# pqh22/ProxyTransformation

Hardware: AMD Instinct MI355X
Metric: scenes/sec (100k pts, 256 clusters, 64 proxies) (higher is better)
Workload: dtype f32; 1 GPU; cfg2: N=100000 pts, gs=8->M'=256 kept clusters, L=64 text + V=196 image proxies, d=256, eval forward; scenes_per_gpu=4, img_feat_dtype=bf16, input_sets_rotated=3, streams=1, lanes=1 (one forward at a time), setup_forwards=32

## Files before the change

proxytransformation_amd/csrc/api.hip:

```cpp
#include <atomic>
#include <chrono>
#include <cmath>
#include <cstdlib>
#include <cstring>
#include <mutex>
#include <utility>
#include <vector>

#include "common.h"

namespace ptx {

static thread_local char g_err[512] = "";

void set_error(const char *fmt, ...)
{
    va_list ap;
    va_start(ap, fmt);
    vsnprintf(g_err, sizeof(g_err), fmt, ap);
    va_end(ap);
}

static const char *const kKernelNames[] = {
    "k_minmax", "k_cluster", "k_select", "k_tags",
    "k_slot_net<pointnet>", "k_img_mean", "k_gemm_nt[qkv0]",
    "k_gemm_nt[we]", "img_pass2", "img_pass3", "k_gemm_nt[o]", "k_gemm_nt[c_proj]",
    "k_ln_rows[norm_img]", "k_gemm_nt[qkv+proxy_proj]", "k_gemm_nt[pp_img]", "k_attn32[proxy_as_query]",
    "k_attn32[proxy_as_key]", "k_gemm_nt[proj]", "k_gemm_nt[fc1]", "k_gemm_nt[fc2]",
    "k_heads", "k_affine<compact>", "k_proxy_attn[fused]", "k_mlp[fc1+gelu+fc2]",
    "k_gate[fork]", "k_signal[join]", "k_gate[join]", "k_gate[tags]", "k_signal[tags]"};
enum Kid : int {
    KID_MINMAX = 0, KID_CLUSTER, KID_SELECT, KID_TAGS, KID_POINTNET,
    KID_IMG_MEAN, KID_IMG_QKV0, KID_IMG_WE, KID_IMG_SCORES, KID_IMG_GATHER, KID_IMG_O, KID_IMG_C,
    KID_IMG_LN, KID_BLK_QKV, KID_BLK_PP, KID_BLK_ATTN_A, KID_BLK_ATTN_B, KID_BLK_PROJ, KID_BLK_FC1,
    KID_BLK_FC2, KID_BLK_HEADS, KID_AFFINE, KID_BLK_ATTN_F, KID_BLK_MLP,
    KID_GATE_FORK, KID_SIGNAL_JOIN, KID_GATE_JOIN, KID_GATE_TAGS, KID_SIGNAL_TAGS, KID_COUNT};
static_assert(sizeof(kKernelNames) / sizeof(kKernelNames[0]) == KID_COUNT, "kernel name table");

struct TimingRec { int kid; hipEvent_t a, b; };
struct TimingState {
    std::mutex mu;
    uint64_t mask = 0;
    int every = 1;
    unsigned seen[64] = {};
    std::vector<TimingRec> pool;
    size_t used = 0;
};
static TimingState g_timing;

static thread_local hipEvent_t g_ext_a = nullptr, g_ext_b = nullptr;
bool timing_ext_take(hipEvent_t *a, hipEvent_t *b)
{
    if (g_ext_a == nullptr) return false;
    *a = g_ext_a; *b = g_ext_b;
    g_ext_a = g_ext_b = nullptr;
    return true;
}

struct Timed {
    hipEvent_t stop = nullptr; hipStream_t st;
    Timed(int kid, hipStream_t s, bool ext = false) : st(s) {
        if (!((g_timing.mask >> kid) & 1u)) return;
        hipStreamCaptureStatus cap = hipStreamCaptureStatusNone;
        if (hipStreamIsCapturing(s, &cap) != hipSuccess || cap != hipStreamCaptureStatusNone) return;
        std::lock_guard<std::mutex> lk(g_timing.mu);
        if (g_timing.seen[kid]++ % (unsigned)g_timing.every != 0) return;
        if (g_timing.used == g_timing.pool.size()) {
            hipEvent_t a, b;
            if (hipEventCreate(&a) != hipSuccess || hipEventCreate(&b) != hipSuccess) return;
            g_timing.pool.push_back(TimingRec{kid, a, b});
        }
        TimingRec &pr = g_timing.pool[g_timing.used++];
        pr.kid = kid;
        if (ext) { g_ext_a = pr.a; g_ext_b = pr.b; return; }
        (void)hipEventRecord(pr.a, st);
        stop = pr.b;
    }
    ~Timed() {
        if (stop) (void)hipEventRecord(stop, st);
        if (g_ext_a != nullptr) {
            (void)hipEventRecord(g_ext_a, st); (void)hipEventRecord(g_ext_b, st);
            g_ext_a = g_ext_b = nullptr;
        }
    }
};
#define PTX_TIMED(kid, st, call) do { ::ptx::Timed t_(kid, st); PTX_TRY(call); } while (0)
#define PTX_TIMED_EXT(kid, st, call) do { ::ptx::Timed t_(kid, st, true); PTX_TRY(call); } while (0)

static inline float attn_scale(int hd) { return (float)(1.0 / std::sqrt((double)hd)); }

int validate_shape(const PtxShape &s)
{
    const long M = (long)s.grid_size * s.grid_size * s.grid_size;
    PTX_REQUIRE(s.B >= 1 && s.N >= 1, "shape: B=%d N=%d", s.B, s.N);
    PTX_REQUIRE(s.grid_size >= 1 && M <= (1 << 20), "shape: grid_size=%d", s.grid_size);
    PTX_REQUIRE(s.K >= 1 && s.K <= 63, "shape: num_sub K=%d must be in [1,63]", s.K);
    PTX_REQUIRE(s.Mk >= 1 && s.Mk <= s.Mt && s.Mt <= M, "shape: need 1 <= Mk=%d <= Mt=%d <= M=%ld", s.Mk, s.Mt, M);
    PTX_REQUIRE(s.C == 256 || s.C == 512, "shape: embed_dim=%d; supported: 256 (the reference, PRE:302) and 512", s.C);
    PTX_REQUIRE((s.heads == 4 || s.heads == 8 || s.heads == 16) && (s.C / s.heads == 32 || s.C / s.heads == 64),
                "shape: num_heads=%d with embed_dim=%d; the image-pool and attention kernels are built for 4, 8 or 16 heads of "
                "head_dim 32 or 64", s.heads, s.C);
    PTX_REQUIRE(s.Mt <= 4096, "shape: Mt=%d clusters after the empty-drop; the farthest point sampling holds at most 4096", s.Mt);
    PTX_REQUIRE(s.hidden >= 4 && s.hidden % 4 == 0, "shape: hidden=%d", s.hidden);
    PTX_REQUIRE(s.in_dim >= 64 && s.in_dim % 64 == 0 && s.in_dim <= 2048,
                "shape: in_dim=%d must be a multiple of 64, at most 2048", s.in_dim);
    PTX_REQUIRE(s.L >= 1 && s.V >= 1, "shape: L=%d V=%d", s.L, s.V);
    PTX_REQUIRE(s.img_dtype >= 0 && s.img_dtype <= 2, "shape: img_dtype=%d (0 fp32, 1 bf16, 2 fp16)", s.img_dtype);
    if (s.img_dtype == 0) PTX_REQUIRE(s.hw >= 4 && s.hw <= 256, "shape: H*W=%d (fp32 image features: 4..256 pixels)", s.hw);
    else PTX_REQUIRE(s.hw >= 8 && s.hw <= 256, "shape: H*W=%d (16-bit image features: 8..256 pixels)", s.hw);
    PTX_REQUIRE((long)s.Mk * s.K < (1l << 31) - 1, "shape: Mk*K overflows the ownership tag");
    return PTX_OK;
}

PrepLayout prep_layout(const PtxShape &s)
{
    PrepLayout P{};
    size_t o = 0;
    auto take = [&](size_t n) { size_t r = o; o += align_up(n, 64); return r; };
    P.hd = s.C / s.heads;
    P.KT1 = s.in_dim + s.hw + 1;
    P.KT2p = (int)align_up((size_t)s.in_dim + s.hw + 1, 4);
    P.off_ab = take(2 * kSlotHidden); P.enc_ab = take(2 * (size_t)s.C);
    P.ttn_ab = take(6); P.itn_ab = take(18);
    P.posb_t = take((size_t)s.Mk * s.C); P.posb_i = take((size_t)s.Mk * s.C);
    P.w3 = take((size_t)3 * s.C * s.in_dim); P.b3 = take((size_t)3 * s.C);
    P.t1 = take((size_t)s.heads * P.KT1 * P.hd);
    P.t2 = take((size_t)s.heads * P.hd * P.KT2p);
    P.ppg_w = take((size_t)s.C * s.C); P.ppg_c = take(s.C);
    for (int i = 0; i < 2; ++i) {
        P.fc1g_w[i] = take((size_t)s.hidden * s.C); P.fc1g_c[i] = take(s.hidden);
        const size_t planes = mlp_fused_supported(s.C, s.hidden, 1, 0) ? (size_t)s.hidden * s.C * 3 / 2 : 0;
        P.mlp_w1p[i] = take(planes); P.mlp_w2p[i] = take(planes);
    }
    for (int i = 0; i < 2; ++i) P.qkvb[i] = take((size_t)s.Mk * 3 * s.C);
    P.total = o;
    return P;
}

struct LayoutForce { int v[4]; };
static LayoutForce layout_force()
{
    LayoutForce f{{-1, -1, -1, -1}};
    if (const char *e = getenv("PTX_LAYOUT"))
        for (int i = 0; i < 4 && e[i] != '\0'; ++i) f.v[i] = e[i] == '0' ? 0 : (e[i] == '1' ? 1 : -1);
    return f;
}
struct LayoutChoice { double est_cluster, est_image; bool cluster_on_caller, img_late, early; LayoutForce lf; };
static LayoutChoice choose_layout(const PtxShape &S)
{
    static const LayoutForce lf = layout_force();
    LayoutChoice c{};
    c.lf = lf;
    const int B = S.B, Kd = S.Mt - S.Mk;
    const double img_mb = (double)B * S.V * S.in_dim * S.hw * (S.img_dtype == 0 ? 4.0 : 2.0) * 1e-6;
    c.est_cluster = 80.0 + 0.42 * Kd;
    c.est_image = 40.0 + (S.img_dtype == 0 ? 0.98 : 0.78) * img_mb;
    c.cluster_on_caller = lf.v[0] >= 0 ? lf.v[0] != 0 : c.est_cluster > c.est_image + 60.0;
    c.img_late = c.cluster_on_caller && (lf.v[2] >= 0 ? lf.v[2] != 0 : c.est_image + 60.0 < 0.8 * c.est_cluster);
    const double est_all = 1.8 * 12.0 * (double)B * S.Mt * S.C * S.C / 70e6;
    c.early = c.cluster_on_caller && (lf.v[1] >= 0 ? lf.v[1] != 0 : (Kd >= 128 && (long)B * S.Mk >= 1024 && est_all < 3.0 * 0.42 * Kd));
    return c;
}

WsLayout ws_layout(const PtxShape &s)
{
    WsLayout L{};
    const PrepLayout P = prep_layout(s);
    size_t o = 0;
    auto take = [&](size_t bytes) { size_t r = o; o += align_up(bytes, 256); return r; };
    const size_t B = s.B, N = s.N, K = s.K, C = s.C;
    const size_t M = (size_t)s.grid_size * s.grid_size * s.grid_size;
    const size_t Mk = s.Mk, Mt = s.Mt, Kd = s.Mt - s.Mk;
    const size_t nimg = B * s.V, Lp = s.L > s.V ? s.L : s.V, R = B * Mk;
    L.zero_begin = o;
    L.mm_enc = take(B * 6 * 4);
    L.scene_acc = take(B * 2 * 4);
    L.tag = take(B * N * 4);
    L.fa_ticket = take(2 * B * s.heads * 4);
    L.mlp_ticket = take(mlp_ticket_bytes((int)R));
    L.mm_ticket = take(4);
    L.zero_bytes = o - L.zero_begin;
    L.minmax = take(B * 6 * 4);
    L.centers0 = take(B * M * 3 * 4); L.cluster1 = take(B * M * K * 3 * 4);
    L.offsets = take(B * M * 3 * 4);  L.centers = take(B * M * 3 * 4);
    L.idx2 = take(B * M * K * 4);     L.cluster2 = take(B * M * K * 3 * 4);
    L.pad_count = take(B * M * 4);
    L.order = take(B * Mt * 4); L.picks = take(B * (Kd ? Kd : 1) * 4); L.keep = take(B * Mk * 4); L.ksrc = take(B * Mk * 4);
    L.kcenter = take(B * Mk * 3 * 4); L.kcluster = take(B * Mk * K * 3 * 4); L.kidx = take(B * Mk * K * 4);
    L.drop_idx = take(B * (Kd ? Kd : 1) * K * 4);
    L.tile_counts = take(B * (size_t)cdiv(s.N, kTilePts) * 4);
    L.point_proxy = take(R * C * 4);
    for (int i = 0; i < 2; ++i) L.x_in[i] = take(R * C * 4);
    bool may_early = false;
    for (int dt = 0; dt < 3; ++dt) { PtxShape t = s; t.img_dtype = dt; may_early = may_early || choose_layout(t).early; }
    const size_t em = may_early ? 1 : 0;
    L.pp_all = take(em * B * Mt * C * 4); L.order_e = take(em * B * Mt * 4);
    for (int i = 0; i < 2; ++i) { L.xln_all[i] = take(em * B * Mt * C * 4); L.g_all[i] = take(em * B * Mt * 3 * C * 4); }
    L.fm = take(nimg * s.in_dim * 4); L.qkv0 = take(nimg * 3 * C * 4);
    L.we = take(nimg * s.heads * (size_t)P.KT1 * 4);
    {
        const size_t pool_b = img_pool_bytes((int)nimg, s.in_dim, P.KT2p - s.in_dim), gbuf_b = nimg * s.heads * (size_t)P.KT2p * 4;
        L.pool = L.gbuf = take(pool_b > gbuf_b ? pool_b : gbuf_b);
    }
    L.obuf = take(nimg * C * 4); L.cbuf = take(nimg * C * 4); L.img_proxy = take(nimg * C * 4);
    for (int i = 0; i < 2; ++i) {
        L.qkv[i] = take(R * 3 * C * 4); L.pt[i] = take(B * Lp * C * 4); L.pv[i] = take(B * Lp * C * 4);
        L.ao[i] = take(R * C * 4); L.x1[i] = take(R * C * 4); L.xn2[i] = take(0);
        L.hbuf[i] = take(mlp_fused_supported(s.C, s.hidden, (int)R, 0) ? 0 : R * (size_t)s.hidden * 4);
        L.x2[i] = take(R * C * 4); L.guide[i] = take(R * C * 4);
        L.head[i] = take(R * 9 * 4);
        L.lnp_x1[i] = take(R * (C / 32) * 2 * 4);
    }
    L.lnp_img = take(nimg * (C / 32) * 2 * 4);
    const size_t fsp = fattn_split_for(s.B, s.heads);
    L.fa_part = take(fsp > 1 ? 2 * B * s.heads * fsp * Mk * kFaPartRow * 4 : 0);
    L.mlp_part = take(mlp_fused_supported(s.C, s.hidden, (int)R, 0) ? mlp_part_bytes((int)R) : 0);
    L.total = o;
    return L;
}

}
struct PtxContext {
    int dev = -1;
    hipStream_t st = nullptr, lo = nullptr;
    hipEvent_t fork = nullptr, join = nullptr, aux = nullptr, tags = nullptr, early_a = nullptr, early_b = nullptr;
    uint32_t *gate = nullptr; uint32_t gate_seq = 0;
    uint32_t *gate_err = nullptr;
    bool gates_on = false;
    bool probed = false; hipStream_t probed_st = nullptr;
    bool lo_ok = false;
    hipStream_t last_st = nullptr;
    bool have_last = false;
    uint64_t gate_ticks = 0, probe_ticks = 0; int gate_trap = 0;
    std::mutex mu;
};
namespace ptx {

static bool env_on(const char *name)
{
    const char *v = getenv(name);
    return v != nullptr && v[0] != '\0' && !(v[0] == '0' && v[1] == '\0');
}
static bool gates_allowed()
{
    if (const char *g = getenv("PTX_GATE")) return atoi(g) != 0;
    for (const char *name : {"ROCPROF_COUNTER_COLLECTION", "ROCPROF_COUNTERS", "ROCPROF_COUNTER_GROUPS", "ROCPROF_ADVANCED_THREAD_TRACE",
                             "ROCPROF_PC_SAMPLING_UNIT", "ROCPROF_PC_SAMPLING_METHOD", "AMD_SERIALIZE_KERNEL", "AMD_SERIALIZE_COPY",
                             "HIP_LAUNCH_BLOCKING", "CUDA_LAUNCH_BLOCKING", "ROCPROFILER_METRICS_PATH", "ROCP_METRICS"})
        if (env_on(name)) return false;
    return true;
}

static int context_init(PtxContext *c)
{
    PTX_HIP(hipGetDevice(&c->dev));
    int lo = 0, hi = 0;
    PTX_HIP(hipDeviceGetStreamPriorityRange(&lo, &hi));
    PTX_HIP(hipStreamCreateWithPriority(&c->st, hipStreamNonBlocking, hi));
    PTX_HIP(hipStreamCreateWithPriority(&c->lo, hipStreamNonBlocking, lo));
    PTX_HIP(hipEventCreateWithFlags(&c->fork, hipEventDisableTiming));
    PTX_HIP(hipEventCreateWithFlags(&c->join, hipEventDisableTiming));
    PTX_HIP(hipEventCreateWithFlags(&c->aux, hipEventDisableTiming));
    PTX_HIP(hipEventCreateWithFlags(&c->tags, hipEventDisableTiming));
    PTX_HIP(hipEventCreateWithFlags(&c->early_a, hipEventDisableTiming));
    PTX_HIP(hipEventCreateWithFlags(&c->early_b, hipEventDisableTiming));
    if (gates_allowed()) {
        PTX_HIP(hipMalloc(reinterpret_cast<void **>(&c->gate), 256));
        PTX_HIP(hipMemset(c->gate, 0, 256));
        PTX_HIP(hipHostMalloc(reinterpret_cast<void **>(&c->gate_err), 64, hipHostMallocMapped));
        c->gate_err[0] = 0u;
        int khz = 0;
        if (hipDeviceGetAttribute(&khz, hipDeviceAttributeWallClockRate, c->dev) != hipSuccess || khz <= 0) khz = 100000;
        const char *ms_env = getenv("PTX_GATE_TIMEOUT_MS");
        const long ms = ms_env ? atol(ms_env) : 30000;
        c->gate_ticks = (uint64_t)(ms > 0 ? ms : 1) * (uint64_t)khz;
        c->probe_ticks = (uint64_t)20 * (uint64_t)khz;
#ifdef PTX_TEST_HOOKS
        c->gate_trap = env_on("PTX_GATE_TRAP") ? 1 : 0;
#endif
        c->gates_on = true;
    }
    return PTX_OK;
}

static void context_release(PtxContext *c)
{
    if (c->gate) (void)hipFree(c->gate);
    if (c->gate_err) (void)hipHostFree(c->gate_err);
    c->gate = nullptr; c->gate_err = nullptr; c->gates_on = false;
    if (c->fork) (void)hipEventDestroy(c->fork);
    if (c->join) (void)hipEventDestroy(c->join);
    if (c->aux) (void)hipEventDestroy(c->aux);
    if (c->tags) (void)hipEventDestroy(c->tags);
    if (c->early_a) (void)hipEventDestroy(c->early_a);
    if (c->early_b) (void)hipEventDestroy(c->early_b);
    if (c->st) (void)hipStreamDestroy(c->st);
    if (c->lo) (void)hipStreamDestroy(c->lo);
    c->fork = c->join = c->aux = c->tags = nullptr; c->st = c->lo = nullptr;
}

static std::mutex g_default_mu;
static PtxContext *g_default_ctx[16] = {};

static int default_context(PtxContext **out)
{
    int dev = 0;
    PTX_HIP(hipGetDevice(&dev));
    PTX_REQUIRE(dev >= 0 && dev < 16, "device %d out of range", dev);
    std::lock_guard<std::mutex> lk(g_default_mu);
    if (g_default_ctx[dev] == nullptr) {
        PtxContext *c = new PtxContext();
        const int rc = context_init(c);
        if (rc != PTX_OK) { context_release(c); delete c; return rc; }
        g_default_ctx[dev] = c;
    }
    *out = g_default_ctx[dev];
    return PTX_OK;
}

int make_scene_pts(const float *stacked, const float *const *list, int B, int N, ScenePts *out)
{
    PTX_REQUIRE(B >= 1 && B <= kMaxScenes, "at most %d scenes per call (got %d): split the batch", kMaxScenes, B);
    PTX_REQUIRE(stacked || list, "null points");
    for (int b = 0; b < kMaxScenes; ++b) out->p[b] = nullptr;
    for (int b = 0; b < B; ++b) {
        out->p[b] = list ? list[b] : stacked + (size_t)b * N * 3;
        PTX_REQUIRE(out->p[b] != nullptr, "null point cloud for scene %d", b);
    }
    return PTX_OK;
}

template <typename T>
static inline T *at(void *base, size_t off) { return reinterpret_cast<T *>(static_cast<char *>(base) + off); }

__global__ void k_signal(uint32_t *flag, uint32_t seq)
{
    if (threadIdx.x == 0) __hip_atomic_store(flag, seq, __ATOMIC_RELAXED, __HIP_MEMORY_SCOPE_AGENT);
}
__global__ void k_gate(GateRef g)
{
    if (threadIdx.x == 0) gate_wait(g);
}

static GateRef gate_ref(const PtxContext *c, int word, uint32_t seq, uint32_t site, bool probe = false)
{
    const uint64_t ticks = probe ? c->probe_ticks : ((site == 2 || site == 7) ? 2 * c->gate_ticks : c->gate_ticks);
    return GateRef{c->gate + word, seq, c->gate_err, probe ? nullptr : c->gate + 48, ticks, site, probe ? 0 : c->gate_trap};
}

static int gate_check(PtxContext *c)
{
    if (c->gate_err == nullptr) return PTX_OK;
    const uint32_t e = *reinterpret_cast<volatile uint32_t *>(c->gate_err);
    if (e == 0u) return PTX_OK;
    static const char *const site_name[] = {"?", "fork (clustering stream waiting for the caller's stream)",
                                            "join (caller's stream waiting for the other chain)", "probe, fork direction",
                                            "probe, join direction", "?", "slot tags' fork (tag stream waiting for the selection)",
                                            "slot tags' join (caller's stream waiting for the tags)"};
    const unsigned site = (e >> 24) & 0x7fu;
    c->gates_on = false;
    *reinterpret_cast<volatile uint32_t *>(c->gate_err) = 0u;
    (void)hipStreamSynchronize(c->st);
    if (c->have_last) (void)hipStreamSynchronize(c->last_st);
    (void)hipMemset(c->gate + 48, 0, 4);
    set_error("stream gate timed out at the %s of forward #%u: the two chains of that forward were not ordered and its outputs "
              "were set to NaN; this context now orders its streams with events (PTX_GATE=0 selects them from the start)",
              site_name[site < 8 ? site : 0], e & 0xffffffu);
    return PTX_EGATE;
}

static int gate_probe_pair(PtxContext *c, hipStream_t waiter, hipStream_t releaser, int word, uint32_t site, bool *ok)
{
    const uint32_t seq = ++c->gate_seq;
    hipLaunchKernelGGL(k_gate, dim3(1), dim3(64), 0, waiter, gate_ref(c, word, seq, site, true));
    PTX_LAUNCHED("k_gate[probe]");
    hipLaunchKernelGGL(k_signal, dim3(1), dim3(64), 0, releaser, c->gate + word, seq);
    PTX_LAUNCHED("k_signal[probe]");
    PTX_HIP(hipStreamSynchronize(waiter));
    PTX_HIP(hipStreamSynchronize(releaser));
    *ok = *reinterpret_cast<volatile uint32_t *>(c->gate_err) == 0u;
    *reinterpret_cast<volatile uint32_t *>(c->gate_err) = 0u;
    return PTX_OK;
}
static int gate_probe(PtxContext *c, hipStream_t st)
{
    c->probed = true; c->probed_st = st; c->lo_ok = false;
    if (!c->gates_on) return PTX_OK;
    PTX_HIP(hipStreamSynchronize(st));
    PTX_HIP(hipStreamSynchronize(c->st));
    PTX_HIP(hipStreamSynchronize(c->lo));
    bool fork_ok = false, join_ok = false, t1 = false, t2 = false;
    PTX_TRY(gate_probe_pair(c, c->st, st, 40, 3, &fork_ok));
    PTX_TRY(gate_probe_pair(c, st, c->st, 44, 4, &join_ok));
    if (!fork_ok || !join_ok) { c->gates_on = false; return PTX_OK; }
    PTX_TRY(gate_probe_pair(c, c->lo, c->st, 40, 3, &t1));
    PTX_TRY(gate_probe_pair(c, st, c->lo, 44, 4, &t2));
    c->lo_ok = t1 && t2;
    return PTX_OK;
}

static int run_img_proxy(const PtxShape &s, const PtxWeights &w, const float *prep, const void *img,
                         float *img_proxy, void *ws, hipStream_t st, int phase = 0, bool need_ln = true,
                         int i0 = 0, int ni = -1, uint32_t *gate = nullptr, uint32_t gate_seq = 0)
{
    const PrepLayout P = prep_layout(s);
    const WsLayout L = ws_layout(s);
    const int C = s.C, hd = P.hd, nall = s.B * s.V, nimg = ni < 0 ? nall : ni;
    float *fm = at<float>(ws, L.fm) + (size_t)i0 * s.in_dim, *qkv0 = at<float>(ws, L.qkv0) + (size_t)i0 * 3 * C;
    float *we = at<float>(ws, L.we) + (size_t)i0 * s.heads * P.KT1, *gbuf = at<float>(ws, L.gbuf) + (size_t)i0 * s.heads * P.KT2p;
    float *obuf = at<float>(ws, L.obuf) + (size_t)i0 * C, *cbuf = at<float>(ws, L.cbuf) + (size_t)i0 * C;
    if (img_proxy) img_proxy += (size_t)i0 * C;
    const int dt = s.img_dtype;
    img = static_cast<const char *>(img) + (size_t)i0 * s.in_dim * s.hw * (dt == 0 ? 4 : 2);
    float *Gs = nullptr, *E = nullptr, *ML = nullptr;
    const int EW = P.KT2p - s.in_dim;
    const bool pooled32 = img_pool32_supported(dt, s.in_dim, s.hw, s.heads);
    const bool pooled = pooled32 || img_pool_supported(dt, s.in_dim, s.hw, s.heads);
    if (pooled) {
        img_pool_layout(at<float>(ws, L.pool), nall, s.in_dim, EW, &Gs, &E, &ML);
        Gs += (size_t)i0 * 2 * s.heads * s.in_dim; E += (size_t)i0 * s.heads * EW; ML += (size_t)i0 * s.heads * 5;
    }
    if (phase != 2) PTX_TIMED(KID_IMG_MEAN, st, launch_img_mean(img, dt, nimg, s.in_dim, s.hw, fm, st, gate, gate_seq));
    if (phase == 1) return PTX_OK;
    const bool chained = hd == 32 && nimg < 4096;
    {
        GemmBatch g{}; g.n = 1;
        g.p[0] = GemmProb{fm, prep + P.w3, qkv0, prep + P.b3, nullptr, nullptr, nullptr,
                          nimg, 3 * C, s.in_dim, s.in_dim, s.in_dim, 3 * C, 0, 0, 0, EPI_NONE};
        if (chained) {
            g.p[0].w2 = prep + P.t1; g.p[0].c2 = we; g.p[0].n2 = P.KT1; g.p[0].ldc2 = s.heads * P.KT1;
            g.p[0].chain_tiles = s.heads; g.p[0].w2_stride = (long)P.KT1 * hd; g.p[0].c2_stride = P.KT1;
        }
        PTX_TIMED(KID_IMG_QKV0, st, launch_gemm(g, st));
    }
    if (!chained) {
        for (int h0 = 0; h0 < s.heads; h0 += kMaxGroups) {
            GemmBatch g{}; g.n = std::min(kMaxGroups, s.heads - h0);
            for (int h = h0; h < h0 + g.n; ++h)
                g.p[h - h0] = GemmProb{qkv0 + h * hd, prep + P.t1 + (size_t)h * P.KT1 * hd, we + (size_t)h * P.KT1,
                                       nullptr, nullptr, nullptr, nullptr, nimg, P.KT1, hd, 3 * C, hd,
                                       s.heads * P.KT1, 0, 0, 0, EPI_NONE};
            PTX_TIMED(KID_IMG_WE, st, launch_gemm(g, st));
        }
    }
    if (pooled32) {
        PTX_TIMED_EXT(KID_IMG_SCORES, st, launch_img_pool32(static_cast<const float *>(img), we, qkv0, nimg, s.in_dim, s.hw, C, P.KT1, EW,
                                                        attn_scale(hd), Gs, E, ML, st));
    } else if (pooled) {
        PTX_TIMED_EXT(KID_IMG_SCORES, st, launch_img_pool(img, dt, we, qkv0, nimg, s.in_dim, s.hw, C, P.KT1,
                                                      EW, attn_scale(hd), Gs, E, ML, st));
    } else {
        PTX_TIMED(KID_IMG_SCORES, st, launch_img_scores(img, dt, we, qkv0, nimg, s.in_dim, s.hw, s.heads, C, P.KT1,
                                                        P.KT2p, attn_scale(hd), gbuf, st));
        PTX_TIMED(KID_IMG_GATHER, st, launch_img_gather(img, dt, nimg, s.in_dim, s.hw, s.heads, P.KT2p, gbuf, st));
    }
    for (int h0 = 0; h0 < s.heads; h0 += kMaxGroups) {
        GemmBatch g{}; g.n = std::min(kMaxGroups, s.heads - h0);
        for (int h = h0; h < h0 + g.n; ++h) {
            GemmProb &gp = g.p[h - h0];
            gp = GemmProb{gbuf + (size_t)h * P.KT2p, prep + P.t2 + (size_t)h * hd * P.KT2p, obuf + h * hd,
                          w.v_b + h * hd, nullptr, gbuf + (size_t)h * P.KT2p + s.in_dim,
                          qkv0 + 2 * C + h * hd, nimg, hd, P.KT2p, s.heads * P.KT2p, P.KT2p, C,
                          0, s.heads * P.KT2p, 3 * C, EPI_NONE};
            if (pooled) {
                gp.A = nullptr; gp.rs = nullptr;
                gp.pg = Gs + (size_t)h * s.in_dim; gp.ldg = 2 * s.heads * s.in_dim; gp.gslab = s.heads * s.in_dim;
                gp.pe = E + (size_t)h * EW; gp.lde = s.heads * EW;
                gp.pml = ML + (size_t)h * 5; gp.ldml = s.heads * 5;
                gp.kg = s.in_dim;
            }
        }
        PTX_TIMED(KID_IMG_O, st, launch_gemm(g, st));
    }
    {
        GemmBatch g{}; g.n = 1;
        g.p[0] = GemmProb{obuf, w.c_w, cbuf, w.c_b, nullptr, nullptr, nullptr,
                          nimg, C, C, C, C, C, 0, 0, 0, EPI_NONE};
        g.p[0].lnp_out = at<float>(ws, L.lnp_img) + (size_t)i0 * (C / 32) * 2;
        PTX_TIMED(KID_IMG_C, st, launch_gemm(g, st));
    }
    if (need_ln) {
        LnBatch lb{}; lb.n = 1; lb.C = C; lb.eps = s.ln_eps;
        lb.p[0] = LnProb{cbuf, img_proxy, w.norm_img_w, w.norm_img_b, nullptr, nimg, 1};
        PTX_TIMED(KID_IMG_LN, st, launch_ln_rows(lb, st));
    }
    return PTX_OK;
}

struct Branch {
    const PtxBlock *blk; const float *x_in; const float *proxy; int Lp; const uint8_t *mask;
    const float *head_w, *head_b, *head_ab; int nout; float *head_out; float *guide; int slot;
    bool late_proxy;
    const float *proxy_lnp, *pp_gw, *pp_gc;
    const float *fc1_gw, *fc1_gc;
    const float *prep;
};

static bool fused_attn_pays(const PtxShape &s, const Branch *br, int nb)
{
    (void)br;
    const long wgs = (long)s.B * s.heads * nb;
    return s.Mk <= 256 || wgs >= 96;
}

static int run_blocks(const PtxShape &s, const Branch *br, int nb, const float *point_proxy, void *ws,
                      hipStream_t st, int phase = 0, int cd = 0, GateRef *join = nullptr, GateRef *tags_join = nullptr,
                      bool skip_qkv = false)
{
    const WsLayout L = ws_layout(s);
    const int C = s.C, R = s.B * s.Mk;
    {
        GemmBatch g{}; g.n = 0;
        for (int i = 0; i < nb; ++i) {
            const int sl = br[i].slot;
            if (phase != 2 && phase != 3 && phase != 4 && !skip_qkv)
                g.p[g.n++] = GemmProb{br[i].x_in, br[i].blk->qkv_w, at<float>(ws, L.qkv[sl]), br[i].blk->qkv_b,
                                      nullptr, nullptr, nullptr, R, 3 * C, C, C, C, 3 * C, 0, 0, 0, EPI_NONE};
            const bool now = phase == 0 || (phase == 1 && !br[i].late_proxy) || ((phase == 2 || phase == 3) && br[i].late_proxy);
            if (now && phase != 4) {
                GemmProb &q = g.p[g.n++];
                q = GemmProb{br[i].proxy, br[i].blk->pp_w, at<float>(ws, L.pt[sl]), br[i].blk->pp_b,
                             nullptr, nullptr, nullptr, s.B * br[i].Lp, C, C, C, C, C, 0, 0, 0, EPI_NONE};
                if (br[i].proxy_lnp != nullptr) {
                    q.W = br[i].pp_gw; q.bias = nullptr;
                    q.lnp_in = br[i].proxy_lnp; q.ln_c = br[i].pp_gc;
                    q.ln_parts = C / 32; q.ln_C = C; q.ln_eps = s.ln_eps;
                }
            }
        }
        if (g.n > 0 && (phase == 2 || phase == 1) && join != nullptr && join->flag != nullptr) { g.tail_gate = *join; join->flag = nullptr; }
        if (g.n > 0) PTX_TIMED(phase == 2 || phase == 3 ? KID_BLK_PP : KID_BLK_QKV, st, launch_gemm(g, st, cd));
        if (phase == 1 || phase == 3) return PTX_OK;
    }
    FAttnBatch fa{}; fa.nb = nb; fa.B = s.B; fa.heads = s.heads; fa.hd = C / s.heads; fa.n = s.Mk; fa.C = C;
    fa.scale = attn_scale(C / s.heads); fa.compute_dtype = cd;
    fa.split = fattn_split_for(s.B, s.heads); fa.part = at<float>(ws, L.fa_part); fa.tickets = at<int>(ws, L.fa_ticket);
    for (int i = 0; i < nb; ++i) {
        const int sl = br[i].slot;
        fa.p[i] = FAttnProb{at<float>(ws, L.qkv[sl]), at<float>(ws, L.pt[sl]), br[i].mask, at<float>(ws, L.ao[sl]), br[i].Lp};
    }
    const bool fused = fused_attn_supported(fa) && (cd == 1 || fused_attn_pays(s, br, nb));
    if (fused) PTX_TIMED(KID_BLK_ATTN_F, st, launch_proxy_attn(fa, st));
    AttnBatch a{}; a.n = nb; a.B = s.B; a.heads = s.heads; a.hd = C / s.heads; a.scale = attn_scale(C / s.heads);
    for (int i = 0; i < nb && !fused; ++i) {
        const int sl = br[i].slot;
        float *qkv = at<float>(ws, L.qkv[sl]);
        a.p[i] = AttnProb{at<float>(ws, L.pt[sl]), qkv + C, qkv + 2 * C, at<float>(ws, L.pv[sl]), nullptr,
                          br[i].Lp, s.Mk, C, 3 * C, 3 * C, C,
                          (long)br[i].Lp * C, (long)s.Mk * 3 * C, (long)s.Mk * 3 * C, (long)br[i].Lp * C};
    }
    if (!fused) PTX_TIMED(KID_BLK_ATTN_A, st, launch_attn32(a, st));
    for (int i = 0; i < nb && !fused; ++i) {
        const int sl = br[i].slot;
        float *qkv = at<float>(ws, L.qkv[sl]);
        a.p[i] = AttnProb{qkv, at<float>(ws, L.pt[sl]), at<float>(ws, L.pv[sl]), at<float>(ws, L.ao[sl]),
                          br[i].mask, s.Mk, br[i].Lp, 3 * C, C, C, C,
                          (long)s.Mk * 3 * C, (long)br[i].Lp * C, (long)br[i].Lp * C, (long)s.Mk * C};
    }
    if (!fused) PTX_TIMED(KID_BLK_ATTN_B, st, launch_attn32(a, st));
    {
        GemmBatch g{}; g.n = nb;
        for (int i = 0; i < nb; ++i) {
            const int sl = br[i].slot;
            g.p[i] = GemmProb{at<float>(ws, L.ao[sl]), br[i].blk->proj_w, at<float>(ws, L.x1[sl]),
                              br[i].blk->proj_b, point_proxy, nullptr, nullptr, R, C, C, C, C, C, C, 0, 0, EPI_NONE};
            g.p[i].lnp_out = at<float>(ws, L.lnp_x1[sl]);
        }
        if (tags_join != nullptr && tags_join->flag != nullptr) { g.tail_gate = *tags_join; tags_join->flag = nullptr; }
        PTX_TIMED(KID_BLK_PROJ, st, launch_gemm(g, st, cd));
    }
    if (mlp_fused_supported(C, s.hidden, R, cd)) {
        const PrepLayout P = prep_layout(s);
        MlpBatch mb{}; mb.n = nb; mb.ln_eps = s.ln_eps; mb.compute_dtype = cd;
        mb.part = at<float>(ws, L.mlp_part); mb.tickets = at<int>(ws, L.mlp_ticket);
        for (int i = 0; i < nb; ++i) {
            const int sl = br[i].slot;
            mb.p[i] = MlpProb{at<float>(ws, L.x1[sl]), at<float>(ws, L.lnp_x1[sl]), br[i].prep + P.mlp_w1p[sl],
                              br[i].prep + P.mlp_w2p[sl], br[i].fc1_gc, br[i].blk->fc2_b,
                              at<float>(ws, L.x2[sl]), R,
                              br[i].blk->out_norm_w, br[i].blk->out_norm_b, br[i].head_w, br[i].head_b, br[i].head_ab,
                              br[i].head_out, br[i].guide, br[i].nout};
        }
        PTX_TIMED(KID_BLK_MLP, st, launch_mlp(mb, st));
        return PTX_OK;
    } else {
    {
        GemmBatch g{}; g.n = nb;
        for (int i = 0; i < nb; ++i) {
            const int sl = br[i].slot;
            g.p[i] = GemmProb{at<float>(ws, L.x1[sl]), br[i].fc1_gw, at<float>(ws, L.hbuf[sl]),
                              nullptr, nullptr, nullptr, nullptr, R, s.hidden, C, C, C, s.hidden,
                              0, 0, 0, EPI_GELU};
            g.p[i].lnp_in = at<float>(ws, L.lnp_x1[sl]); g.p[i].ln_c = br[i].fc1_gc;
            g.p[i].ln_parts = C / 32; g.p[i].ln_C = C; g.p[i].ln_eps = s.ln_eps;
        }
        PTX_TIMED(KID_BLK_FC1, st, launch_gemm(g, st, cd));
    }
    {
        GemmBatch g{}; g.n = nb;
        for (int i = 0; i < nb; ++i) {
            const int sl = br[i].slot;
            g.p[i] = GemmProb{at<float>(ws, L.hbuf[sl]), br[i].blk->fc2_w, at<float>(ws, L.x2[sl]),
                              br[i].blk->fc2_b, at<float>(ws, L.x1[sl]), nullptr, nullptr, R, C, s.hidden,
                              s.hidden, s.hidden, C, C, 0, 0, EPI_NONE};
        }
        PTX_TIMED(KID_BLK_FC2, st, launch_gemm(g, st, cd));
    }
    }
    HeadBatch hb{}; hb.n = nb; hb.C = C; hb.eps = s.ln_eps;
    for (int i = 0; i < nb; ++i) {
        const int sl = br[i].slot;
        hb.p[i] = HeadProb{at<float>(ws, L.x2[sl]), br[i].blk->out_norm_w, br[i].blk->out_norm_b,
                           br[i].head_w, br[i].head_b, br[i].head_ab, br[i].head_out, br[i].guide, R, br[i].nout};
    }
    PTX_TIMED(KID_BLK_HEADS, st, launch_heads(hb, st));
    return PTX_OK;
}

static Branch make_branch(const PtxShape &s, const PtxWeights &w, const float *prep, int which,
                          const float *x_in, const float *proxy, int Lp, const uint8_t *mask,
                          float *head_out, float *guide)
{
    const PrepLayout P = prep_layout(s);
    Branch b{};
    b.blk = which == 0 ? &w.text : &w.img;
    b.x_in = x_in; b.proxy = proxy; b.Lp = Lp; b.mask = mask;
    b.head_w = which == 0 ? w.text_trans_w : w.img_trans_w;
    b.head_b = which == 0 ? w.text_trans_b : w.img_trans_b;
    b.head_ab = prep + (which == 0 ? P.ttn_ab : P.itn_ab);
    b.nout = which == 0 ? 3 : 9;
    b.head_out = head_out; b.guide = guide; b.slot = which; b.late_proxy = which == 1;
    b.proxy_lnp = nullptr; b.pp_gw = prep + P.ppg_w; b.pp_gc = prep + P.ppg_c;
    b.fc1_gw = prep + P.fc1g_w[which]; b.fc1_gc = prep + P.fc1g_c[which];
    b.prep = prep;
    return b;
}

static int check_bufs(const PtxShape *s, const void *ws, size_t ws_bytes)
{
    PTX_REQUIRE(s != nullptr, "null shape");
    PTX_TRY(validate_shape(*s));
    PTX_REQUIRE(ws != nullptr, "null workspace");
    const size_t need = ws_layout(*s).total;
    if (ws_bytes < need) { set_error("workspace too small: %zu < %zu bytes", ws_bytes, need); return PTX_ENOSPACE; }
    PTX_REQUIRE((reinterpret_cast<uintptr_t>(ws) & 255) == 0, "workspace must be 256-byte aligned");
    return PTX_OK;
}

}

using namespace ptx;

extern "C" {

int ptx_abi_version(void) { return PTX_ABI_VERSION; }

int ptx_kernel_count(void) { return KID_COUNT; }
const char *ptx_kernel_name(int kid) { return kid >= 0 && kid < KID_COUNT ? kKernelNames[kid] : nullptr; }

int ptx_timing_select(int kid)
{
    PTX_REQUIRE(kid >= -1 && kid < KID_COUNT, "ptx_timing_select: kid=%d", kid);
    std::lock_guard<std::mutex> lk(g_timing.mu);
    g_timing.mask = kid < 0 ? 0 : (1ull << kid);
    g_timing.used = 0;
    for (unsigned &s : g_timing.seen) s = 0;
    return PTX_OK;
}

int ptx_timing_every(int n)
{
    PTX_REQUIRE(n >= 1, "ptx_timing_every: n=%d", n);
    std::lock_guard<std::mutex> lk(g_timing.mu);
    g_timing.every = n;
    return PTX_OK;
}

int ptx_timing_select_mask(uint64_t mask)
{
    static_assert(KID_COUNT <= 64, "timing mask is 64 bits");
    std::lock_guard<std::mutex> lk(g_timing.mu);
    g_timing.mask = mask & ((KID_COUNT >= 64) ? ~0ull : ((1ull << KID_COUNT) - 1));
    g_timing.used = 0;
    for (unsigned &s : g_timing.seen) s = 0;
    return PTX_OK;
}

static int timing_collect(int *launches, float *total_ms, int nsites)
{
    for (int k = 0; k < nsites; ++k) { launches[k] = 0; total_ms[k] = 0.0f; }
    for (size_t i = 0; i < g_timing.used; ++i) {
        const TimingRec &r = g_timing.pool[i];
        PTX_HIP(hipEventSynchronize(r.b));
        float ms = 0.0f;
        PTX_HIP(hipEventElapsedTime(&ms, r.a, r.b));
        const int k = nsites == 1 ? 0 : r.kid;
        if (k >= 0 && k < nsites) { launches[k] += 1; total_ms[k] += ms; }
    }
    g_timing.used = 0;
    return PTX_OK;
}

int ptx_timing_read(int *launches, float *total_ms)
{
    PTX_REQUIRE(launches && total_ms, "ptx_timing_read: null argument");
    std::lock_guard<std::mutex> lk(g_timing.mu);
    return timing_collect(launches, total_ms, 1);
}

int ptx_timing_read_sites(int *launches, float *total_ms, int n)
{
    PTX_REQUIRE(launches && total_ms && n == KID_COUNT, "ptx_timing_read_sites: need arrays of ptx_kernel_count() = %d entries", KID_COUNT);
    std::lock_guard<std::mutex> lk(g_timing.mu);
    return timing_collect(launches, total_ms, n);
}
const char *ptx_last_error(void) { return g_err; }

int ptx_context_create(PtxContext **ctx)
{
    PTX_REQUIRE(ctx != nullptr, "ptx_context_create: null argument");
    PtxContext *c = new PtxContext();
    const int rc = context_init(c);
    if (rc != PTX_OK) { context_release(c); delete c; *ctx = nullptr; return rc; }
    *ctx = c;
    return PTX_OK;
}

int ptx_context_destroy(PtxContext *ctx)
{
    if (ctx == nullptr) return PTX_OK;
    if (ctx->st) (void)hipStreamSynchronize(ctx->st);
    if (ctx->lo) (void)hipStreamSynchronize(ctx->lo);
    context_release(ctx);
    delete ctx;
    return PTX_OK;
}

int ptx_context_check(PtxContext *ctx)
{
    PTX_REQUIRE(ctx != nullptr, "ptx_context_check: null context");
    std::lock_guard<std::mutex> lk(ctx->mu);
    return gate_check(ctx);
}

int ptx_context_sync_check(PtxContext *ctx)
{
    PTX_REQUIRE(ctx != nullptr, "ptx_context_sync_check: null context");
    std::lock_guard<std::mutex> lk(ctx->mu);
    if (ctx->have_last) PTX_HIP(hipStreamSynchronize(ctx->last_st));
    PTX_HIP(hipStreamSynchronize(ctx->st));
    PTX_HIP(hipStreamSynchronize(ctx->lo));
    return gate_check(ctx);
}

int ptx_context_gates(const PtxContext *ctx) { return ctx != nullptr && ctx->gates_on ? (ctx->lo_ok ? 3 : 1) : 0; }
// ... 534 lines not shown
```

proxytransformation_amd/csrc/common.h:

```cpp
#pragma once
#include <hip/hip_runtime.h>
#include <cstdarg>
#include <cstdint>
#include <cstdio>

#include "../../include/proxyt.h"

namespace ptx {

void set_error(const char *fmt, ...);
bool timing_ext_take(hipEvent_t *start, hipEvent_t *stop);

#define PTX_REQUIRE(cond, ...)                                   \
    do {                                                         \
        if (!(cond)) {                                           \
            ::ptx::set_error(__VA_ARGS__);                       \
            return PTX_EINVAL;                                   \
        }                                                        \
    } while (0)

#define PTX_HIP(expr)                                                              \
    do {                                                                           \
        hipError_t e_ = (expr);                                                    \
        if (e_ != hipSuccess) {                                                    \
            ::ptx::set_error("%s failed: %s", #expr, hipGetErrorString(e_));       \
            return PTX_ELAUNCH;                                                    \
        }                                                                          \
    } while (0)

#define PTX_LAUNCHED(name)                                                         \
    do {                                                                           \
        hipError_t e_ = hipGetLastError();                                         \
        if (e_ != hipSuccess) {                                                    \
            ::ptx::set_error("launch %s failed: %s", name, hipGetErrorString(e_)); \
            return PTX_ELAUNCH;                                                    \
        }                                                                          \
    } while (0)

#define PTX_TRY(expr)                 \
    do {                              \
        int rc_ = (expr);             \
        if (rc_ != PTX_OK) return rc_;\
    } while (0)

constexpr int kWave = 64;
constexpr int kSlotHidden = 256;
constexpr int kTilePts = 2048;

inline size_t align_up(size_t x, size_t a) { return (x + a - 1) / a * a; }
inline int cdiv(int a, int b) { return (a + b - 1) / b; }

__device__ __forceinline__ int lane_id() { return threadIdx.x & 63; }

#define PTX_ROR_F(v, n) __int_as_float(__builtin_amdgcn_update_dpp(0, __float_as_int(v), 0x120 + (n), 0xf, 0xf, false))
#define PTX_ROR_I(v, n) __builtin_amdgcn_update_dpp(0, (v), 0x120 + (n), 0xf, 0xf, false)
#define PTX_LANE_F(v, l) __int_as_float(__builtin_amdgcn_readlane(__float_as_int(v), (l)))
__device__ __forceinline__ float wave_sum(float v) {
    v += PTX_ROR_F(v, 8); v += PTX_ROR_F(v, 4); v += PTX_ROR_F(v, 2); v += PTX_ROR_F(v, 1);
    return (PTX_LANE_F(v, 0) + PTX_LANE_F(v, 16)) + (PTX_LANE_F(v, 32) + PTX_LANE_F(v, 48));
}
__device__ __forceinline__ int wave_sum(int v) {
    v += PTX_ROR_I(v, 8); v += PTX_ROR_I(v, 4); v += PTX_ROR_I(v, 2); v += PTX_ROR_I(v, 1);
    return (__builtin_amdgcn_readlane(v, 0) + __builtin_amdgcn_readlane(v, 16)) +
           (__builtin_amdgcn_readlane(v, 32) + __builtin_amdgcn_readlane(v, 48));
}
__device__ __forceinline__ float wave_max(float v) {
    v = fmaxf(v, PTX_ROR_F(v, 8)); v = fmaxf(v, PTX_ROR_F(v, 4)); v = fmaxf(v, PTX_ROR_F(v, 2)); v = fmaxf(v, PTX_ROR_F(v, 1));
    return fmaxf(fmaxf(PTX_LANE_F(v, 0), PTX_LANE_F(v, 16)), fmaxf(PTX_LANE_F(v, 32), PTX_LANE_F(v, 48)));
}
__device__ __forceinline__ float wave_min(float v) {
    v = fminf(v, PTX_ROR_F(v, 8)); v = fminf(v, PTX_ROR_F(v, 4)); v = fminf(v, PTX_ROR_F(v, 2)); v = fminf(v, PTX_ROR_F(v, 1));
    return fminf(fminf(PTX_LANE_F(v, 0), PTX_LANE_F(v, 16)), fminf(PTX_LANE_F(v, 32), PTX_LANE_F(v, 48)));
}
__device__ __forceinline__ float wave_max_dpp(float v) { return wave_max(v); }
__device__ __forceinline__ uint32_t f2ord(float f) {
    uint32_t u = __float_as_uint(f);
    return (u & 0x80000000u) ? ~u : (u | 0x80000000u);
}
__device__ __forceinline__ float ord2f(uint32_t u) {
    return __uint_as_float((u & 0x80000000u) ? (u & 0x7fffffffu) : ~u);
}

__device__ __forceinline__ float dist2_nofma(float ax, float ay, float az, float bx, float by, float bz) {
    float dx = __fsub_rn(ax, bx), dy = __fsub_rn(ay, by), dz = __fsub_rn(az, bz);
    return __fadd_rn(__fadd_rn(__fmul_rn(dx, dx), __fmul_rn(dy, dy)), __fmul_rn(dz, dz));
}

__device__ __forceinline__ float gelu_erf(float x)
{
    const float z = fabsf(x) * 0.70710678118654752440f;
    const float t = __frcp_rn(fmaf(0.3275911f, z, 1.0f));
    float p = fmaf(1.061405429f, t, -1.453152027f);
    p = fmaf(p, t, 1.421413741f);
    p = fmaf(p, t, -0.284496736f);
    p = fmaf(p, t, 0.254829592f);
    const float erfz = 1.0f - p * t * __expf(-z * z);
    return 0.5f * x * (1.0f + copysignf(erfz, x));
}

struct GateRef {
    const uint32_t *flag; uint32_t seq;
    uint32_t *err;
    uint32_t *poison;
    uint64_t ticks;
    uint32_t site;
    int trap;
};
__device__ __forceinline__ void gate_wait(const GateRef &g)
{
    const uint64_t t0 = __builtin_amdgcn_s_memrealtime();
    for (unsigned it = 0;; ++it) {
        if ((int32_t)(__hip_atomic_load(g.flag, __ATOMIC_RELAXED, __HIP_MEMORY_SCOPE_AGENT) - g.seq) >= 0) return;
        if (it < 64) __builtin_amdgcn_s_sleep(4); else __builtin_amdgcn_s_sleep(64);
        if ((it & 7u) == 7u && __builtin_amdgcn_s_memrealtime() - t0 > g.ticks) break;
    }
    if (g.poison) __hip_atomic_store(g.poison, 1u, __ATOMIC_RELAXED, __HIP_MEMORY_SCOPE_AGENT);
    if (g.err) __hip_atomic_store(g.err, 0x80000000u | (g.site << 24) | (g.seq & 0xffffffu), __ATOMIC_RELEASE, __HIP_MEMORY_SCOPE_SYSTEM);
    if (g.trap) __builtin_trap();
}

constexpr int kMaxScenes = 32;
struct ScenePts { const float *p[kMaxScenes]; };
template <bool WAIT>
__device__ __forceinline__ void minmax_block(const float *__restrict__ p, int N, uint32_t *__restrict__ mm_enc, int b,
                                             int chunk, int nchunks, float (*red)[6])
{
    float lo[3] = {INFINITY, INFINITY, INFINITY}, hi[3] = {-INFINITY, -INFINITY, -INFINITY};
    const int tid = chunk * 256 + threadIdx.x;
    const int nth = nchunks * 256;
    const bool vec = ((N & 3) == 0) && ((reinterpret_cast<uintptr_t>(p) & 15) == 0);
    if (vec) {
        const float4 *p4 = reinterpret_cast<const float4 *>(p);
        const int nq = N >> 2;
        constexpr int U = 4;
        for (int q0 = tid; q0 < nq; q0 += nth * U) {
            float4 v[U][3];
#pragma unroll
            for (int u = 0; u < U; ++u) {
                const int q = min(q0 + u * nth, nq - 1);
                v[u][0] = p4[3 * q]; v[u][1] = p4[3 * q + 1]; v[u][2] = p4[3 * q + 2];
            }
#pragma unroll
            for (int u = 0; u < U; ++u) {
                const float4 a = v[u][0], c = v[u][1], e = v[u][2];
                const float xs[4] = {a.x, a.w, c.z, e.y}, ys[4] = {a.y, c.x, c.w, e.z}, zs[4] = {a.z, c.y, e.x, e.w};
#pragma unroll
                for (int i = 0; i < 4; ++i) {
                    lo[0] = fminf(lo[0], xs[i]); hi[0] = fmaxf(hi[0], xs[i]);
                    lo[1] = fminf(lo[1], ys[i]); hi[1] = fmaxf(hi[1], ys[i]);
                    lo[2] = fminf(lo[2], zs[i]); hi[2] = fmaxf(hi[2], zs[i]);
                }
            }
        }
    } else {
        for (int i = tid; i < N; i += nth) {
#pragma unroll
            for (int d = 0; d < 3; ++d) {
                float v = p[(size_t)i * 3 + d];
                lo[d] = fminf(lo[d], v); hi[d] = fmaxf(hi[d], v);
            }
        }
    }
#pragma unroll
    for (int d = 0; d < 3; ++d) { lo[d] = wave_min(lo[d]); hi[d] = wave_max(hi[d]); }
    const int w = threadIdx.x >> 6;
    if (lane_id() == 0) {
#pragma unroll
        for (int d = 0; d < 3; ++d) { red[w][d] = lo[d]; red[w][3 + d] = hi[d]; }
    }
    __syncthreads();
    if (threadIdx.x < 6) {
        const int d = threadIdx.x;
        float v = red[0][d];
        for (int i = 1; i < 4; ++i) v = d < 3 ? fminf(v, red[i][d]) : fmaxf(v, red[i][d]);
        uint32_t old = 0u;
        if (d < 3) { if (v != INFINITY) old = atomicMax(&mm_enc[b * 6 + d], ~f2ord(v)); }
        else       { if (v != -INFINITY) old = atomicMax(&mm_enc[b * 6 + d], f2ord(v)); }
        if (WAIT) asm volatile("" :: "v"(old));
    }
}
inline int minmax_chunks(int N) { int c = (N + 256 * 16 - 1) / (256 * 16); return c < 1 ? 1 : (c > 256 ? 256 : c); }

__device__ __forceinline__ void mean_prologue(uint32_t *gate, uint32_t gate_seq)
{
    if (gate != nullptr && blockIdx.x == 0 && threadIdx.x == 0) __hip_atomic_store(gate, gate_seq, __ATOMIC_RELAXED, __HIP_MEMORY_SCOPE_AGENT);
}

struct PrepLayout {
    size_t off_ab, enc_ab;
    size_t ttn_ab, itn_ab;
    size_t posb_t, posb_i;
    size_t w3, b3;
    size_t t1;
    size_t t2;
    size_t ppg_w, ppg_c;
    size_t fc1g_w[2], fc1g_c[2];
    size_t mlp_w1p[2], mlp_w2p[2];
    size_t qkvb[2];
    size_t total;
    int KT1, KT2p, hd;
};
PrepLayout prep_layout(const PtxShape &s);

struct WsLayout {
    size_t zero_begin, zero_bytes;
    size_t mm_enc;
    size_t scene_acc;
    size_t tag;
    size_t fa_ticket;
    size_t mlp_ticket;
    size_t mm_ticket;
    size_t minmax, centers0, cluster1, offsets, centers, idx2, cluster2, pad_count;
    size_t order, picks, keep, ksrc, kcenter, kcluster, kidx, drop_idx, tile_counts;
    size_t point_proxy, x_in[2];
    size_t pp_all, xln_all[2], g_all[2];
    size_t order_e;
    size_t fm, qkv0, we, pool, gbuf, obuf, cbuf, img_proxy;
    size_t qkv[2], pt[2], pv[2], ao[2], x1[2], xn2[2], hbuf[2], x2[2], guide[2], head[2];
    size_t lnp_img, lnp_x1[2];
    size_t fa_part;
    size_t mlp_part;
    size_t total;
};
WsLayout ws_layout(const PtxShape &s);

int validate_shape(const PtxShape &s);

enum : int { EPI_NONE = 0, EPI_GELU = 1 };
struct GemmProb {
    const float *A; const float *W; float *C;
    const float *bias;
    const float *res;
    const float *rs;
    const float *ad;
    int R, N, K, lda, ldw, ldc, ldres, rs_stride, ldad, epi;
    const float *pg, *pe, *pml; int ldg, gslab, lde, ldml, kg;
    float *lnp_out;
    const float *lnp_in, *ln_c; int ln_parts, ln_C; float ln_eps;
    const float *w2; float *c2; int n2, ldc2, chain_tiles; long w2_stride, c2_stride;
};
constexpr int kMaxGroups = 8;
struct GemmBatch {
    GemmProb p[kMaxGroups]; int n; int rotate;
    GateRef tail_gate;
};
int launch_gemm(const GemmBatch &gb, hipStream_t st, int compute_dtype = 0);
int gemm_policy(int min_tiles_128);

struct LnProb { const float *x; float *y; const float *w; const float *b; const float *add; int R, add_rows; };
struct LnBatch { LnProb p[2]; int n; int C; float eps; };
int launch_ln_rows(const LnBatch &lb, hipStream_t st);

struct HeadProb {
    const float *x; const float *nw; const float *nb;
    const float *hw; const float *hb;
    const float *ab;
    float *out; float *guide; int R, nout;
};
struct HeadBatch { HeadProb p[2]; int n; int C; float eps; };
int launch_heads(const HeadBatch &hb, hipStream_t st);

struct AttnProb {
    const float *Q, *K, *V; float *O; const uint8_t *mask;
    int nq, nk, ldq, ldk, ldv, ldo;
    long sQ, sK, sV, sO;
};
struct AttnBatch { AttnProb p[2]; int n; int B, heads, hd; float scale; };
int launch_attn32(const AttnBatch &ab, hipStream_t st);

struct FAttnProb { const float *qkv, *pt; const uint8_t *mask; float *out; int Lp; };
struct FAttnBatch {
    FAttnProb p[2]; int nb, B, heads, hd, n, C; float scale; int compute_dtype;
    int split; float *part; int *tickets;
};
int fattn_split_for(int B, int heads);
constexpr int kFaMaxSplit = 4, kFaPartRow = 34;
bool fused_attn_supported(const FAttnBatch &ab);
int launch_proxy_attn(const FAttnBatch &ab, hipStream_t st);

struct MlpProb {
    const float *x1, *lnp;
    const void *w1p, *w2p;
    const float *fc1_c, *b2;
    float *x2; int R;
    const float *nw, *nb, *hw, *hb, *ab; float *head_out, *guide; int nout;
};
struct MlpBatch { MlpProb p[2]; int n; float ln_eps; float *part; int *tickets; int compute_dtype; };
bool mlp_fused_supported(int C, int hidden, int R, int compute_dtype);
size_t mlp_part_bytes(int R);
size_t mlp_ticket_bytes(int R);
int launch_mlp(const MlpBatch &mb, hipStream_t st);
int launch_prep_planes(const float *W, int rows, int K, void *out, hipStream_t st);
int launch_prep_lnfold(const float *W, const float *gamma, const float *beta, const float *bias, int N, int K, float *Wg,
                       float *cv, hipStream_t st);

int make_scene_pts(const float *stacked, const float *const *list, int B, int N, ScenePts *out);

int launch_minmax(const ScenePts &points, int B, int N, uint32_t *mm_enc, hipStream_t st);
int launch_ball_query(const float *centers, const uint32_t *mm_enc, const float *lin, int gs,
                      float margin, float *minmax_out, float *centers_out, const ScenePts &points,
                      int B, int M, int N, int K, float radius, int32_t *idx, float *cluster,
                      int32_t *pad_count, hipStream_t st);
int launch_offset_net(const float *ab, const PtxSlotMlp &mlp, const float *map_w,
                      const float *centers_in, const float *cluster, const float *minmax,
                      int BM, int M, int K, float margin, float *centers_out, float *offsets_out,
                      hipStream_t st);
int launch_pointnet(const float *ab, const PtxSlotMlp &mlp, const float *kcenter,
                    const float *kcluster, int BM, int Mk, int K, int width, float *point_proxy,
                    const PtxBlock *blk_t, const PtxBlock *blk_i, const float *posb_t,
                    const float *posb_i, float *xin_t, float *xin_i, float ln_eps,
                    const int32_t *ksrc, int Msrc, hipStream_t st, uint32_t *head_flag = nullptr, uint32_t head_seq = 0,
                    bool center_src = false);
int launch_order(const PtxShape &s, const int32_t *pad_count, const int32_t *order_override, int32_t *order, hipStream_t st);
int launch_qkv_gather(const float *pp_all, const float *const g[2], const float *const tb[2], const int32_t *ksrc, int B, int M, int Mk,
                      int C, float *point_proxy, float *const qkv[2], hipStream_t st);
int launch_cluster(const PtxShape &s, const uint32_t *mm_enc, const float *lin, const ScenePts &points,
                   const float *off_ab, const PtxSlotMlp &mlp, const float *map_w, const float *centers_override,
                   float *minmax_out, float *centers0, float *cluster1, float *offsets, float *centers,
                   int32_t *idx2, float *cluster2, int32_t *pad_count, hipStream_t st, hipEvent_t done = nullptr);
int launch_select(const PtxShape &s, const int32_t *idx, const float *centers, const float *cluster,
                  const int32_t *pad_count, const int32_t *order_override, int32_t *order,
                  int32_t *picks, int32_t *keep, float *kcenter, float *kcluster, int32_t *kidx,
                  int32_t *drop_idx, uint32_t *tag, hipStream_t st);
int launch_select_order(const PtxShape &s, const float *centers, const int32_t *pad_count,
                        const int32_t *order_override, int32_t *order, int32_t *picks, int32_t *keep,
                        float *kcenter, int32_t *ksrc, uint32_t *mm_clear, hipStream_t st, bool critical,
                        hipEvent_t done, const GateRef *tail = nullptr);
int launch_tags(const PtxShape &s, const int32_t *idx, const int32_t *order, const int32_t *picks, const int32_t *ksrc,
                uint32_t *tag, int32_t *tile_counts, int32_t *counts, int32_t *scene_acc, hipStream_t st,
                const int32_t *keep = nullptr);
int launch_select_slots(const PtxShape &s, const int32_t *idx, const float *cluster, const int32_t *order,
                        const int32_t *picks, const int32_t *keep, float *kcluster, int32_t *kidx,
                        int32_t *drop_idx, uint32_t *tag, hipStream_t st);
int launch_t_ln_fwd(const float *x, const float *w, const float *b, int R, int C, float eps, float *y, float *stats, hipStream_t st);
int t_ln_chunks(int R);
int launch_t_ln_bwd(const float *x, const float *stats, const float *w, const float *dy, int R, int C, float *dx, float *part, hipStream_t st);
int launch_tile_count(const uint32_t *tag, int B, int N, int32_t *tile_counts, int32_t *counts, int32_t *scene_acc,
                      hipStream_t st);
int launch_affine(const PtxShape &s, const ScenePts &points, uint32_t *tag, const float *kcenter,
                  const float *translate, const float *transform, float *out, int32_t *counts,
                  const int32_t *tile_counts, bool compact, bool clear_tag, hipStream_t st,
                  const uint32_t *poison = nullptr);

int launch_img_mean(const void *img, int dt, int nimg, int in_dim, int hw, float *fm, hipStream_t st,
                    uint32_t *gate = nullptr, uint32_t gate_seq = 0);
int launch_img_scores(const void *img, int dt, const float *we, const float *qkv0, int nimg, int in_dim,
                      int hw, int heads, int C, int KT1, int KT2p, float scale, float *gbuf, hipStream_t st);
int launch_img_gather(const void *img, int dt, int nimg, int in_dim, int hw, int heads, int KT2p, float *gbuf,
                      hipStream_t st);
bool img_pool_supported(int dt, int in_dim, int hw, int heads);
size_t img_pool_bytes(int nimg, int in_dim, int EW);
void img_pool_layout(float *scratch, int nimg, int in_dim, int EW, float **Gs, float **E, float **ML);
int launch_img_pool(const void *img, int dt, const float *we, const float *qkv0, int nimg, int in_dim, int hw, int C,
                    int KT1, int EW, float scale, float *Gs, float *E, float *ML, hipStream_t st);

bool img_pool32_supported(int dt, int in_dim, int hw, int heads);
int launch_img_pool32(const float *img, const float *we, const float *qkv0, int nimg, int in_dim, int hw, int C, int KT1, int EW,
                      float scale, float *Gs, float *E, float *ML, hipStream_t st);

int run_prepare(const PtxShape &s, const PtxWeights &w, float *prep, hipStream_t st);

}
```

proxytransformation_amd/csrc/gemm.hip:

```cpp
#include <atomic>
#include <cstdlib>

#include "common.h"
#include "split3.h"
#include "mfma64.h"

namespace ptx {


__device__ __forceinline__ void pin4(float4 &v) { asm volatile("" : "+v"(v.x), "+v"(v.y), "+v"(v.z), "+v"(v.w)); }
__device__ __forceinline__ void ln_row_stats(const GemmProb &pr, int row, float &mu, float &rstd)
{
    const float2 *pp = reinterpret_cast<const float2 *>(pr.lnp_in) + (size_t)row * pr.ln_parts;
    constexpr int kMaxParts = 16;
    float2 v[kMaxParts];
#pragma unroll
    for (int t = 0; t < kMaxParts; ++t) v[t] = pp[min(t, pr.ln_parts - 1)];
    float s1 = 0.0f, s2 = 0.0f;
#pragma unroll
    for (int t = 0; t < kMaxParts; ++t) { s1 += t < pr.ln_parts ? v[t].x : 0.0f; s2 += t < pr.ln_parts ? v[t].y : 0.0f; }
    const float inv = 1.0f / (float)pr.ln_C;
    mu = s1 * inv;
    float between = 0.0f;
#pragma unroll
// ... 149 lines not shown
        const char *A_ = smem + (buf_) * kXBuf + (wr * 32 + li) * XROW;                    \
        const char *W_ = smem + (buf_) * kXBuf + 3 * kXPlane + (wc * 32 + li) * XROW;      \
        _Pragma("unroll") for (int kg = 0; kg < BK / 16; ++kg) {                           \
            const int o_ = xswz(li, kg * 2 + hh);            \
            const bf16x8 a1 = *reinterpret_cast<const bf16x8 *>(A_ + o_);                  \
            const bf16x8 b1 = *reinterpret_cast<const bf16x8 *>(W_ + o_);                  \
            if (NP == 1) {                                        \
                acc = __builtin_amdgcn_mfma_f32_32x32x16_bf16(a1, b1, acc, 0, 0, 0);       \
                continue;                                                                  \
            }                                                                              \
            const bf16x8 a2 = *reinterpret_cast<const bf16x8 *>(A_ + o_ + kXPlane);        \
            const bf16x8 a3 = *reinterpret_cast<const bf16x8 *>(A_ + o_ + 2 * kXPlane);    \
            const bf16x8 b2 = *reinterpret_cast<const bf16x8 *>(W_ + o_ + kXPlane);        \
            const bf16x8 b3 = *reinterpret_cast<const bf16x8 *>(W_ + o_ + 2 * kXPlane);    \
            acc = __builtin_amdgcn_mfma_f32_32x32x16_bf16(a3, b1, acc, 0, 0, 0);    \
            acc = __builtin_amdgcn_mfma_f32_32x32x16_bf16(a2, b2, acc, 0, 0, 0);           \
            acc = __builtin_amdgcn_mfma_f32_32x32x16_bf16(a1, b3, acc, 0, 0, 0);           \
            acc = __builtin_amdgcn_mfma_f32_32x32x16_bf16(a2, b1, acc, 0, 0, 0);           \
            acc = __builtin_amdgcn_mfma_f32_32x32x16_bf16(a1, b2, acc, 0, 0, 0);           \
            acc = __builtin_amdgcn_mfma_f32_32x32x16_bf16(a1, b1, acc, 0, 0, 0);           \
        }                                                                                  \
    } while (0)

template <int NKG, int REP, int NP = 3, bool LN = false>
__global__ __launch_bounds__(256) void k_gemm64x(GemmBatch gb)
{
    constexpr int kXPlane = 64 * XROW, kXBuf = 6 * kXPlane;
    static_assert(2 * kXBuf >= 4 * 32 * 33 * 4, "the LayerNorm-partials scratch re-uses the staging area");
    const GemmProb pr = gb.p[blockIdx.z];
    const int row0 = blockIdx.x * 64, col0 = blockIdx.y * 64;
    if (row0 >= pr.R || col0 >= pr.N) return;
    __shared__ __attribute__((aligned(16))) char smem[2 * kXBuf];
    __shared__ float s_mu[64], s_rs[64];
    const int tid = threadIdx.x, lane = tid & 63, wid = tid >> 6;
    const bool ln = LN && pr.lnp_in != nullptr;
    const int wr = wid >> 1, wc = wid & 1;
    const int li = lane & 31, hh = lane >> 5;
    const int sr = tid >> 3, kq = (tid & 7) * 4;
    const size_t ao0 = (size_t)min(row0 + sr, pr.R - 1) * pr.lda, ao1 = (size_t)min(row0 + sr + 32, pr.R - 1) * pr.lda;
    const size_t wo0 = (size_t)min(col0 + sr, pr.N - 1) * pr.ldw, wo1 = (size_t)min(col0 + sr + 32, pr.N - 1) * pr.ldw;
    float4 aA0, aA1, wA0, wA1, aB0, aB1, wB0, wB1, aC0, aC1, wC0, wC1, aD0, aD1, wD0, wD1;
    f32x16 acc;
#pragma unroll
    for (int i = 0; i < 16; ++i) acc[i] = 0.0f;
    const int n = col0 + wc * 32 + li;
    const float bias = (pr.bias && n < pr.N) ? pr.bias[n] : 0.0f;
    float lnc = 0.0f;
    if (ln) lnc = pr.ln_c[min(n, pr.N - 1)];
    float resv[16];
#pragma unroll
    for (int r = 0; r < 16; ++r) {
        const int row = row0 + wr * 32 + (r & 3) + 8 * (r >> 2) + 4 * hh;
        resv[r] = (pr.res && row < pr.R && n < pr.N) ? pr.res[(size_t)row * pr.ldres + n] : 0.0f;
    }
#define PTX_X64_PIPE()                                                                     \
    do {                                                                                   \
        if (NP != 3) break;          \
        __builtin_amdgcn_sched_group_barrier(0x100, 12, 0);              \
        _Pragma("unroll") for (int g_ = 0; g_ < 12; ++g_) {                                \
            __builtin_amdgcn_sched_group_barrier(0x008, 1, 0);                             \
            __builtin_amdgcn_sched_group_barrier(0x002, 7, 0);                   \
            __builtin_amdgcn_sched_group_barrier(0x200, 1, 0);                             \
        }                                                                                  \
    } while (0)
#define PTX_X64_STEP(S, SN, par_)                                                          \
    if (it + 4 < 4 * NKG || rep + 1 < REP) PTX_X64_FETCH(S, kbase + it + 4);               \
    __builtin_amdgcn_sched_barrier(0);      \
    PTX_X64_COMPUTE(par_);                                                                 \
    PTX_X64_STASH(SN, 1 - (par_));                                                         \
    PTX_X64_PIPE();                                                                        \
    __syncthreads();                                                                       \
    ++it;
    PTX_X64_FETCH(A, 0); PTX_X64_FETCH(B, 1); PTX_X64_FETCH(C, 2); PTX_X64_FETCH(D, 3);
    float mu0 = 0.0f, mu1 = 0.0f;
    if (ln) {
        if (tid < 64) {
            float mu, rs;
            ln_row_stats(pr, min(row0 + tid, pr.R - 1), mu, rs);
            s_mu[tid] = mu; s_rs[tid] = rs;
        }
        __syncthreads();
        mu0 = s_mu[sr]; mu1 = s_mu[sr + 32];
    }
    PTX_X64_STASH(A, 0);
    __syncthreads();
    int kbase = 0;
    for (int rep = 0; rep < REP; ++rep) {
        int it = 0;
#pragma unroll
        for (int g = 0; g < NKG; ++g) {
            PTX_X64_STEP(A, B, 0) PTX_X64_STEP(B, C, 1) PTX_X64_STEP(C, D, 0) PTX_X64_STEP(D, A, 1)
        }
        kbase += 4 * NKG;
    }
#undef PTX_X64_STEP
#undef PTX_X64_PIPE
    const bool ncol = n < pr.N;
    float fin[16];
#pragma unroll
    for (int r = 0; r < 16; ++r) {
        const int rl = wr * 32 + (r & 3) + 8 * (r >> 2) + 4 * hh, row = row0 + rl;
        float v = acc[r] + bias;
        if (ln) v = fmaf(s_rs[rl], acc[r], lnc);
        if (pr.epi == EPI_GELU) v = gelu_erf(v);
        const bool ok = ncol && row < pr.R;
        if (ok) {
            if (pr.rs) v = fmaf(pr.rs[(size_t)row * pr.rs_stride], pr.ad[(size_t)row * pr.ldad + n], v);
            if (pr.res) v += resv[r];
            pr.C[(size_t)row * pr.ldc + n] = v;
        }
        fin[r] = ok ? v : 0.0f;
    }
    if (pr.lnp_out != nullptr)
        ln_tile_partials(pr, fin, reinterpret_cast<float *>(smem) + wid * (32 * 33), row0 + wr * 32, (col0 >> 5) + wc,
                         (pr.N + 31) >> 5);
    PTX_TAIL_GATE(gb, tid == 0);
}
#undef PTX_X64_FETCH
#undef PTX_X64_STASH
#undef PTX_X64_COMPUTE

constexpr int kYHalf = 128 * 16 + 64, kYPlane = 2 * kYHalf, kYBuf = 6 * kYPlane;
#ifndef PTX_G128_NM
#define PTX_G128_NM 8
#endif
#ifndef PTX_G128_ORDER
#define PTX_G128_ORDER 0
#endif
#ifndef PTX_G128_SWZ
#define PTX_G128_SWZ 0
#endif
#ifndef PTX_G128_PIPE
#define PTX_G128_PIPE 1
#endif

#define PTX_Y_FETCH(S, m_)                                                                 \
    do {                                                                                   \
        const int kc_ = (m_) * 32 + kq;                                                    \
        a##S##0 = *reinterpret_cast<const float4 *>(pr.A + ao0 + kc_);                     \
        a##S##1 = *reinterpret_cast<const float4 *>(pr.A + ao0 + kc_ + 16);                \
        a##S##2 = *reinterpret_cast<const float4 *>(pr.A + ao1 + kc_);                     \
        a##S##3 = *reinterpret_cast<const float4 *>(pr.A + ao1 + kc_ + 16);                \
        w##S##0 = *reinterpret_cast<const float4 *>(pr.W + wo0 + kc_);                     \
        w##S##1 = *reinterpret_cast<const float4 *>(pr.W + wo0 + kc_ + 16);                \
        w##S##2 = *reinterpret_cast<const float4 *>(pr.W + wo1 + kc_);                     \
        w##S##3 = *reinterpret_cast<const float4 *>(pr.W + wo1 + kc_ + 16);                \
    } while (0)
#define PTX_Y_STASH(S, h_, buf_)                                                           \
    do {                                                                                   \
        float4 &pa_ = (h_) ? a##S##1 : a##S##0, &pb_ = (h_) ? a##S##3 : a##S##2;           \
        float4 &pc_ = (h_) ? w##S##1 : w##S##0, &pd_ = (h_) ? w##S##3 : w##S##2;           \
        pin4(pa_); pin4(pb_); pin4(pc_); pin4(pd_);                                        \
        if (LN) { sub4(pa_, mu0); sub4(pb_, mu1); }                                        \
        char *d_ = smem + (buf_) * kYBuf + stash_off;                                      \
        stash_parts<NP>(d_, kYPlane, pa_);                                                 \
        stash_parts<NP>(d_ + 64 * 16, kYPlane, pb_);                                       \
        stash_parts<NP>(d_ + 3 * kYPlane, kYPlane, pc_);                                   \
        stash_parts<NP>(d_ + 3 * kYPlane + 64 * 16, kYPlane, pd_);                         \
    } while (0)
#define PTX_Y_COMPUTE(buf_)                                                                \
    do {                                                                                   \
        const char *A_ = smem + (buf_) * kYBuf + frag_a;                                   \
        const char *W_ = smem + (buf_) * kYBuf + frag_w;                                   \
        bf16x8 fa[2][3], fw[2][3];                                                         \
        _Pragma("unroll") for (int i_ = 0; i_ < 2; ++i_)                                   \
            _Pragma("unroll") for (int p_ = 0; p_ < NP; ++p_) {                            \
                fa[i_][p_] = *reinterpret_cast<const bf16x8 *>(A_ + i_ * 512 + p_ * kYPlane); \
                fw[i_][p_] = *reinterpret_cast<const bf16x8 *>(W_ + i_ * 512 + p_ * kYPlane); \
            }                                                                              \
        if (NP == 3 && PTX_G128_ORDER == 0) {                                              \
            constexpr int ta_[6] = {2, 1, 0, 1, 0, 0}, tw_[6] = {0, 1, 2, 0, 1, 0};        \
            _Pragma("unroll") for (int t_ = 0; t_ < 6; ++t_)                               \
                _Pragma("unroll") for (int q_ = 0; q_ < 4; ++q_)                           \
                    acc[q_] = __builtin_amdgcn_mfma_f32_32x32x16_bf16(fa[q_ >> 1][ta_[t_]], fw[q_ & 1][tw_[t_]], acc[q_], 0, 0, 0); \
        } else if (NP == 3) {                                                              \
            _Pragma("unroll") for (int q_ = 0; q_ < 4; ++q_) acc[q_] = mfma_split6(fa[q_ >> 1], fw[q_ & 1], acc[q_]); \
        } else {                                                                           \
            _Pragma("unroll") for (int q_ = 0; q_ < 4; ++q_)                               \
                acc[q_] = __builtin_amdgcn_mfma_f32_32x32x16_bf16(fa[q_ >> 1][0], fw[q_ & 1][0], acc[q_], 0, 0, 0); \
        }                                                                                  \
    } while (0)

template <int NM, int NP = 3, bool LN = false>
__global__ __launch_bounds__(256, 2) void k_gemm128x(GemmBatch gb, int nrep)
{
    static_assert(NM >= 2 && NM % 2 == 0, "macro steps come in P / Q pairs");
    const GemmProb pr = gb.p[blockIdx.z];
    int bx = blockIdx.x, by = blockIdx.y;
    if (PTX_G128_SWZ) {
        const unsigned total = gridDim.x * gridDim.y, lin = blockIdx.x + gridDim.x * blockIdx.y;
        if ((total & 7u) == 0u) {
            const unsigned l2 = (lin & 7u) * (total >> 3) + (lin >> 3);
            bx = (int)(l2 / gridDim.y); by = (int)(l2 % gridDim.y);
        }
    }
    const int row0 = bx * 128, col0 = by * 128;
    if (row0 >= pr.R || col0 >= pr.N) return;
    __shared__ __attribute__((aligned(16))) char smem[2 * kYBuf];
    __shared__ float s_mu[128], s_rs[128];
    static_assert(2 * kYBuf >= 4 * 32 * 33 * 4, "the LayerNorm-partials scratch re-uses the staging area");
    const int tid = threadIdx.x, lane = tid & 63, wid = tid >> 6;
    const int wr = wid >> 1, wc = wid & 1;
    const int li = lane & 31, hh = lane >> 5;
    const int sr = tid >> 2, kq = (tid & 3) * 4;
    const size_t ao0 = (size_t)min(row0 + sr, pr.R - 1) * pr.lda, ao1 = (size_t)min(row0 + sr + 64, pr.R - 1) * pr.lda;
    const size_t wo0 = (size_t)min(col0 + sr, pr.N - 1) * pr.ldw, wo1 = (size_t)min(col0 + sr + 64, pr.N - 1) * pr.ldw;
    const int stash_off = (kq >> 3) * kYHalf + sr * 16 + (kq & 4) * 2;
    const int frag_a = hh * kYHalf + (wr * 64 + li) * 16, frag_w = 3 * kYPlane + hh * kYHalf + (wc * 64 + li) * 16;
    float4 aP0, aP1, aP2, aP3, wP0, wP1, wP2, wP3, aQ0, aQ1, aQ2, aQ3, wQ0, wQ1, wQ2, wQ3;
    f32x16 acc[4];
#pragma unroll
    for (int q = 0; q < 4; ++q)
#pragma unroll
        for (int i = 0; i < 16; ++i) acc[q][i] = 0.0f;
    const int total = NM * nrep;
    PTX_Y_FETCH(P, 0);
    PTX_Y_FETCH(Q, 1);
    const bool ln = LN && pr.lnp_in != nullptr;
    float mu0 = 0.0f, mu1 = 0.0f;
    if (ln) {
        if (tid < 128) {
            float mu, rs;
            ln_row_stats(pr, min(row0 + tid, pr.R - 1), mu, rs);
            s_mu[tid] = mu; s_rs[tid] = rs;
        }
        __syncthreads();
        mu0 = s_mu[sr]; mu1 = s_mu[sr + 64];
    }
    PTX_Y_STASH(P, 0, 0);
    __syncthreads();
#define PTX_Y_PIPE()                                                                       \
    do {                                                                                   \
        if (NP != 3 || !PTX_G128_PIPE) break;                                              \
        __builtin_amdgcn_sched_group_barrier(0x100, 12, 0);              \
        _Pragma("unroll") for (int g_ = 0; g_ < 12; ++g_) {                                \
            __builtin_amdgcn_sched_group_barrier(0x008, 2, 0);                             \
            __builtin_amdgcn_sched_group_barrier(0x002, 8, 0);                             \
            __builtin_amdgcn_sched_group_barrier(0x200, 1, 0);                             \
        }                                                                                  \
    } while (0)
#define PTX_Y_MACRO(S, T, u_)                                                              \
    PTX_Y_COMPUTE(0);                                                                      \
    PTX_Y_STASH(S, 1, 1);                                                                  \
    PTX_Y_PIPE();                                                                          \
    __syncthreads();                                                                       \
    if ((u_) + 2 < NM || rep + 1 < nrep) PTX_Y_FETCH(S, mbase + (u_) + 2);                 \
    __builtin_amdgcn_sched_barrier(0);                                                     \
    PTX_Y_COMPUTE(1);                                                                      \
    if ((u_) + 1 < NM || rep + 1 < nrep) PTX_Y_STASH(T, 0, 0);                             \
    PTX_Y_PIPE();                                                                          \
    __syncthreads();
    int mbase = 0;
    for (int rep = 0; rep < nrep; ++rep) {
#pragma unroll
        for (int u = 0; u < NM; u += 2) {
            PTX_Y_MACRO(P, Q, u)
            PTX_Y_MACRO(Q, P, u + 1)
        }
        mbase += NM;
    }
#undef PTX_Y_MACRO
#undef PTX_Y_PIPE
    (void)total;
    float *scratch = reinterpret_cast<float *>(smem) + wid * (32 * 33);
#pragma unroll
    for (int q = 0; q < 4; ++q) {
        const int i = q >> 1, j = q & 1;
        const int n = col0 + wc * 64 + j * 32 + li, nc = min(n, pr.N - 1);
        const bool ncol = n < pr.N;
        const float bias = pr.bias ? pr.bias[nc] : 0.0f;
        float lnc = 0.0f;
        if (ln) lnc = pr.ln_c[nc];
        float resv[16], adv[16], rsv[16];
#pragma unroll
        for (int r = 0; r < 16; ++r) {
            const int row = min(row0 + wr * 64 + i * 32 + (r & 3) + 8 * (r >> 2) + 4 * hh, pr.R - 1);
            resv[r] = pr.res ? pr.res[(size_t)row * pr.ldres + nc] : 0.0f;
            adv[r] = pr.rs ? pr.ad[(size_t)row * pr.ldad + nc] : 0.0f;
            rsv[r] = pr.rs ? pr.rs[(size_t)row * pr.rs_stride] : 0.0f;
        }
        float fin[16];
#pragma unroll
        for (int r = 0; r < 16; ++r) {
            const int rl = wr * 64 + i * 32 + (r & 3) + 8 * (r >> 2) + 4 * hh, row = row0 + rl;
            float v = acc[q][r] + bias;
            if (ln) v = fmaf(s_rs[rl], acc[q][r], lnc);
            if (pr.epi == EPI_GELU) v = gelu_erf(v);
            const bool ok = ncol && row < pr.R;
            if (pr.rs) v = fmaf(rsv[r], adv[r], v);
            if (pr.res) v += resv[r];
            if (ok) pr.C[(size_t)row * pr.ldc + n] = v;
            fin[r] = ok ? v : 0.0f;
        }
        if (pr.lnp_out != nullptr)
            ln_tile_partials(pr, fin, scratch, row0 + wr * 64 + i * 32, (col0 >> 5) + wc * 2 + j, (pr.N + 31) >> 5);
    }
    PTX_TAIL_GATE(gb, tid == 0);
}
#undef PTX_Y_FETCH
#undef PTX_Y_STASH
#undef PTX_Y_COMPUTE

template <int SK, int AMODE, bool CHAIN = false, bool LN = false>
__global__ __launch_bounds__(SK * 64) void k_gemm32(GemmBatch gb)
{
    const GemmProb pr = gb.p[blockIdx.z];
    const int row0 = blockIdx.x * 32, col0 = blockIdx.y * 32;
    if (row0 >= pr.R || col0 >= pr.N) return;
    extern __shared__ __attribute__((aligned(16))) float lds[];
    const int lane = threadIdx.x & 63;
    const int wv = __builtin_amdgcn_readfirstlane(threadIdx.x >> 6);
    float *base = lds + (size_t)wv * (4 * 32 * LDT);
    const int li = lane & 31, hh = lane >> 5;
    const int nk = (pr.K + BK - 1) / BK, per = (nk + SK - 1) / SK;
    const int it0 = wv * per, it1 = min(nk, it0 + per);
    const int r0 = lane >> 3, kq = (lane & 7) * 4;
    const size_t a0 = (size_t)min(row0 + r0, pr.R - 1) * pr.lda, a1 = (size_t)min(row0 + r0 + 8, pr.R - 1) * pr.lda;
    const size_t a2 = (size_t)min(row0 + r0 + 16, pr.R - 1) * pr.lda, a3 = (size_t)min(row0 + r0 + 24, pr.R - 1) * pr.lda;
    const size_t w0 = (size_t)min(col0 + r0, pr.N - 1) * pr.ldw, w1 = (size_t)min(col0 + r0 + 8, pr.N - 1) * pr.ldw;
    const size_t w2 = (size_t)min(col0 + r0 + 16, pr.N - 1) * pr.ldw, w3 = (size_t)min(col0 + r0 + 24, pr.N - 1) * pr.ldw;
    const float4 z4 = make_float4(0.f, 0.f, 0.f, 0.f);
    float4 aA0, aA1, aA2, aA3, wA0, wA1, wA2, wA3, aB0, aB1, aB2, aB3, wB0, wB1, wB2, wB3;
    float4 gA0 = z4, gA1 = z4, gA2 = z4, gA3 = z4, gB0 = z4, gB1 = z4, gB2 = z4, gB3 = z4;
    int kA = 0, kB = 0;
    (void)kA; (void)kB;
    size_t g0 = 0, g1 = 0, g2 = 0, g3 = 0, e0 = 0, e1 = 0, e2 = 0, e3 = 0;
    float fc0[4] = {0.f, 0.f, 0.f, 0.f}, fc1[4] = {0.f, 0.f, 0.f, 0.f}, fct[4] = {0.f, 0.f, 0.f, 0.f};
    float *cts = lds + (size_t)SK * (4 * 32 * LDT);
    float *lnst = cts + 32 + wv * 64;
    const bool ln = LN && pr.lnp_in != nullptr;
    float mu4[4] = {0.0f, 0.0f, 0.0f, 0.0f};
    if (AMODE == 1) {
#pragma unroll
        for (int i = 0; i < 4; ++i) {
            const int row = min(row0 + r0 + 8 * i, pr.R - 1);
            const float *ml = pr.pml + (size_t)row * pr.ldml;
            const float m0 = ml[0], l0 = ml[1], m1 = ml[2], l1 = ml[3], s0 = ml[4];
            const float m = fmaxf(fmaxf(m0, m1), s0);
            const float x0 = __expf(m0 - m), x1 = __expf(m1 - m), xt = __expf(s0 - m);
            const float inv = 1.0f / ((l0 * x0 + l1 * x1) + xt);
            fc0[i] = x0 * inv; fc1[i] = x1 * inv; fct[i] = xt * inv;
            if (wv == 0 && (lane & 7) == 0) cts[r0 + 8 * i] = fct[i];
        }
        g0 = (size_t)min(row0 + r0, pr.R - 1) * pr.ldg; g1 = (size_t)min(row0 + r0 + 8, pr.R - 1) * pr.ldg;
        g2 = (size_t)min(row0 + r0 + 16, pr.R - 1) * pr.ldg; g3 = (size_t)min(row0 + r0 + 24, pr.R - 1) * pr.ldg;
        e0 = (size_t)min(row0 + r0, pr.R - 1) * pr.lde; e1 = (size_t)min(row0 + r0 + 8, pr.R - 1) * pr.lde;
        e2 = (size_t)min(row0 + r0 + 16, pr.R - 1) * pr.lde; e3 = (size_t)min(row0 + r0 + 24, pr.R - 1) * pr.lde;
    }
#define PTX_FETCH(S, j_)                                                                  \
    do {                                                                                  \
        int jj_ = min((j_), cnt - 1) + rot;                                               \
        jj_ -= jj_ >= cnt ? cnt : 0;                                                      \
        const int k_ = (it0 + jj_) * BK + kq, kc_ = min(k_, pr.K - 4);                    \
        const bool ok_ = k_ < pr.K;                                                       \
        if (AMODE == 0) {                                                                 \
            a##S##0 = *reinterpret_cast<const float4 *>(pr.A + a0 + kc_);                 \
            a##S##1 = *reinterpret_cast<const float4 *>(pr.A + a1 + kc_);                 \
            a##S##2 = *reinterpret_cast<const float4 *>(pr.A + a2 + kc_);                 \
            a##S##3 = *reinterpret_cast<const float4 *>(pr.A + a3 + kc_);                 \
        } else if (kc_ < pr.kg) {               \
            a##S##0 = *reinterpret_cast<const float4 *>(pr.pg + g0 + kc_);                \
            a##S##1 = *reinterpret_cast<const float4 *>(pr.pg + g1 + kc_);                \
            a##S##2 = *reinterpret_cast<const float4 *>(pr.pg + g2 + kc_);                \
            a##S##3 = *reinterpret_cast<const float4 *>(pr.pg + g3 + kc_);                \
            g##S##0 = *reinterpret_cast<const float4 *>(pr.pg + g0 + pr.gslab + kc_);     \
            g##S##1 = *reinterpret_cast<const float4 *>(pr.pg + g1 + pr.gslab + kc_);     \
            g##S##2 = *reinterpret_cast<const float4 *>(pr.pg + g2 + pr.gslab + kc_);     \
            g##S##3 = *reinterpret_cast<const float4 *>(pr.pg + g3 + pr.gslab + kc_);     \
        } else {                                                                          \
            a##S##0 = *reinterpret_cast<const float4 *>(pr.pe + e0 + (kc_ - pr.kg));      \
            a##S##1 = *reinterpret_cast<const float4 *>(pr.pe + e1 + (kc_ - pr.kg));      \
            a##S##2 = *reinterpret_cast<const float4 *>(pr.pe + e2 + (kc_ - pr.kg));      \
            a##S##3 = *reinterpret_cast<const float4 *>(pr.pe + e3 + (kc_ - pr.kg));      \
        }                                                                                 \
        k##S = kc_;                                                                       \
        w##S##0 = *reinterpret_cast<const float4 *>(pr.W + w0 + kc_);                     \
        w##S##1 = *reinterpret_cast<const float4 *>(pr.W + w1 + kc_);                     \
        w##S##2 = *reinterpret_cast<const float4 *>(pr.W + w2 + kc_);                     \
        w##S##3 = *reinterpret_cast<const float4 *>(pr.W + w3 + kc_);                     \
        if (!ok_) { w##S##0 = z4; w##S##1 = z4; w##S##2 = z4; w##S##3 = z4; }             \
    } while (0)
#define PTX_MERGE(S, i_)                                                                  \
    do {                                                                                  \
        if (k##S < pr.kg) {                                                               \
            a##S##i_ = make_float4(a##S##i_.x * fc0[i_] + g##S##i_.x * fc1[i_], a##S##i_.y * fc0[i_] + g##S##i_.y * fc1[i_], \
                                   a##S##i_.z * fc0[i_] + g##S##i_.z * fc1[i_], a##S##i_.w * fc0[i_] + g##S##i_.w * fc1[i_]); \
        } else {                                                                          \
            const int t_ = k##S - pr.kg;       \
            a##S##i_.x *= t_ == 0 ? fct[i_] : (t_ <= 128 ? fc0[i_] : fc1[i_]);           \
            a##S##i_.y *= t_ + 1 <= 128 ? fc0[i_] : fc1[i_];                              \
            a##S##i_.z *= t_ + 2 <= 128 ? fc0[i_] : fc1[i_];                              \
            a##S##i_.w *= t_ + 3 <= 128 ? fc0[i_] : fc1[i_];                              \
        }                                                                                 \
    } while (0)
#define PTX_STASH(S, buf_)                                                                \
    do {                                                                                  \
        float *A_s = base + (buf_) * (2 * 32 * LDT) + r0 * LDT + kq, *W_s = A_s + 32 * LDT; \
        if (AMODE == 1) { PTX_MERGE(S, 0); PTX_MERGE(S, 1); PTX_MERGE(S, 2); PTX_MERGE(S, 3); } \
        if (LN) { sub4(a##S##0, mu4[0]); sub4(a##S##1, mu4[1]); sub4(a##S##2, mu4[2]); sub4(a##S##3, mu4[3]); } \
        *reinterpret_cast<float4 *>(A_s) = a##S##0;                                       \
        *reinterpret_cast<float4 *>(A_s + 8 * LDT) = a##S##1;                             \
        *reinterpret_cast<float4 *>(A_s + 16 * LDT) = a##S##2;                            \
        *reinterpret_cast<float4 *>(A_s + 24 * LDT) = a##S##3;                            \
        *reinterpret_cast<float4 *>(W_s) = w##S##0;                                       \
        *reinterpret_cast<float4 *>(W_s + 8 * LDT) = w##S##1;                             \
        *reinterpret_cast<float4 *>(W_s + 16 * LDT) = w##S##2;                            \
        *reinterpret_cast<float4 *>(W_s + 24 * LDT) = w##S##3;                            \
    } while (0)
#define PTX_COMPUTE(buf_)                                                                 \
    do {                                                                                  \
        const float *A_ = base + (buf_) * (2 * 32 * LDT) + li * LDT + hh * 4, *W_ = A_ + 32 * LDT; \
        _Pragma("unroll") for (int kk = 0; kk < BK / 8; ++kk) {                           \
            const float4 a4 = *reinterpret_cast<const float4 *>(A_ + kk * 8);             \
            const float4 b4 = *reinterpret_cast<const float4 *>(W_ + kk * 8);             \
            acc = __builtin_amdgcn_mfma_f32_32x32x2f32(a4.x, b4.x, acc, 0, 0, 0);         \
            acc = __builtin_amdgcn_mfma_f32_32x32x2f32(a4.y, b4.y, acc, 0, 0, 0);         \
            acc = __builtin_amdgcn_mfma_f32_32x32x2f32(a4.z, b4.z, acc, 0, 0, 0);         \
            acc = __builtin_amdgcn_mfma_f32_32x32x2f32(a4.w, b4.w, acc, 0, 0, 0);         \
        }                                                                                 \
    } while (0)
    const int n = col0 + li;
    float bias = 0.0f, lnc = 0.0f, resv[16], adv[16], rsv[16];
#pragma unroll
    for (int r = 0; r < 16; ++r) { resv[r] = 0.0f; adv[r] = 0.0f; rsv[r] = 0.0f; }
    const bool has_ad = AMODE == 1 || pr.rs != nullptr;
    if (wv == 0) {
        const int nc = min(n, pr.N - 1);
        if (pr.bias) bias = pr.bias[nc];
        if (ln) lnc = pr.ln_c[nc];
#pragma unroll
        for (int r = 0; r < 16; ++r) {
            const int row = min(row0 + (r & 3) + 8 * (r >> 2) + 4 * hh, pr.R - 1);
            if (pr.res) resv[r] = pr.res[(size_t)row * pr.ldres + nc];
            if (has_ad) adv[r] = pr.ad[(size_t)row * pr.ldad + nc];
            if (AMODE != 1 && has_ad) rsv[r] = pr.rs[(size_t)row * pr.rs_stride];
        }
    }
    f32x16 acc;
#pragma unroll
    for (int i = 0; i < 16; ++i) acc[i] = 0.0f;
    const int cnt = it1 - it0;
    const int rot = (cnt > 1 && gb.rotate) ? (int)((blockIdx.x + 3u * blockIdx.y) % (unsigned)cnt) : 0;
    if (cnt > 0) {
        PTX_FETCH(A, 0);
        PTX_FETCH(B, 1);
        if (ln) {
            if (lane < 32) {
                float mu, rs;
                ln_row_stats(pr, min(row0 + lane, pr.R - 1), mu, rs);
                lnst[2 * lane] = mu; lnst[2 * lane + 1] = rs;
            }
#pragma unroll
            for (int i = 0; i < 4; ++i) mu4[i] = lnst[2 * (r0 + 8 * i)];
        }
        PTX_STASH(A, 0);
        for (int j = 0; j < cnt; j += 2) {
            PTX_FETCH(A, j + 2);
            PTX_COMPUTE(0);
            PTX_STASH(B, 1);
            if (j + 1 >= cnt) break;
            PTX_FETCH(B, j + 3);
            PTX_COMPUTE(1);
            PTX_STASH(A, 0);
        }
    }
#undef PTX_FETCH
#undef PTX_STASH
#undef PTX_COMPUTE
    const bool chain = CHAIN && pr.w2 != nullptr && (int)blockIdx.y < pr.chain_tiles;
    if (SK > 1) {
        __syncthreads();
        if (wv > 0) {
#pragma unroll
            for (int r = 0; r < 16; ++r) base[r * 64 + lane] = acc[r];
        }
        __syncthreads();
        if (wv > 0 && !chain) return;
        if (wv == 0) {
#pragma unroll
            for (int w = 1; w < SK; ++w) {
                const float *o = lds + (size_t)w * (4 * 32 * LDT);
#pragma unroll
                for (int r = 0; r < 16; ++r) acc[r] += o[r * 64 + lane];
            }
        }
    }
    if (wv == 0) {
        const bool ncol = n < pr.N;
        float fin[16];
#pragma unroll
        for (int r = 0; r < 16; ++r) {
            const int rl = (r & 3) + 8 * (r >> 2) + 4 * hh, row = row0 + rl;
            float v = acc[r] + bias;
            if (ln) v = fmaf(lnst[2 * rl + 1], acc[r], lnc);
            if (pr.epi == EPI_GELU) v = gelu_erf(v);
            const bool ok = ncol && row < pr.R;
            if (ok) {
                if (AMODE == 1) v = fmaf(cts[rl], adv[r], v);
                else if (pr.rs) v = fmaf(rsv[r], adv[r], v);
                if (pr.res) v += resv[r];
                pr.C[(size_t)row * pr.ldc + n] = v;
            }
            fin[r] = ok ? v : 0.0f;
        }
        if (pr.lnp_out != nullptr)
            ln_tile_partials(pr, fin, lds, row0, col0 >> 5, (pr.N + 31) >> 5);
        if (chain) {
#pragma unroll
            for (int r = 0; r < 16; ++r) lds[((r & 3) + 8 * (r >> 2) + 4 * hh) * LDT + li] = fin[r];
        }
    }
    PTX_TAIL_GATE(gb, threadIdx.x == 0);
    if (!chain) return;
    if (CHAIN) {
        __syncthreads();
        const float *W2 = pr.w2 + (size_t)blockIdx.y * pr.w2_stride;
        float *C2 = pr.c2 + (size_t)blockIdx.y * pr.c2_stride;
        float4 ya[4];
#pragma unroll
        for (int kk = 0; kk < 4; ++kk) ya[kk] = *reinterpret_cast<const float4 *>(lds + li * LDT + kk * 8 + hh * 4);
        const int nt2 = (pr.n2 + 31) >> 5;
        auto load_w2 = [&](int t, float4 (&wb)[4]) {
            const float *wr = W2 + (size_t)min(t * 32 + li, pr.n2 - 1) * 32 + hh * 4;
#pragma unroll
            for (int kk = 0; kk < 4; ++kk) wb[kk] = *reinterpret_cast<const float4 *>(wr + kk * 8);
        };
        float4 wb[4], wn[4];
        load_w2(min(wv, nt2 - 1), wb);
        for (int t = wv; t < nt2; t += SK) {
            const int m = t * 32 + li;
            load_w2(min(t + SK, nt2 - 1), wn);
            f32x16 c2;
#pragma unroll
            for (int i = 0; i < 16; ++i) c2[i] = 0.0f;
#pragma unroll
            for (int kk = 0; kk < 4; ++kk) {
                c2 = __builtin_amdgcn_mfma_f32_32x32x2f32(ya[kk].x, wb[kk].x, c2, 0, 0, 0);
                c2 = __builtin_amdgcn_mfma_f32_32x32x2f32(ya[kk].y, wb[kk].y, c2, 0, 0, 0);
                c2 = __builtin_amdgcn_mfma_f32_32x32x2f32(ya[kk].z, wb[kk].z, c2, 0, 0, 0);
                c2 = __builtin_amdgcn_mfma_f32_32x32x2f32(ya[kk].w, wb[kk].w, c2, 0, 0, 0);
            }
            if (m < pr.n2) {
#pragma unroll
                for (int r = 0; r < 16; ++r) {
                    const int row = row0 + (r & 3) + 8 * (r >> 2) + 4 * hh;
                    if (row < pr.R) C2[(size_t)row * pr.ldc2 + m] = c2[r];
                }
            }
#pragma unroll
            for (int kk = 0; kk < 4; ++kk) wb[kk] = wn[kk];
        }
    }
}

template <int SK, int AMODE, bool CHAIN = false, bool LN = false>
static int launch_gemm32(const GemmBatch &gb, int rmax, int nmax, hipStream_t st)
{
    const size_t lds = sizeof(float) * (SK * 4 * 32 * LDT + 32 + 64 * SK);
    if (lds > 64 * 1024)
        PTX_HIP(hipFuncSetAttribute(reinterpret_cast<const void *>(&k_gemm32<SK, AMODE, CHAIN, LN>),
                                    hipFuncAttributeMaxDynamicSharedMemorySize, (int)lds));
    hipLaunchKernelGGL((k_gemm32<SK, AMODE, CHAIN, LN>), dim3(cdiv(rmax, 32), cdiv(nmax, 32), gb.n), dim3(SK * 64), lds, st, gb);
    return PTX_OK;
}

static std::atomic<int> g_gemm128_min_tiles{256};
int gemm_policy(int min_tiles_128)
{
    return min_tiles_128 < 0 ? g_gemm128_min_tiles.load() : g_gemm128_min_tiles.exchange(min_tiles_128);
}

int launch_gemm(const GemmBatch &gb_in, hipStream_t st, int compute_dtype)
{
    GemmBatch gb = gb_in;
    gb.rotate = 0;
    PTX_REQUIRE(gb.n >= 1 && gb.n <= kMaxGroups, "gemm: %d groups", gb.n);
    int rmax = 0, nmax = 0, kmin = 1 << 30, kmax = 0;
    long tiles32 = 0;
    bool any_ln = false;
    for (int g = 0; g < gb.n; ++g) {
        const GemmProb &p = gb.p[g];
        PTX_REQUIRE((p.A || p.pg) && p.W && p.C, "gemm: null operand in group %d", g);
        PTX_REQUIRE((p.pg != nullptr) == (gb.p[0].pg != nullptr), "gemm: mixed A modes in one batch");
        PTX_REQUIRE(p.pg == nullptr || (p.pe && p.pml && p.ad && p.kg % BK == 0 && p.kg <= p.K && p.ldg % 4 == 0 &&
                                        p.gslab % 4 == 0 && p.lde % 4 == 0),
                    "gemm: bad pooled-A description in group %d", g);
        PTX_REQUIRE(p.R >= 1 && p.N >= 1 && p.K >= 4, "gemm: empty problem in group %d", g);
        PTX_REQUIRE(p.K % 4 == 0 && p.lda % 4 == 0 && p.ldw % 4 == 0,
                    "gemm: K=%d lda=%d ldw=%d must be multiples of 4", p.K, p.lda, p.ldw);
        PTX_REQUIRE(((reinterpret_cast<uintptr_t>(p.A) | reinterpret_cast<uintptr_t>(p.W) | reinterpret_cast<uintptr_t>(p.pg) |
                      reinterpret_cast<uintptr_t>(p.pe)) & 15) == 0,
                    "gemm: operands of group %d are not 16-byte aligned", g);
        PTX_REQUIRE(p.rs == nullptr || p.ad != nullptr, "gemm: row scale without addend");
        PTX_REQUIRE(p.lnp_in == nullptr || (p.ln_c && p.ln_parts >= 1 && p.ln_parts <= 16 && p.ln_C == 32 * p.ln_parts &&
                                            p.K == p.ln_C && p.pg == nullptr && p.bias == nullptr),
                    "gemm: bad LayerNorm-consumer description in group %d", g);
        any_ln = any_ln || p.lnp_in != nullptr;
        rmax = p.R > rmax ? p.R : rmax;
        nmax = p.N > nmax ? p.N : nmax;
        kmin = p.K < kmin ? p.K : kmin;
        kmax = p.K > kmax ? p.K : kmax;
        tiles32 += (long)cdiv(p.R, 32) * cdiv(p.N, 32);
    }
    if (gb.p[0].w2 != nullptr) {
        PTX_REQUIRE(gb.n == 1 && gb.p[0].pg == nullptr && gb.p[0].c2 && gb.p[0].n2 >= 1 && gb.p[0].chain_tiles >= 1 &&
                    gb.p[0].chain_tiles * 32 <= gb.p[0].N && gb.p[0].K >= 4 * BK && gb.p[0].lnp_out == nullptr && !any_ln,
                    "gemm: bad chained-product description");
        PTX_TRY((launch_gemm32<4, 0, true>(gb, rmax, nmax, st)));
        PTX_LAUNCHED("k_gemm");
        return PTX_OK;
    }
    constexpr int g64_min = 1024;
    long tiles128 = 0;
    for (int g = 0; g < gb.n; ++g) tiles128 += (long)cdiv(gb.p[g].R, 128) * cdiv(gb.p[g].N, 128);
    const int min128 = g_gemm128_min_tiles.load(std::memory_order_relaxed);
    const bool enough = tiles128 >= min128 && (min128 == 1 || 2 * tiles128 >= 3 * (long)min128 || kmin >= 512);
    const bool use128 = gb.p[0].pg == nullptr && kmin == kmax && kmin % 256 == 0 && kmin <= 4096 && min128 > 0 && enough;
    if (use128) {
        const dim3 grid(cdiv(rmax, 128), cdiv(nmax, 128), gb.n);
        const int nrep = kmin / (32 * PTX_G128_NM);
        if (compute_dtype == 1) {
            if (any_ln) hipLaunchKernelGGL((k_gemm128x<PTX_G128_NM, 1, true>), grid, dim3(256), 0, st, gb, nrep);
            else        hipLaunchKernelGGL((k_gemm128x<PTX_G128_NM, 1>), grid, dim3(256), 0, st, gb, nrep);
        } else {
            if (any_ln) hipLaunchKernelGGL((k_gemm128x<PTX_G128_NM, 3, true>), grid, dim3(256), 0, st, gb, nrep);
            else        hipLaunchKernelGGL((k_gemm128x<PTX_G128_NM, 3>), grid, dim3(256), 0, st, gb, nrep);
        }
        PTX_LAUNCHED("k_gemm128x");
        return PTX_OK;
    }
    if (compute_dtype == 1 && gb.p[0].pg == nullptr && kmin == kmax && kmin % 128 == 0 && kmin / 128 <= 8) {
        const dim3 grid(cdiv(rmax, 64), cdiv(nmax, 64), gb.n);
        const int nkg = kmin / 128;
        if (any_ln && nkg == 1) hipLaunchKernelGGL((k_gemm64x<1, 1, 1, true>), grid, dim3(256), 0, st, gb);
        else if (any_ln && nkg == 2) hipLaunchKernelGGL((k_gemm64x<2, 1, 1, true>), grid, dim3(256), 0, st, gb);
        else if (any_ln && nkg == 4) hipLaunchKernelGGL((k_gemm64x<4, 1, 1, true>), grid, dim3(256), 0, st, gb);
        else if (any_ln) { set_error("gemm: LayerNorm consumer with K=%d in bf16 mode", kmin); return PTX_EINVAL; }
        else if (nkg == 1) hipLaunchKernelGGL((k_gemm64x<1, 1, 1>), grid, dim3(256), 0, st, gb);
        else if (nkg == 2) hipLaunchKernelGGL((k_gemm64x<2, 1, 1>), grid, dim3(256), 0, st, gb);
        else if (nkg == 4) hipLaunchKernelGGL((k_gemm64x<4, 1, 1>), grid, dim3(256), 0, st, gb);
        else if (nkg == 8) hipLaunchKernelGGL((k_gemm64x<8, 1, 1>), grid, dim3(256), 0, st, gb);
        else if (nkg == 6) hipLaunchKernelGGL((k_gemm64x<2, 3, 1>), grid, dim3(256), 0, st, gb);
        else { set_error("gemm: K=%d in bf16 mode", kmin); return PTX_EINVAL; }
        PTX_LAUNCHED("k_gemm64x<bf16>");
        return PTX_OK;
    }
    if (gb.p[0].pg != nullptr) {
        PTX_TRY((launch_gemm32<4, 1>(gb, rmax, nmax, st)));
    } else if (tiles32 >= g64_min) {
        const dim3 grid(cdiv(rmax, 64), cdiv(nmax, 64), gb.n);
        const int nkg = (kmin == kmax && kmin % 128 == 0) ? kmin / 128 : 0;
        if (any_ln && nkg == 1) hipLaunchKernelGGL((k_gemm64x<1, 1, 3, true>), grid, dim3(256), 0, st, gb);
        else if (any_ln && nkg == 2) hipLaunchKernelGGL((k_gemm64x<2, 1, 3, true>), grid, dim3(256), 0, st, gb);
        else if (any_ln && nkg == 4) hipLaunchKernelGGL((k_gemm64x<4, 1, 3, true>), grid, dim3(256), 0, st, gb);
        else if (any_ln) hipLaunchKernelGGL(k_gemm64<true>, grid, dim3(256), 0, st, gb);
        else if (nkg == 1) hipLaunchKernelGGL((k_gemm64x<1, 1>), grid, dim3(256), 0, st, gb);
        else if (nkg == 2) hipLaunchKernelGGL((k_gemm64x<2, 1>), grid, dim3(256), 0, st, gb);
        else if (nkg == 4) hipLaunchKernelGGL((k_gemm64x<4, 1>), grid, dim3(256), 0, st, gb);
        else if (nkg == 8) hipLaunchKernelGGL((k_gemm64x<8, 1>), grid, dim3(256), 0, st, gb);
        else if (nkg == 6) hipLaunchKernelGGL((k_gemm64x<2, 3>), grid, dim3(256), 0, st, gb);
        else if (nkg == 12) hipLaunchKernelGGL((k_gemm64x<4, 3>), grid, dim3(256), 0, st, gb);
        else if (nkg == 16) hipLaunchKernelGGL((k_gemm64x<8, 2>), grid, dim3(256), 0, st, gb);
        else if (nkg == 32) hipLaunchKernelGGL((k_gemm64x<8, 4>), grid, dim3(256), 0, st, gb);
        else hipLaunchKernelGGL(k_gemm64<false>, grid, dim3(256), 0, st, gb);
    } else {
        const int nk = cdiv(kmin, BK);
        int sk = 1;
        while (sk < 4 && tiles32 * sk < 4096 && nk >= 4 * sk) sk *= 2;
        if (any_ln) {
            if (sk == 1) PTX_TRY((launch_gemm32<1, 0, false, true>(gb, rmax, nmax, st)));
            else if (sk == 2) PTX_TRY((launch_gemm32<2, 0, false, true>(gb, rmax, nmax, st)));
            else PTX_TRY((launch_gemm32<4, 0, false, true>(gb, rmax, nmax, st)));
        } else if (sk == 1) PTX_TRY((launch_gemm32<1, 0>(gb, rmax, nmax, st)));
        else if (sk == 2) PTX_TRY((launch_gemm32<2, 0>(gb, rmax, nmax, st)));
        else PTX_TRY((launch_gemm32<4, 0>(gb, rmax, nmax, st)));
    }
    PTX_LAUNCHED("k_gemm");
    return PTX_OK;
}

constexpr int kMaxPerLane = 8;

__device__ __forceinline__ void ln_row(const float *x, int C, float eps, float (&v)[kMaxPerLane],
                                       float &mean, float &rstd)
{
    const int lane = lane_id();
    float s = 0.0f;
#pragma unroll
    for (int q = 0; q < kMaxPerLane; ++q) {
        const int c = lane + 64 * q;
        v[q] = c < C ? x[c] : 0.0f;
        s += v[q];
    }
    mean = wave_sum(s) / (float)C;
    float var = 0.0f;
#pragma unroll
    for (int q = 0; q < kMaxPerLane; ++q) {
        const int c = lane + 64 * q;
        const float d = c < C ? v[q] - mean : 0.0f;
        var = fmaf(d, d, var);
    }
    rstd = 1.0f / sqrtf(wave_sum(var) / (float)C + eps);
}

__global__ __launch_bounds__(256) void k_ln_rows(LnBatch lb)
{
    const LnProb p = lb.p[blockIdx.y];
    const int row = __builtin_amdgcn_readfirstlane(blockIdx.x * 4 + (threadIdx.x >> 6));
    if (row >= p.R) return;
    float v[kMaxPerLane], mean, rstd;
    ln_row(p.x + (size_t)row * lb.C, lb.C, lb.eps, v, mean, rstd);
    const int lane = lane_id();
#pragma unroll
    for (int q = 0; q < kMaxPerLane; ++q) {
        const int c = lane + 64 * q;
        if (c < lb.C) {
            float y = (v[q] - mean) * rstd * p.w[c] + p.b[c];
            if (p.add) y += p.add[(size_t)(row % p.add_rows) * lb.C + c];
            p.y[(size_t)row * lb.C + c] = y;
        }
    }
}

int launch_ln_rows(const LnBatch &lb, hipStream_t st)
{
    PTX_REQUIRE(lb.C % 64 == 0 && lb.C <= 64 * kMaxPerLane, "layer norm: C=%d unsupported", lb.C);
    int rmax = 0;
    for (int g = 0; g < lb.n; ++g) rmax = lb.p[g].R > rmax ? lb.p[g].R : rmax;
    if (rmax == 0) return PTX_OK;
    hipLaunchKernelGGL(k_ln_rows, dim3(cdiv(rmax, 4), lb.n), dim3(256), 0, st, lb);
    PTX_LAUNCHED("k_ln_rows");
    return PTX_OK;
}

constexpr int kHeadRows = 4;

template <int Q>
__global__ __launch_bounds__(256) void k_heads(HeadBatch hb)
{
    const HeadProb p = hb.p[blockIdx.y];
    const int row0 = __builtin_amdgcn_readfirstlane((blockIdx.x * 4 + (threadIdx.x >> 6)) * kHeadRows);
    if (row0 >= p.R) return;
    const int lane = lane_id();
    constexpr int kMaxOut = 9;
    float hbias = 0.0f, bn_a = 0.0f, bn_b = 0.0f;
    if (lane < p.nout) { hbias = p.hb[lane]; bn_a = p.ab[lane]; bn_b = p.ab[p.nout + lane]; }
    float nw[Q], nb[Q], hwt[kMaxOut][Q];
#pragma unroll
    for (int q = 0; q < Q; ++q) { nw[q] = p.nw[lane + 64 * q]; nb[q] = p.nb[lane + 64 * q]; }
#pragma unroll
    for (int o = 0; o < kMaxOut; ++o)
#pragma unroll
        for (int q = 0; q < Q; ++q) hwt[o][q] = o < p.nout ? p.hw[(size_t)o * hb.C + lane + 64 * q] : 0.0f;
    float x[kHeadRows][Q];
#pragma unroll
    for (int r = 0; r < kHeadRows; ++r)
#pragma unroll
        for (int q = 0; q < Q; ++q)
            x[r][q] = row0 + r < p.R ? p.x[(size_t)(row0 + r) * hb.C + lane + 64 * q] : 0.0f;
#pragma unroll
    for (int r = 0; r < kHeadRows; ++r) {
        const int row = row0 + r;
        if (row >= p.R) break;
        float rsum = (x[r][0] + x[r][1]) + (x[r][2] + x[r][3]);
#pragma unroll
        for (int q = 4; q < Q; ++q) rsum += x[r][q];
        const float mean = wave_sum(rsum) / (float)hb.C;
        float var = 0.0f;
#pragma unroll
        for (int q = 0; q < Q; ++q) { const float d = x[r][q] - mean; var = fmaf(d, d, var); }
        const float rstd = 1.0f / sqrtf(wave_sum(var) / (float)hb.C + hb.eps);
        float v[Q];
#pragma unroll
        for (int q = 0; q < Q; ++q) {
            v[q] = (x[r][q] - mean) * rstd * nw[q] + nb[q];
            if (p.guide) p.guide[(size_t)row * hb.C + lane + 64 * q] = v[q];
        }
        float mine = 0.0f;
#pragma unroll
        for (int o = 0; o < kMaxOut; ++o) {
            if (o < p.nout) {
                float part = 0.0f;
#pragma unroll
                for (int q = 0; q < Q; ++q) part = fmaf(hwt[o][q], v[q], part);
                const float s = wave_sum(part);
                if (lane == o) mine = s;
            }
        }
        if (lane < p.nout) p.out[(size_t)row * p.nout + lane] = fmaf(mine + hbias, bn_a, bn_b);
    }
}

int launch_heads(const HeadBatch &hb, hipStream_t st)
{
    PTX_REQUIRE(hb.C == 256 || hb.C == 512, "heads: C=%d unsupported (256, 512)", hb.C);
    int rmax = 0;
    for (int g = 0; g < hb.n; ++g) {
        PTX_REQUIRE(hb.p[g].nout >= 1 && hb.p[g].nout <= 9, "heads: nout=%d", hb.p[g].nout);
        rmax = hb.p[g].R > rmax ? hb.p[g].R : rmax;
    }
    if (rmax == 0) return PTX_OK;
    const dim3 grid(cdiv(rmax, 4 * kHeadRows), hb.n);
    if (hb.C == 256) hipLaunchKernelGGL(k_heads<4>, grid, dim3(256), 0, st, hb);
    else             hipLaunchKernelGGL(k_heads<8>, grid, dim3(256), 0, st, hb);
    PTX_LAUNCHED("k_heads");
    return PTX_OK;
}

}
```

proxytransformation_amd/csrc/imgpool.hip:

```cpp
#include <cstdlib>
#include <hip/hip_ext.h>

#include "common.h"
#include "imgstore.h"

namespace ptx {

typedef __bf16 bf16x8 __attribute__((ext_vector_type(8)));

constexpr int kPoolHeads = 8;
constexpr int kPoolNtImages = 4096;
constexpr int kPoolWPad = 544;
constexpr int kPoolPPad = 136;

typedef _Float16 f16x8 __attribute__((ext_vector_type(8)));

template <int DT>
__device__ __forceinline__ void split3(float x, unsigned short &q1, unsigned short &q2, unsigned short &q3)
{
    if (DT == 1) {
        const unsigned int u1 = __float_as_uint(x) & 0xffff0000u;
        const float r1 = x - __uint_as_float(u1);
        const unsigned int u2 = __float_as_uint(r1) & 0xffff0000u;
        const float r2 = r1 - __uint_as_float(u2);
        q1 = (unsigned short)(u1 >> 16); q2 = (unsigned short)(u2 >> 16); q3 = (unsigned short)(__float_as_uint(r2) >> 16);
    } else {
        const _Float16 h1 = (_Float16)x;
        const float r1 = x - (float)h1;
        const _Float16 h2 = (_Float16)r1;
        const float r2 = r1 - (float)h2;
        const _Float16 h3 = (_Float16)r2;
        q1 = __builtin_bit_cast(unsigned short, h1); q2 = __builtin_bit_cast(unsigned short, h2);
        q3 = __builtin_bit_cast(unsigned short, h3);
    }
}

template <int DT>
__device__ __forceinline__ f32x4 mfma16(const u32x4 &a, const u32x4 &b, const f32x4 &c)
{
    if (DT == 1) return __builtin_amdgcn_mfma_f32_16x16x32_bf16(__builtin_bit_cast(bf16x8, a), __builtin_bit_cast(bf16x8, b), c, 0, 0, 0);
    return __builtin_amdgcn_mfma_f32_16x16x32_f16(__builtin_bit_cast(f16x8, a), __builtin_bit_cast(f16x8, b), c, 0, 0, 0);
}

__device__ __forceinline__ int pow2_scale_exp(float amax)
{
    const int e = (int)((__float_as_uint(amax) >> 23) & 0xffu) - 127;
    return (amax > 0.0f && e > -100 && e < 100) ? 13 - e : 0;
}
__device__ __forceinline__ float pow2f(int k) { return __uint_as_float((unsigned int)(127 + k) << 23); }
constexpr float kPoolEScale = 16384.0f;

__device__ __forceinline__ u32x4 shr_elems(const u32x4 &v, int k)
{
    const int ws = k >> 1;
    unsigned int w[8] = {v[0], v[1], v[2], v[3], 0u, 0u, 0u, 0u};
    u32x4 o;
#pragma unroll
    for (int q = 0; q < 4; ++q) {
        unsigned int lo = 0u, hi = 0u;
#pragma unroll
        for (int s = 0; s < 4; ++s) {
            if (ws == s) { lo = w[q + s]; hi = w[q + s + 1]; }
        }
        o[q] = (k & 1) ? ((lo >> 16) | (hi << 16)) : lo;
    }
    return o;
}

struct PoolArgs {
    const unsigned short *img; const float *we, *qkv0;
    int nimg, in_dim, hw, C, KT1, EW; float scale;
    float *Gs;
    float *E;
    float *ML;
};

template <int DT, bool NT>
__global__ __launch_bounds__(512) void k_img_pool(PoolArgs a)
{
    constexpr int heads = kPoolHeads;
    extern __shared__ __attribute__((aligned(16))) unsigned char smem[];
    float *partial = reinterpret_cast<float *>(smem);
    unsigned short *wpart = reinterpret_cast<unsigned short *>(partial + 8 * heads * 128);
    unsigned short *parts = wpart + 24 * kPoolWPad;
    const int in_dim = a.in_dim, hw = a.hw;
    const int xcd = blockIdx.x & 7, slot = blockIdx.x >> 3;
    const int T = slot & 1, imr = (slot >> 1) * 8 + xcd;
    if (imr >= a.nimg) return;
    const int im = a.nimg - 1 - imr;
    const int slab = im * 2 + T;
    const int tid = threadIdx.x, lane = lane_id();
    const int wid = __builtin_amdgcn_readfirstlane(tid >> 6);
    const int n = lane & 15, kq = lane >> 4;
    const float *wim = a.we + (size_t)im * heads * a.KT1;
    const unsigned short *f = a.img + (size_t)im * in_dim * hw;
    const int px = 128 * T + 8 * n;
    const bool full = px + 8 <= hw;
    const int cw = 64 * wid;
    float wv[heads];
#pragma unroll
    for (int h = 0; h < heads; ++h) wv[h] = wim[(size_t)h * a.KT1 + tid];
    u32x4 L[2][8];
    const bool tensor_end = im == a.nimg - 1 && cw + 64 == in_dim;
#pragma unroll
    for (int kb = 0; kb < 2; ++kb) {
        const unsigned short *r = f + (size_t)(cw + 32 * kb + 8 * kq) * hw + px;
#pragma unroll
        for (int i = 0; i < 8; ++i) {
            if (kb == 1 && i == 7 && tensor_end) {
                const bool lastrow = kq == 3 && !full;
                const int back = lastrow ? px + 8 - hw : 0;
                const int bk = back > 8 ? px - (hw - 8) : back;
                u32x4 v = __builtin_nontemporal_load(reinterpret_cast<const u4u2 *>(r + (size_t)i * hw - bk));
                L[kb][i] = lastrow ? (back >= 8 ? u32x4{0u, 0u, 0u, 0u} : shr_elems(v, back)) : v;
            } else {
                L[kb][i] = __builtin_nontemporal_load(reinterpret_cast<const u4u2 *>(r + (size_t)i * hw));
            }
        }
    }
    float ev[2];
#pragma unroll
    for (int u = 0; u < 2; ++u) {
        const int p = 128 * T + lane + 64 * u;
        ev[u] = p < hw ? wim[(size_t)wid * a.KT1 + in_dim + 1 + p] : 0.0f;
    }
    float sq = 0.0f, sk = 0.0f;
    if (T == 0) {
        const int hd = a.C / heads;
        const float *qv = a.qkv0 + (size_t)im * 3 * a.C + wid * hd;
        if (lane < hd) { sq = qv[lane]; sk = qv[a.C + lane]; }
    }
    {
        const int c = tid;
#pragma unroll
        for (int h = 0; h < heads; ++h) {
            if (DT == 2) {
                const int k = pow2_scale_exp(wave_max(fabsf(wv[h])));
                wv[h] *= pow2f(k);
                if (lane == 0) *reinterpret_cast<float *>(wpart + (size_t)h * kPoolWPad + in_dim + 2 * wid) = pow2f(-k);
            }
            unsigned short q1, q2, q3;
            split3<DT>(wv[h], q1, q2, q3);
            wpart[(size_t)h * kPoolWPad + c] = q1;
            wpart[(size_t)(8 + h) * kPoolWPad + c] = q2;
            wpart[(size_t)(16 + h) * kPoolWPad + c] = q3;
        }
    }
    __syncthreads();

    {
        f32x4 acc[8];
#pragma unroll
        for (int j = 0; j < 8; ++j) acc[j] = f32x4{0.f, 0.f, 0.f, 0.f};
        const bool lo = n < heads;
#pragma unroll
        for (int kb = 0; kb < 2; ++kb) {
            u32x4 af[3];
#pragma unroll
            for (int pt = 0; pt < 3; ++pt) {
                u32x4 t = *reinterpret_cast<const u32x4 *>(wpart + (size_t)(pt * 8 + (n & 7)) * kPoolWPad + cw + 32 * kb + 8 * kq);
                if (!lo) t = u32x4{0u, 0u, 0u, 0u};
                af[pt] = t;
            }
#pragma unroll
            for (int j = 0; j < 8; ++j) {
                const unsigned int sel = (j & 1) ? 0x07060302u : 0x05040100u;
                u32x4 b;
#pragma unroll
                for (int qd = 0; qd < 4; ++qd) b[qd] = __builtin_amdgcn_perm(L[kb][2 * qd + 1][j >> 1], L[kb][2 * qd][j >> 1], sel);
#pragma unroll
                for (int pt = 0; pt < 3; ++pt) acc[j] = mfma16<DT>(af[pt], b, acc[j]);
            }
        }
        if (kq < 2) {
#pragma unroll
            for (int r = 0; r < 4; ++r) {
                float us = 1.0f;
                if (DT == 2) us = *reinterpret_cast<const float *>(wpart + (size_t)(4 * kq + r) * kPoolWPad + in_dim + 2 * wid);
                float *d = partial + ((size_t)wid * heads + 4 * kq + r) * 128 + 8 * n;
                *reinterpret_cast<float4 *>(d) = make_float4(acc[0][r] * us, acc[1][r] * us, acc[2][r] * us, acc[3][r] * us);
                *reinterpret_cast<float4 *>(d + 4) = make_float4(acc[4][r] * us, acc[5][r] * us, acc[6][r] * us, acc[7][r] * us);
            }
        }
    }
    __syncthreads();

    {
        const int h = wid;
        float e[2], mloc = -INFINITY, sv[2];
#pragma unroll
        for (int u = 0; u < 2; ++u) {
            const int p = lane + 64 * u;
            float s = 0.0f;
#pragma unroll
            for (int w = 0; w < 8; ++w) s += partial[((size_t)w * heads + h) * 128 + p];
            sv[u] = 128 * T + p < hw ? s + ev[u] : -INFINITY;
            mloc = fmaxf(mloc, sv[u]);
        }
        const float m = wave_max(mloc);
#pragma unroll
        for (int u = 0; u < 2; ++u) e[u] = 128 * T + lane + 64 * u < hw ? expf(sv[u] - m) : 0.0f;
        const float l = wave_sum(e[0] + e[1]);
        float *erow = a.E + ((size_t)im * heads + h) * a.EW;
        const float s0 = T == 0 ? wave_sum(sq * sk) * a.scale : 0.0f;
        if (lane == 0) {
            float *ml = a.ML + ((size_t)im * heads + h) * 5;
            ml[2 * T] = m;
            ml[2 * T + 1] = l;
            if (T == 0) { ml[4] = s0; erow[0] = 1.0f; }
        }
#pragma unroll
        for (int u = 0; u < 2; ++u) {
            const int p = lane + 64 * u;
            const int t = 1 + 128 * T + p;
            if (t <= hw || (T == (hw > 128 ? 1 : 0) && t < a.EW)) erow[t] = t <= hw ? e[u] : 0.0f;
            unsigned short q1, q2, q3;
            split3<DT>(DT == 2 ? e[u] * kPoolEScale : e[u], q1, q2, q3);
            parts[(size_t)h * kPoolPPad + p] = q1;
            parts[(size_t)(8 + h) * kPoolPPad + p] = q2;
            parts[(size_t)(16 + h) * kPoolPPad + p] = q3;
        }
    }
    __syncthreads();

    {
        const int ps = n & 3, hh = n >> 2;
        const int src = ((ps + 4 * kq) + 16 * (n >> 2)) * 4;
        u32x4 bfr[2][3];
#pragma unroll
        for (int hg = 0; hg < 2; ++hg)
#pragma unroll
            for (int pt = 0; pt < 3; ++pt)
                bfr[hg][pt] = *reinterpret_cast<const u32x4 *>(parts + (size_t)(pt * 8 + 4 * hg + hh) * kPoolPPad + 8 * (ps + 4 * kq));
        const unsigned m0 = ps == 0 ? ~0u : 0u, m1 = ps == 1 ? ~0u : 0u, m2 = ps == 2 ? ~0u : 0u, m3 = ps == 3 ? ~0u : 0u;
        float *G = partial;
#pragma unroll
        for (int kb = 0; kb < 2; ++kb) {
#pragma unroll
            for (int i = 0; i < 8; ++i)
#pragma unroll
                for (int d = 0; d < 4; ++d) L[kb][i][d] = (unsigned int)__builtin_amdgcn_ds_bpermute(src, (int)L[kb][i][d]);
            float xs[2][8];
#pragma unroll
            for (int ig = 0; ig < 4; ++ig) {
                f32x4 c[2][2];
#pragma unroll
                for (int ii = 0; ii < 2; ++ii)
#pragma unroll
                    for (int hg = 0; hg < 2; ++hg) c[ii][hg] = f32x4{0.f, 0.f, 0.f, 0.f};
#pragma unroll
                for (int pt = 0; pt < 3; ++pt)
#pragma unroll
                    for (int ii = 0; ii < 2; ++ii)
#pragma unroll
                        for (int hg = 0; hg < 2; ++hg) c[ii][hg] = mfma16<DT>(L[kb][2 * ig + ii], bfr[hg][pt], c[ii][hg]);
#pragma unroll
                for (int ii = 0; ii < 2; ++ii)
#pragma unroll
                    for (int hg = 0; hg < 2; ++hg) {
                        const f32x4 &acc = c[ii][hg];
                        float x = __uint_as_float((__float_as_uint(acc[0]) & m0) | (__float_as_uint(acc[1]) & m1) |
                                                  (__float_as_uint(acc[2]) & m2) | (__float_as_uint(acc[3]) & m3));
                        x += __int_as_float(__builtin_amdgcn_mov_dpp(__float_as_int(x), 0xB1, 0xF, 0xF, true));
                        x += __int_as_float(__builtin_amdgcn_mov_dpp(__float_as_int(x), 0x4E, 0xF, 0xF, true));
                        xs[hg][2 * ig + ii] = DT == 2 ? x * (1.0f / kPoolEScale) : x;
                    }
            }
            if (ps == 0) {
#pragma unroll
                for (int hg = 0; hg < 2; ++hg)
#pragma unroll
                    for (int q = 0; q < 2; ++q)
                        *reinterpret_cast<f32x4 *>(G + (size_t)(4 * hg + hh) * in_dim + cw + 32 * kb + 8 * kq + 4 * q) =
                            f32x4{xs[hg][4 * q], xs[hg][4 * q + 1], xs[hg][4 * q + 2], xs[hg][4 * q + 3]};
            }
        }
    }
    __syncthreads();
    {
        const float *G = partial;
        float *dst = a.Gs + (size_t)slab * heads * in_dim;
        for (int i = tid * 4; i < heads * in_dim; i += 512 * 4)
        {
            const f32x4 v = *reinterpret_cast<const f32x4 *>(G + i);
            if (NT) asm volatile("global_store_dwordx4 %0, %1, off sc1 nt" :: "v"(dst + i), "v"(v) : "memory");
            else    asm volatile("global_store_dwordx4 %0, %1, off sc1" :: "v"(dst + i), "v"(v) : "memory");
        }
    }
}

bool img_pool_supported(int dt, int in_dim, int hw, int heads)
{
    return (dt == 1 || dt == 2) && heads == kPoolHeads && in_dim == 512 && hw > 128 && hw <= 255;
}

size_t img_pool_bytes(int nimg, int in_dim, int EW)
{
    return (size_t)nimg * kPoolHeads * (2 * (size_t)in_dim + EW + 8) * sizeof(float);
}

void img_pool_layout(float *scratch, int nimg, int in_dim, int EW, float **Gs, float **E, float **ML)
{
    *Gs = scratch;
    *E = *Gs + (size_t)nimg * 2 * kPoolHeads * in_dim;
    *ML = *E + (size_t)nimg * kPoolHeads * EW;
}

int launch_img_pool(const void *img, int dt, const float *we, const float *qkv0, int nimg, int in_dim, int hw, int C,
                    int KT1, int EW, float scale, float *Gs, float *E, float *ML, hipStream_t st)
{
    PTX_REQUIRE(EW % 4 == 0 && EW >= hw + 1 && hw > 128 && hw <= 255, "img pool: hw=%d EW=%d", hw, EW);
    PoolArgs pa{static_cast<const unsigned short *>(img), we, qkv0, nimg, in_dim, hw, C, KT1, EW, scale, Gs, E, ML};
    const size_t lds = sizeof(float) * 8 * kPoolHeads * 128 + sizeof(unsigned short) * 24 * (kPoolWPad + kPoolPPad);
    PTX_REQUIRE(lds <= 64 * 1024, "img pool: %zu B of LDS", lds);
    static const int nt_env = getenv("PTX_POOL_NT") ? atoi(getenv("PTX_POOL_NT")) : -1;
    const bool nt = nt_env >= 0 ? nt_env != 0 : nimg >= kPoolNtImages;
    const dim3 grid(cdiv(nimg, 8) * 16);
    hipEvent_t ta = nullptr, tb = nullptr;
    (void)timing_ext_take(&ta, &tb);
    if (dt == 1) { if (nt) hipExtLaunchKernelGGL((k_img_pool<1, true>), grid, dim3(512), lds, st, ta, tb, 0, pa); else hipExtLaunchKernelGGL((k_img_pool<1, false>), grid, dim3(512), lds, st, ta, tb, 0, pa); }
    else         { if (nt) hipExtLaunchKernelGGL((k_img_pool<2, true>), grid, dim3(512), lds, st, ta, tb, 0, pa); else hipExtLaunchKernelGGL((k_img_pool<2, false>), grid, dim3(512), lds, st, ta, tb, 0, pa); }
    PTX_LAUNCHED("k_img_pool");
    return PTX_OK;
}

}
```

proxytransformation_amd/csrc/imgpool32.hip:

```cpp
#include <hip/hip_ext.h>

#include "common.h"

namespace ptx {

typedef float p32_f4u __attribute__((ext_vector_type(4), aligned(4)));
typedef float p32_f4 __attribute__((ext_vector_type(4)));

constexpr int kP32Heads = 8;
constexpr int kP32Tile = 32;
constexpr int kP32Tiles = 128 / kP32Tile;
constexpr int kP32TRow = 36;

struct Pool32Args {
    const float *img; const float *we, *qkv0;
    int nimg, in_dim, hw, C, KT1, EW; float scale;
    float *Gs, *E, *ML;
};

__global__ __launch_bounds__(512) __attribute__((amdgpu_waves_per_eu(4, 4))) void k_img_pool32(Pool32Args a)
{
    constexpr int heads = kP32Heads, TP = kP32Tile;
    extern __shared__ __attribute__((aligned(16))) float p32_sm[];
    float *W_s = p32_sm;
    float *S_s = W_s + 512 * heads;
    float *E_s = S_s + 8 * heads * TP;
    float *sc_s = E_s + heads * TP;
    float *T_s = sc_s + 16;
    const int in_dim = a.in_dim, hw = a.hw;
    const int xcd = blockIdx.x & 7, slot = blockIdx.x >> 3;
    const int H = slot & 1, imr = (slot >> 1) * 8 + xcd;
    if (imr >= a.nimg) return;
    const int im = a.nimg - 1 - imr;
    const int tid = threadIdx.x, lane = lane_id();
    const int wid = __builtin_amdgcn_readfirstlane(tid >> 6);
    const int n = lane & 7, kq = lane >> 3;
    const int mr = lane & 15, mk = lane >> 4;
    const float *wim = a.we + (size_t)im * heads * a.KT1;
    const float *f = a.img + (size_t)im * in_dim * hw;
    float *T_w = T_s + (size_t)wid * (16 * kP32TRow);
    float wv[heads];
#pragma unroll
    for (int h = 0; h < heads; ++h) wv[h] = wim[(size_t)h * a.KT1 + tid];
    float ev[kP32Tiles];
#pragma unroll
    for (int t = 0; t < kP32Tiles; ++t) {
        const int p = 128 * H + TP * t + (lane & (TP - 1));
        ev[t] = p < hw ? wim[(size_t)wid * a.KT1 + in_dim + 1 + p] : 0.0f;
    }
    float sq = 0.0f, sk = 0.0f;
    if (H == 0) {
        const int hd = a.C / heads;
        const float *qv = a.qkv0 + (size_t)im * 3 * a.C + wid * hd;
        if (lane < hd) { sq = qv[lane]; sk = qv[a.C + lane]; }
    }
    const char *fb = reinterpret_cast<const char *>(f);
    const unsigned row_off = (unsigned)(64 * wid + kq) * (unsigned)hw * 4u, row_step = 8u * (unsigned)hw * 4u;
    const bool tensor_end = im == a.nimg - 1 && wid == 7 && kq == 7;
    {
        *reinterpret_cast<p32_f4 *>(W_s + tid * heads) = p32_f4{wv[0], wv[1], wv[2], wv[3]};
        *reinterpret_cast<p32_f4 *>(W_s + tid * heads + 4) = p32_f4{wv[4], wv[5], wv[6], wv[7]};
        if (tid < 16) sc_s[tid] = 0.0f;
    }
    p32_f4 D[4];
#pragma unroll
    for (int q = 0; q < 4; ++q) D[q] = p32_f4{0.f, 0.f, 0.f, 0.f};
    float m_run = -INFINITY, l_run = 0.0f, e_t[kP32Tiles];
#pragma unroll
    for (int t = 0; t < kP32Tiles; ++t) e_t[t] = 0.0f;

#pragma unroll
    for (int t = 0; t < kP32Tiles; ++t) {
        const int px0 = 128 * H + TP * t;
        p32_f4u L[8];
        {
            const int p = px0 + 4 * n;
            const int pc = p < hw ? p : 0;
            const unsigned off0 = row_off + (unsigned)pc * 4u;
#pragma unroll
            for (int i = 0; i < 8; ++i) {
                const float *rowp = reinterpret_cast<const float *>(fb + (off0 + (unsigned)i * row_step)) - pc;
                if (i == 7 && tensor_end && pc + 4 > hw) {
                    const p32_f4u v = *reinterpret_cast<const p32_f4u *>(rowp + hw - 4);
                    const int back = pc + 4 - hw;
                    L[i] = back == 1 ? p32_f4u{v[1], v[2], v[3], 0.f} : back == 2 ? p32_f4u{v[2], v[3], 0.f, 0.f} : p32_f4u{v[3], 0.f, 0.f, 0.f};
                } else {
                    L[i] = __builtin_nontemporal_load(reinterpret_cast<const p32_f4u *>(rowp + pc));
                }
            }
        }
        __syncthreads();
#pragma unroll
        for (int hb = 0; hb < heads; hb += 4) {
            float acc[4][4];
#pragma unroll
            for (int h = 0; h < 4; ++h) { acc[h][0] = acc[h][1] = acc[h][2] = acc[h][3] = 0.0f; }
#pragma unroll
            for (int i = 0; i < 8; ++i) {
                const p32_f4 w4 = *reinterpret_cast<const p32_f4 *>(W_s + (64 * wid + 8 * i + kq) * heads + hb);
                const p32_f4u v = L[i];
#pragma unroll
                for (int h = 0; h < 4; ++h) {
                    acc[h][0] = fmaf(w4[h], v[0], acc[h][0]); acc[h][1] = fmaf(w4[h], v[1], acc[h][1]);
                    acc[h][2] = fmaf(w4[h], v[2], acc[h][2]); acc[h][3] = fmaf(w4[h], v[3], acc[h][3]);
                }
            }
#pragma unroll
            for (int h = 0; h < 4; ++h)
#pragma unroll
                for (int c = 0; c < 4; ++c) {
                    float x = acc[h][c];
                    x += PTX_ROR_F(x, 8);
                    x += __shfl_xor(x, 16, 64);
                    x += __shfl_xor(x, 32, 64);
                    acc[h][c] = x;
                }
            if (kq == 0) {
#pragma unroll
                for (int h = 0; h < 4; ++h)
                    *reinterpret_cast<p32_f4 *>(S_s + ((size_t)wid * heads + hb + h) * TP + 4 * n) = p32_f4{acc[h][0], acc[h][1], acc[h][2], acc[h][3]};
            }
            __builtin_amdgcn_sched_barrier(0);
        }
        __syncthreads();
        {
            const int h = wid, pl = lane & (TP - 1);
            float s = 0.0f;
#pragma unroll
            for (int w = 0; w < 8; ++w) s += S_s[((size_t)w * heads + h) * TP + pl];
            const bool valid = lane < TP && px0 + pl < hw;
            const float sv = valid ? s + ev[t] : -INFINITY;
            const float m_new = fmaxf(m_run, wave_max(sv));
            const float resc = expf(m_run - m_new);
            const float e = valid ? expf(sv - m_new) : 0.0f;
            l_run = l_run * resc + wave_sum(e);
            m_run = m_new;
#pragma unroll
            for (int u = 0; u < kP32Tiles; ++u) e_t[u] = u < t ? e_t[u] * resc : (u == t ? e : 0.0f);
            if (lane < TP) E_s[h * TP + lane] = e;
            if (lane == 0) sc_s[h] = resc;
            if (t == kP32Tiles - 1) {
                float *erow = a.E + ((size_t)im * heads + h) * a.EW;
#pragma unroll
                for (int u = 0; u < kP32Tiles; ++u) {
                    const int tok = 1 + 128 * H + TP * u + lane;
                    if (lane < TP && tok < a.EW) erow[tok] = e_t[u];
                }
                const float s0 = H == 0 ? wave_sum(sq * sk) * a.scale : 0.0f;
                if (lane == 0) {
                    float *ml = a.ML + ((size_t)im * heads + h) * 5;
                    ml[2 * H] = m_run; ml[2 * H + 1] = l_run;
                    if (H == 0) { ml[4] = s0; erow[0] = 1.0f; }
                }
            }
        }
        __syncthreads();
        {
            const float resc = sc_s[mr];
#pragma unroll
            for (int q = 0; q < 4; ++q) { D[q][0] *= resc; D[q][1] *= resc; D[q][2] *= resc; D[q][3] *= resc; }
#pragma unroll
            for (int q = 0; q < 4; ++q) {
#pragma unroll
                for (int ii = 0; ii < 2; ++ii)
                    *reinterpret_cast<p32_f4 *>(T_w + (8 * ii + kq) * kP32TRow + 4 * n) = p32_f4{L[2 * q + ii][0], L[2 * q + ii][1], L[2 * q + ii][2], L[2 * q + ii][3]};
                __builtin_amdgcn_wave_barrier();
                __builtin_amdgcn_fence(__ATOMIC_RELEASE, "wavefront");
#pragma unroll
                for (int pb = 0; pb < TP / 16; ++pb) {
                    const p32_f4 a4 = *reinterpret_cast<const p32_f4 *>(T_w + mr * kP32TRow + 16 * pb + 4 * mk);
                    p32_f4 e4 = *reinterpret_cast<const p32_f4 *>(E_s + (mr & 7) * TP + 16 * pb + 4 * mk);
                    if (mr >= heads) e4 = p32_f4{0.f, 0.f, 0.f, 0.f};
#pragma unroll
                    for (int c = 0; c < 4; ++c) D[q] = __builtin_amdgcn_mfma_f32_16x16x4f32(a4[c], e4[c], D[q], 0, 0, 0);
                }
                __builtin_amdgcn_wave_barrier();
                __builtin_amdgcn_fence(__ATOMIC_ACQUIRE, "wavefront");
            }
        }
    }
    __syncthreads();
    float *G = W_s;
    if (mr < heads) {
#pragma unroll
        for (int q = 0; q < 4; ++q)
            *reinterpret_cast<p32_f4 *>(G + (size_t)mr * in_dim + 64 * wid + 16 * q + 4 * mk) = D[q];
    }
    __syncthreads();
    {
        float *dst = a.Gs + (size_t)(im * 2 + H) * heads * in_dim;
        for (int i = tid * 4; i < heads * in_dim; i += 512 * 4) {
            const p32_f4 v = *reinterpret_cast<const p32_f4 *>(G + i);
            asm volatile("global_store_dwordx4 %0, %1, off sc1" :: "v"(dst + i), "v"(v) : "memory");
        }
    }
}

bool img_pool32_supported(int dt, int in_dim, int hw, int heads)
{
    return dt == 0 && heads == kP32Heads && in_dim == 512 && hw > 128 && hw <= 255;
}

int launch_img_pool32(const float *img, const float *we, const float *qkv0, int nimg, int in_dim, int hw, int C, int KT1, int EW,
                      float scale, float *Gs, float *E, float *ML, hipStream_t st)
{
    PTX_REQUIRE(EW % 4 == 0 && EW >= hw + 1 && hw > 128 && hw <= 255 && in_dim == 512, "img pool (fp32): hw=%d EW=%d in_dim=%d", hw, EW, in_dim);
    PTX_REQUIRE((reinterpret_cast<uintptr_t>(img) & 15) == 0, "img_feat must be 16-byte aligned");
    Pool32Args pa{img, we, qkv0, nimg, in_dim, hw, C, KT1, EW, scale, Gs, E, ML};
    const size_t lds = sizeof(float) * (512 * kP32Heads + 8 * kP32Heads * kP32Tile + kP32Heads * kP32Tile + 16 + 8 * 16 * kP32TRow);
    const dim3 grid(cdiv(nimg, 8) * 16);
    hipEvent_t ta = nullptr, tb = nullptr;
    (void)timing_ext_take(&ta, &tb);
    hipExtLaunchKernelGGL(k_img_pool32, grid, dim3(512), lds, st, ta, tb, 0, pa);
    PTX_LAUNCHED("k_img_pool32");
    return PTX_OK;
}

}
```

proxytransformation_amd/csrc/imgproxy.hip:

```cpp
#include "common.h"
#include "imgstore.h"

namespace ptx {

__global__ __launch_bounds__(256) void k_img_mean(const float *__restrict__ img, int ngroups,
                                                  int hw, float *__restrict__ fm, uint32_t *gate, uint32_t gate_seq)
{
    mean_prologue(gate, gate_seq);
    const int blk = blockIdx.x;
    const int lane = lane_id();
    const int g = __builtin_amdgcn_readfirstlane(blk * 4 + (threadIdx.x >> 6));
    if (g >= ngroups) return;
    const f32x4 *src = reinterpret_cast<const f32x4 *>(img + (size_t)g * 4 * hw);
    float s0 = 0.f, s1 = 0.f, s2 = 0.f, s3 = 0.f;
    for (int j = lane; j < hw; j += 64) {
        const f32x4 v = __builtin_nontemporal_load(src + j);
        const float vv[4] = {v.x, v.y, v.z, v.w};
#pragma unroll
        for (int c = 0; c < 4; ++c) {
            const int e = 4 * j + c;
            const int row = (e >= hw) + (e >= 2 * hw) + (e >= 3 * hw);
            s0 += row == 0 ? vv[c] : 0.f; s1 += row == 1 ? vv[c] : 0.f;
            s2 += row == 2 ? vv[c] : 0.f; s3 += row == 3 ? vv[c] : 0.f;
        }
    }
    s0 = wave_sum(s0); s1 = wave_sum(s1); s2 = wave_sum(s2); s3 = wave_sum(s3);
    if (lane == 0) {
        const float inv = 1.0f / (float)hw;
        *reinterpret_cast<float4 *>(fm + (size_t)g * 4) = make_float4(s0 * inv, s1 * inv, s2 * inv, s3 * inv);
    }
}

struct RowLanes {
    int half, j, poff, cfirst; bool act;
    __device__ RowLanes(int lane, int hw) {
        half = lane >> 5; j = lane & 31;
        const int nv8 = hw >> 3, tail = hw & 7;
        const bool edge = tail != 0 && j == nv8;
        act = j < nv8 || edge;
        poff = edge ? hw - 8 : 8 * j;
        cfirst = edge ? 8 - tail : 0;
    }
};

constexpr int kMeanGroups = 4;

template <int DT>
__global__ __launch_bounds__(256) void k_img_mean16(const unsigned short *__restrict__ img, int ngroups,
                                                    int hw, float *__restrict__ fm, uint32_t *gate, uint32_t gate_seq)
{
    mean_prologue(gate, gate_seq);
    const int blk = blockIdx.x;
    const int lane = lane_id();
    const int g0 = __builtin_amdgcn_readfirstlane((blk * 4 + (threadIdx.x >> 6)) * kMeanGroups);
    if (g0 >= ngroups) return;
    const RowLanes rl(lane, hw);
    u32x4 d[kMeanGroups][4];
#pragma unroll
    for (int gg = 0; gg < kMeanGroups; ++gg) {
        const int g = min(g0 + gg, ngroups - 1);
        const unsigned short *base = img + (size_t)g * 8 * hw;
#pragma unroll
        for (int u = 0; u < 4; ++u)
            d[gg][u] = __builtin_nontemporal_load(reinterpret_cast<const u4u2 *>(base + (size_t)(2 * u + rl.half) * hw + (rl.act ? rl.poff : 0)));
    }
    const float inv = 1.0f / (float)hw;
#pragma unroll
    for (int gg = 0; gg < kMeanGroups; ++gg) {
        float out = 0.0f;
#pragma unroll
        for (int u = 0; u < 4; ++u) {
            float v[8], s = 0.0f;
            ImgStore<DT>::widen8(d[gg][u], v);
#pragma unroll
            for (int c = 0; c < 8; ++c) s += (rl.act && c >= rl.cfirst) ? v[c] : 0.0f;
            s += PTX_ROR_F(s, 8); s += PTX_ROR_F(s, 4); s += PTX_ROR_F(s, 2); s += PTX_ROR_F(s, 1);
            const float lo = PTX_LANE_F(s, 0) + PTX_LANE_F(s, 16), hi = PTX_LANE_F(s, 32) + PTX_LANE_F(s, 48);
            if (lane == 2 * u) out = lo * inv;
            if (lane == 2 * u + 1) out = hi * inv;
        }
        if (lane < 8 && g0 + gg < ngroups) fm[(size_t)(g0 + gg) * 8 + lane] = out;
    }
}

int launch_img_mean(const void *img, int dt, int nimg, int in_dim, int hw, float *fm, hipStream_t st, uint32_t *gate, uint32_t gate_seq)
{
    if (dt == 0) {
        PTX_REQUIRE(in_dim % 4 == 0, "img mean: in_dim=%d must be a multiple of 4", in_dim);
        PTX_REQUIRE((reinterpret_cast<uintptr_t>(img) & 15) == 0, "img_feat must be 16-byte aligned");
        const int ngroups = nimg * (in_dim / 4);
        hipLaunchKernelGGL(k_img_mean, dim3(cdiv(ngroups, 4)), dim3(256), 0, st, static_cast<const float *>(img), ngroups, hw, fm,
                           gate, gate_seq);
        PTX_LAUNCHED("k_img_mean");
        return PTX_OK;
    }
    PTX_REQUIRE(in_dim % 8 == 0, "img mean: in_dim=%d must be a multiple of 8", in_dim);
    PTX_REQUIRE(hw >= 8 && (hw >> 3) + ((hw & 7) ? 1 : 0) <= 32, "half-precision image features: hw=%d (supported: 8..255)", hw);
    const int ngroups = nimg * (in_dim / 8);
    const unsigned short *p = static_cast<const unsigned short *>(img);
    const dim3 grid(cdiv(ngroups, 4 * kMeanGroups));
    if (dt == 1) hipLaunchKernelGGL((k_img_mean16<1>), grid, dim3(256), 0, st, p, ngroups, hw, fm, gate, gate_seq);
    else         hipLaunchKernelGGL((k_img_mean16<2>), grid, dim3(256), 0, st, p, ngroups, hw, fm, gate, gate_seq);
    PTX_LAUNCHED("k_img_mean16");
    return PTX_OK;
}

constexpr int kMaxHeads = 16;

constexpr int kScoreWaves = 8;

template <int HEADS, int DT>
__global__ __launch_bounds__(kScoreWaves * 64) void k_img_scores(
    const typename ImgStore<DT>::elem *__restrict__ img, const float *__restrict__ we, const float *__restrict__ qkv0,
    int in_dim, int hw, int C, int KT1, int KT2p, float scale, float *__restrict__ gbuf)
{
    using St = ImgStore<DT>;
    constexpr int heads = HEADS, NW = kScoreWaves;
    extern __shared__ __attribute__((aligned(16))) float sm[];
    float *red = sm;
    float *S = sm + (NW / 2) * heads * 256;
    const int im = gridDim.x - 1 - blockIdx.x, tid = threadIdx.x, lane = lane_id();
    const int wid = __builtin_amdgcn_readfirstlane(tid >> 6);
    const float *wim = we + (size_t)im * heads * KT1;
    const typename St::elem *f = img + (size_t)im * in_dim * hw;
    const int nv4 = hw >> 2, tail = hw & 3;
    const bool edge = tail != 0 && lane == nv4;
    const bool vec = lane < nv4 || edge;
    const int poff = edge ? hw - 4 : 4 * lane;
    const int cfirst = edge ? 4 - tail : 0;
    float acc[HEADS][4];
#pragma unroll
    for (int h = 0; h < HEADS; ++h) { acc[h][0] = acc[h][1] = acc[h][2] = acc[h][3] = 0.0f; }
    const int cper = in_dim / NW, cbeg = wid * cper;
    float wreg[HEADS];
    for (int h0 = wid; h0 < heads; h0 += NW) {
        const int hd = C / heads;
        const float *q = qkv0 + (size_t)im * 3 * C + h0 * hd;
        const float qk = lane < hd ? q[lane] * q[C + lane] : 0.0f;
        const float s0 = wave_sum(qk);
        if (lane == 0) S[h0 * (hw + 1)] = s0 * scale;
    }
    constexpr int UNR = 8;
    const typename St::elem *fl = f + (vec ? poff : 0);
    for (int c0 = 0; c0 < cper; c0 += 64) {
    const int cn = min(64, cper - c0);
#pragma unroll
    for (int h = 0; h < HEADS; ++h) wreg[h] = lane < cn ? wim[(size_t)h * KT1 + cbeg + c0 + lane] : 0.0f;
    for (int cc = 0; cc < cn; cc += UNR) {
        typename St::px4 t[UNR];
#pragma unroll
        for (int u = 0; u < UNR; ++u) t[u] = St::load4_nt(fl + (size_t)(cbeg + c0 + cc + u) * hw);
        __builtin_amdgcn_sched_barrier(0);
#pragma unroll
        for (int u = 0; u < UNR; ++u) {
            float v[4];
            St::widen4(t[u], v);
#pragma unroll
            for (int h = 0; h < HEADS; ++h) {
                const float wv = __int_as_float(__builtin_amdgcn_readlane(__float_as_int(wreg[h]), cc + u));
                acc[h][0] = fmaf(wv, v[0], acc[h][0]); acc[h][1] = fmaf(wv, v[1], acc[h][1]);
                acc[h][2] = fmaf(wv, v[2], acc[h][2]); acc[h][3] = fmaf(wv, v[3], acc[h][3]);
            }
        }
    }
    }
    float ev[HEADS][4];
#pragma unroll
    for (int h = 0; h < HEADS; ++h)
#pragma unroll
        for (int c = 0; c < 4; ++c)
            ev[h][c] = (wid == 0 && vec && c >= cfirst) ? wim[(size_t)h * KT1 + in_dim + 1 + poff + c] : 0.0f;
#pragma unroll
    for (int half = NW / 2; half >= 1; half >>= 1) {
        if (wid >= half && wid < 2 * half) {
#pragma unroll
            for (int h = 0; h < HEADS; ++h)
                *reinterpret_cast<float4 *>(red + ((size_t)(wid - half) * heads + h) * 256 + 4 * lane) =
                    make_float4(acc[h][0], acc[h][1], acc[h][2], acc[h][3]);
        }
        __syncthreads();
        if (wid < half) {
#pragma unroll
            for (int h = 0; h < HEADS; ++h) {
                const float4 t = *reinterpret_cast<const float4 *>(red + ((size_t)wid * heads + h) * 256 + 4 * lane);
                acc[h][0] += t.x; acc[h][1] += t.y; acc[h][2] += t.z; acc[h][3] += t.w;
            }
        }
        __syncthreads();
    }
    if (wid == 0 && vec) {
#pragma unroll
        for (int h = 0; h < HEADS; ++h) {
            float *d = S + h * (hw + 1) + 1 + poff;
#pragma unroll
            for (int c = 0; c < 4; ++c)
                if (c >= cfirst) d[c] = acc[h][c] + ev[h][c];
        }
    }
    __syncthreads();
    for (int h = wid; h < heads; h += NW) {
        const float *sh = S + h * (hw + 1);
        float mx = -INFINITY;
        for (int i = lane; i <= hw; i += 64) mx = fmaxf(mx, sh[i]);
        mx = wave_max(mx);
        float sum = 0.0f;
        for (int i = lane; i <= hw; i += 64) sum += expf(sh[i] - mx);
        sum = wave_sum(sum);
        const float inv = 1.0f / sum;
        float *dst = gbuf + ((size_t)im * heads + h) * KT2p + in_dim;
        for (int i = lane; i < KT2p - in_dim; i += 64) dst[i] = i <= hw ? expf(sh[i] - mx) * inv : 0.0f;
    }
}

int launch_img_scores(const void *img, int dt, const float *we, const float *qkv0, int nimg, int in_dim,
                      int hw, int heads, int C, int KT1, int KT2p, float scale, float *gbuf,
                      hipStream_t st)
{
    PTX_REQUIRE((heads == 4 || heads == 8 || heads == 16) && in_dim % (8 * kScoreWaves) == 0 && in_dim / kScoreWaves <= 256,
                "img scores: heads=%d in_dim=%d unsupported", heads, in_dim);
    PTX_REQUIRE(hw >= 4 && (hw >> 2) + ((hw & 3) ? 1 : 0) <= 64, "img scores: hw=%d (supported: 4..256 pixels)", hw);
    const size_t lds = sizeof(float) * ((size_t)(kScoreWaves / 2) * heads * 256 + (size_t)heads * (hw + 1));
    PTX_REQUIRE(lds <= 160 * 1024, "img scores: %zu B of LDS", lds);
#define PTX_SCORES(H_, DT_)                                                                                                         \
    do {                                                                                                                          \
        if (lds > 64 * 1024)                                                                                                      \
            PTX_HIP(hipFuncSetAttribute(reinterpret_cast<const void *>(&k_img_scores<H_, DT_>), hipFuncAttributeMaxDynamicSharedMemorySize, (int)lds)); \
        hipLaunchKernelGGL((k_img_scores<H_, DT_>), dim3(nimg), dim3(kScoreWaves * 64), lds, st,                                    \
                           static_cast<const ImgStore<DT_>::elem *>(img), we, qkv0, in_dim, hw, C, KT1, KT2p, scale, gbuf);         \
    } while (0)
#define PTX_SCORES_DT(DT_)                                                                                                          \
    do { if (heads == 4) PTX_SCORES(4, DT_); else if (heads == 8) PTX_SCORES(8, DT_); else PTX_SCORES(16, DT_); } while (0)
    if (dt == 0) PTX_SCORES_DT(0); else if (dt == 1) PTX_SCORES_DT(1); else PTX_SCORES_DT(2);
#undef PTX_SCORES_DT
#undef PTX_SCORES
    PTX_LAUNCHED("k_img_scores");
    return PTX_OK;
}

constexpr int kGatherCh = 64;

template <int DT>
__global__ __launch_bounds__(256) void k_img_gather(const typename ImgStore<DT>::elem *__restrict__ img, int in_dim, int hw,
                                                    int heads, int KT2p, float *__restrict__ gbuf)
{
    using St = ImgStore<DT>;
    extern __shared__ __attribute__((aligned(16))) float sm[];
    const int hwp = (hw + 3) & ~3;
    float *a_s = sm;
    const int chunks = in_dim / kGatherCh;
    const int im = blockIdx.x / chunks, c0 = (blockIdx.x - im * chunks) * kGatherCh;
    const int tid = threadIdx.x, lane = lane_id(), wid = tid >> 6;
    const int ci = lane & 15, kq = lane >> 4;
    const int cb = c0 + wid * 16;
    const typename St::elem *row = img + ((size_t)im * in_dim + cb + ci) * hw;
    const bool live = ci < heads;
    const float *arow = a_s + (size_t)(live ? ci : 0) * hwp;
    const int nkb = hw >> 5;
    constexpr int PRE = 4;
    typename St::px8 pf[PRE];
#pragma unroll
    for (int kb = 0; kb < PRE; ++kb) pf[kb] = St::load8(row, 32 * min(kb, nkb - 1), 8 * kq);
    {
        constexpr int NR = 16;
        float av[NR];
#pragma unroll
        for (int r = 0; r < NR; ++r) {
            const int i = tid + 256 * r, h = i / hwp, p = i - h * hwp;
            av[r] = (i < heads * hwp && p < hw) ? gbuf[((size_t)im * heads + h) * KT2p + in_dim + 1 + p] : 0.0f;
        }
#pragma unroll
        for (int r = 0; r < NR; ++r) {
            const int i = tid + 256 * r;
            if (i < heads * hwp) a_s[i] = av[r];
        }
    }
    __syncthreads();
    f32x4 acc = {0.f, 0.f, 0.f, 0.f};
    auto step = [&](int kb, const typename St::px8 &d) {
        const int p0 = 32 * kb + 8 * kq;
        float fv[8];
        St::widen8(d, fv);
        float4 b0 = *reinterpret_cast<const float4 *>(arow + p0);
        float4 b1 = *reinterpret_cast<const float4 *>(arow + p0 + 4);
        if (!live) { b0 = make_float4(0.f, 0.f, 0.f, 0.f); b1 = b0; }
        acc = __builtin_amdgcn_mfma_f32_16x16x4f32(fv[0], b0.x, acc, 0, 0, 0);
        acc = __builtin_amdgcn_mfma_f32_16x16x4f32(fv[1], b0.y, acc, 0, 0, 0);
        acc = __builtin_amdgcn_mfma_f32_16x16x4f32(fv[2], b0.z, acc, 0, 0, 0);
        acc = __builtin_amdgcn_mfma_f32_16x16x4f32(fv[3], b0.w, acc, 0, 0, 0);
        acc = __builtin_amdgcn_mfma_f32_16x16x4f32(fv[4], b1.x, acc, 0, 0, 0);
        acc = __builtin_amdgcn_mfma_f32_16x16x4f32(fv[5], b1.y, acc, 0, 0, 0);
        acc = __builtin_amdgcn_mfma_f32_16x16x4f32(fv[6], b1.z, acc, 0, 0, 0);
        acc = __builtin_amdgcn_mfma_f32_16x16x4f32(fv[7], b1.w, acc, 0, 0, 0);
    };
#pragma unroll
    for (int kb = 0; kb < PRE; ++kb)
        if (kb < nkb) step(kb, pf[kb]);
#pragma unroll 3
    for (int kb = PRE; kb < nkb; ++kb) step(kb, St::load8(row, 32 * kb, 8 * kq));
    for (int pp = 32 * nkb; pp < hw; pp += 4) {
        const int p = pp + kq;
        const float fa = p < hw ? img_load<DT>(row, p) : 0.0f;
        const float ba = (p < hw && live) ? arow[p] : 0.0f;
        acc = __builtin_amdgcn_mfma_f32_16x16x4f32(fa, ba, acc, 0, 0, 0);
    }
    if (live) {
        float *dst = gbuf + ((size_t)im * heads + ci) * KT2p + cb + 4 * kq;
        *reinterpret_cast<float4 *>(dst) = make_float4(acc[0], acc[1], acc[2], acc[3]);
    }
}

int launch_img_gather(const void *img, int dt, int nimg, int in_dim, int hw, int heads, int KT2p,
                      float *gbuf, hipStream_t st)
{
    PTX_REQUIRE(in_dim % kGatherCh == 0 && heads <= kMaxHeads, "img gather: in_dim=%d heads=%d", in_dim, heads);
    PTX_REQUIRE(hw <= 256, "img gather: hw=%d (max 256 pixels)", hw);
    const int hwp = (hw + 3) & ~3;
    const size_t lds = sizeof(float) * (size_t)heads * hwp;
    PTX_REQUIRE(lds <= 64 * 1024, "img gather: %zu B of LDS", lds);
    const dim3 grid(nimg * (in_dim / kGatherCh));
#define PTX_GATHER(DT_) \
    hipLaunchKernelGGL(k_img_gather<DT_>, grid, dim3(256), lds, st, static_cast<const ImgStore<DT_>::elem *>(img), in_dim, hw, heads, KT2p, gbuf)
    if (dt == 0) PTX_GATHER(0); else if (dt == 1) PTX_GATHER(1); else PTX_GATHER(2);
#undef PTX_GATHER
    PTX_LAUNCHED("k_img_gather");
    return PTX_OK;
}

}
```

proxytransformation_amd/csrc/prep.hip:

```cpp
#include "common.h"

namespace ptx {

__global__ void k_prep_bn(const float *w, const float *b, const float *mean, const float *var,
                          int n, float eps, float *ab)
{
    const int i = blockIdx.x * blockDim.x + threadIdx.x;
    if (i >= n) return;
    const float alpha = w[i] / sqrtf(var[i] + eps);
    ab[i] = alpha;
    ab[n + i] = b[i] - mean[i] * alpha;
}

__global__ void k_prep_posbias(const float *pb, const float *pc, const float *pr, int Mk, int s, int C,
                               float *out)
{
    const int i = blockIdx.x * blockDim.x + threadIdx.x;
    if (i >= Mk * C) return;
    const int j = i / C, yx = i - j * C, y = yx / s, x = yx - y * s;
    const float sc = 4.0f / (float)s;
    float sy = sc * ((float)y + 0.5f) - 0.5f; if (sy < 0.f) sy = 0.f;
    float sx = sc * ((float)x + 0.5f) - 0.5f; if (sx < 0.f) sx = 0.f;
    const int y0 = (int)sy, x0 = (int)sx;
    const int y1 = y0 + (y0 < 3 ? 1 : 0), x1 = x0 + (x0 < 3 ? 1 : 0);
    const float ly1 = sy - (float)y0, ly0 = 1.f - ly1, lx1 = sx - (float)x0, lx0 = 1.f - lx1;
    const float *p = pb + (size_t)j * 16;
    const float v = ly0 * (lx0 * p[y0 * 4 + x0] + lx1 * p[y0 * 4 + x1]) +
                    ly1 * (lx0 * p[y1 * 4 + x0] + lx1 * p[y1 * 4 + x1]);
    out[i] = v + (pc[(size_t)j * s + y] + pr[(size_t)j * s + x]);
}

__global__ void k_prep_w3(const float *qw, const float *kw, const float *vw, const float *qb,
                          const float *cw, const float *cb, const float *pos, int C, int in_dim,
                          float *w3, float *b3)
{
    const int i = blockIdx.x * blockDim.x + threadIdx.x;
    if (i >= 3 * C * (in_dim + 1)) return;
    const int n = i / (in_dim + 1), c = i - n * (in_dim + 1);
    const int part = n / C, r = n - part * C;
    const float *wrow = (part == 0 ? qw : (part == 1 ? kw : vw)) + (size_t)r * C;
    float s = 0.0f;
    if (c < in_dim) {
        for (int j = 0; j < C; ++j) s = fmaf(wrow[j], cw[(size_t)j * in_dim + c], s);
        w3[(size_t)n * in_dim + c] = s;
    } else {
        for (int j = 0; j < C; ++j) s = fmaf(wrow[j], cb[j] + pos[j], s);
        b3[n] = s + (part == 0 ? qb[r] : 0.0f);
    }
}

__global__ void k_prep_t1(const float *kw, const float *cw, const float *cb, const float *pos, int C,
                          int in_dim, int hw, int heads, float scale, float *t1)
{
    const int hd = C / heads, KT1 = in_dim + hw + 1;
    const int i = blockIdx.x * blockDim.x + threadIdx.x;
    if (i >= heads * KT1 * hd) return;
    const int h = i / (KT1 * hd), rem = i - h * KT1 * hd, t = rem / hd, d = rem - t * hd;
    const float *wk = kw + (size_t)(h * hd + d) * C;
    float s = 0.0f;
    if (t < in_dim) {
        for (int j = 0; j < C; ++j) s = fmaf(wk[j], cw[(size_t)j * in_dim + t], s);
    } else if (t > in_dim) {
        const float *pi = pos + (size_t)(t - in_dim) * C;
        for (int j = 0; j < C; ++j) s = fmaf(wk[j], cb[j] + pi[j], s);
    }
    t1[i] = s * scale;
}

__global__ void k_prep_t2(const float *vw, const float *cw, const float *cb, const float *pos, int C,
                          int in_dim, int hw, int heads, int KT2p, float *t2)
{
    const int hd = C / heads;
    const int i = blockIdx.x * blockDim.x + threadIdx.x;
    if (i >= heads * hd * KT2p) return;
    const int h = i / (hd * KT2p), rem = i - h * hd * KT2p, d = rem / KT2p, t = rem - d * KT2p;
    const float *wv = vw + (size_t)(h * hd + d) * C;
    float s = 0.0f;
    if (t < in_dim) {
        for (int j = 0; j < C; ++j) s = fmaf(wv[j], cw[(size_t)j * in_dim + t], s);
    } else if (t > in_dim && t <= in_dim + hw) {
        const float *pi = pos + (size_t)(t - in_dim) * C;
        for (int j = 0; j < C; ++j) s = fmaf(wv[j], cb[j] + pi[j], s);
    }
    t2[i] = s;
}

__global__ void k_prep_lnfold(const float *W, const float *gamma, const float *beta, const float *bias, int N, int K,
                              float *Wg, float *cv)
{
    const int n = blockIdx.x * (blockDim.x >> 6) + (threadIdx.x >> 6);
    if (n >= N) return;
    const int lane = threadIdx.x & 63;
    float c1 = 0.0f;
    for (int k = lane; k < K; k += 64) {
        const float wv = W[(size_t)n * K + k];
        Wg[(size_t)n * K + k] = wv * gamma[k];
        c1 = fmaf(wv, beta[k], c1);
    }
    c1 = wave_sum(c1);
    if (lane == 0) cv[n] = c1 + (bias ? bias[n] : 0.0f);
}

int launch_prep_lnfold(const float *W, const float *gamma, const float *beta, const float *bias, int N, int K, float *Wg,
                       float *cv, hipStream_t st)
{
    hipLaunchKernelGGL(k_prep_lnfold, dim3(cdiv(N, 4)), dim3(256), 0, st, W, gamma, beta, bias, N, K, Wg, cv);
    PTX_LAUNCHED("k_prep_lnfold");
    return PTX_OK;
}

int run_prepare(const PtxShape &s, const PtxWeights &w, float *prep, hipStream_t st)
{
    const PrepLayout P = prep_layout(s);
    const int C = s.C, T = 256;
    hipLaunchKernelGGL(k_prep_bn, dim3(1), dim3(T), 0, st, w.offset.bn_w, w.offset.bn_b,
                       w.offset.bn_mean, w.offset.bn_var, kSlotHidden, s.bn_eps, prep + P.off_ab);
    hipLaunchKernelGGL(k_prep_bn, dim3(cdiv(C, T)), dim3(T), 0, st, w.encoder.bn_w, w.encoder.bn_b,
                       w.encoder.bn_mean, w.encoder.bn_var, C, s.bn_eps, prep + P.enc_ab);
    hipLaunchKernelGGL(k_prep_bn, dim3(1), dim3(T), 0, st, w.text_trans_norm.w, w.text_trans_norm.b,
                       w.text_trans_norm.mean, w.text_trans_norm.var, 3, s.bn_eps, prep + P.ttn_ab);
    hipLaunchKernelGGL(k_prep_bn, dim3(1), dim3(T), 0, st, w.img_trans_norm.w, w.img_trans_norm.b,
                       w.img_trans_norm.mean, w.img_trans_norm.var, 9, s.bn_eps, prep + P.itn_ab);
    PTX_LAUNCHED("k_prep_bn");
    int sd = 1;
    while (sd * sd < C) ++sd;
    const int nb = s.Mk * C;
    hipLaunchKernelGGL(k_prep_posbias, dim3(cdiv(nb, T)), dim3(T), 0, st, w.text.pb_bias, w.text.pc_bias,
                       w.text.pr_bias, s.Mk, sd, C, prep + P.posb_t);
    hipLaunchKernelGGL(k_prep_posbias, dim3(cdiv(nb, T)), dim3(T), 0, st, w.img.pb_bias, w.img.pc_bias,
                       w.img.pr_bias, s.Mk, sd, C, prep + P.posb_i);
    PTX_LAUNCHED("k_prep_posbias");
    hipLaunchKernelGGL(k_prep_w3, dim3(cdiv(3 * C * (s.in_dim + 1), T)), dim3(T), 0, st, w.q_w, w.k_w, w.v_w,
                       w.q_b, w.cm_w, w.cm_b, w.pos, C, s.in_dim, prep + P.w3, prep + P.b3);
    PTX_LAUNCHED("k_prep_w3");
    const float scale = (float)(1.0 / sqrt((double)P.hd));
    hipLaunchKernelGGL(k_prep_t1, dim3(cdiv(s.heads * P.KT1 * P.hd, T)), dim3(T), 0, st, w.k_w, w.cm_w,
                       w.cm_b, w.pos, C, s.in_dim, s.hw, s.heads, scale, prep + P.t1);
    PTX_LAUNCHED("k_prep_t1");
    hipLaunchKernelGGL(k_prep_t2, dim3(cdiv(s.heads * P.hd * P.KT2p, T)), dim3(T), 0, st, w.v_w, w.cm_w,
                       w.cm_b, w.pos, C, s.in_dim, s.hw, s.heads, P.KT2p, prep + P.t2);
    PTX_LAUNCHED("k_prep_t2");
    PTX_TRY(launch_prep_lnfold(w.img.pp_w, w.norm_img_w, w.norm_img_b, w.img.pp_b, C, C, prep + P.ppg_w, prep + P.ppg_c, st));
    const PtxBlock *blk[2] = {&w.text, &w.img};
    for (int i = 0; i < 2; ++i)
        PTX_TRY(launch_prep_lnfold(blk[i]->fc1_w, blk[i]->norm2_w, blk[i]->norm2_b, blk[i]->fc1_b, s.hidden, C,
                                   prep + P.fc1g_w[i], prep + P.fc1g_c[i], st));
    {
        GemmBatch g{}; g.n = 2;
        for (int i = 0; i < 2; ++i)
            g.p[i] = GemmProb{prep + (i == 0 ? P.posb_t : P.posb_i), blk[i]->qkv_w, prep + P.qkvb[i], blk[i]->qkv_b, nullptr, nullptr, nullptr,
                              s.Mk, 3 * C, C, C, C, 3 * C, 0, 0, 0, EPI_NONE};
        PTX_TRY(launch_gemm(g, st));
    }
    if (mlp_fused_supported(C, s.hidden, 1, 0))
        for (int i = 0; i < 2; ++i) {
            PTX_TRY(launch_prep_planes(prep + P.fc1g_w[i], s.hidden, C, prep + P.mlp_w1p[i], st));
            PTX_TRY(launch_prep_planes(blk[i]->fc2_w, C, s.hidden, prep + P.mlp_w2p[i], st));
        }
    return PTX_OK;
}

}
```

scratch/pool_variants.py:

```python
import os, re, subprocess
R = os.path.dirname(os.path.dirname(os.path.abspath(__file__)))
C = os.path.join(R, "proxytransformation_amd", "csrc")
src = open(os.path.join(C, "imgpool.hip")).read()
i_k = src.index("void k_img_pool(PoolArgs a)")
i_e = src.index("bool img_pool_supported(int dt")
head, k, tail = src[:i_k], src[i_k:i_e], src[i_e:]

def variant(name):
    t = k.replace("void k_img_pool(PoolArgs a)", "__attribute__((amdgpu_waves_per_eu(4, 4))) void k_img_pool(PoolArgs a)", 1)
    if name in ("nostore", "loadsonly", "nostore_nostage3"):
        t = t.replace('asm volatile("global_store_dwordx4 %0, %1, off sc1" :: "v"(dst + i), "v"(v) : "memory");',
                      'if (v[0] == 1.2345e-30f) asm volatile("global_store_dwordx4 %0, %1, off sc1" :: "v"(dst + i), "v"(v) : "memory");')
        t = t.replace("erow[t] = t <= hw ? e[u] : 0.0f;", "if (e[u] == 1.2345e-30f) erow[t] = t <= hw ? e[u] : 0.0f;")
        t = t.replace("            ml[2 * T] = m;\n            ml[2 * T + 1] = l;\n            if (T == 0) { ml[4] = s0; erow[0] = 1.0f; }",
                      "            if (m == 1.2345e-30f) { ml[2 * T] = m; ml[2 * T + 1] = l; if (T == 0) { ml[4] = s0; erow[0] = 1.0f; } }")
    if name in ("nostage3", "loadsonly", "nostore_nostage3"):
        a = t.index("    // ---- 3. weighted sums over the tile's pixels from the registers.")
        b = t.index("    __syncthreads();\n    {\n        const float *G = partial;")
        keep = "    { unsigned x_ = 0;\n"
        keep += "".join("      x_ ^= L[%d][%d][0] ^ L[%d][%d][3];\n" % (kb, i, kb, i) for kb in range(2) for i in range(8))
        keep += "      if (x_ == 0x12345678u) partial[threadIdx.x] = 1.0f; }\n"
        t = t[:a] + keep + t[b:]
    if name == "s12_notrail":
        t = variant("nostore_nostage3")
        t = t.replace("ev[u] = p < hw ? wim[(size_t)wid * a.KT1 + in_dim + 1 + p] : 0.0f;", "ev[u] = p < hw ? 0.25f * (float)p : 0.0f;")
        t = t.replace("if (lane < hd) { sq = qv[lane]; sk = qv[a.C + lane]; }", "if (lane < hd) { sq = (float)lane; sk = 0.5f; (void)qv; }")
        return t
    if name == "s1only":
        a = t.index("    // ---- 2. wave = head: sum the eight channel slices")
        b = t.index("    __syncthreads();\n    {\n        const float *G = partial;")
        keep = "    { unsigned x_ = 0;\n"
        keep += "".join("      x_ ^= L[%d][%d][0] ^ L[%d][%d][3];\n" % (kb, i, kb, i) for kb in range(2) for i in range(8))
        keep += "      if (x_ == 0x12345678u) partial[threadIdx.x] = 1.0f; }\n"
        t = t[:a] + keep + t[b:]
        t = t.replace('asm volatile("global_store_dwordx4 %0, %1, off sc1" :: "v"(dst + i), "v"(v) : "memory");',
                      'if (v[0] == 1.2345e-30f) asm volatile("global_store_dwordx4 %0, %1, off sc1" :: "v"(dst + i), "v"(v) : "memory");')
    if name == "loadsonly":
        a = t.index("    // ---- 1. scores of this wave's 64 channels")
        b = t.index("    { unsigned x_ = 0;")
        t = t[:a] + t[b:]
    return t

out = os.path.join(R, "scratch", "lab"); os.makedirs(out, exist_ok=True)
flags = "--offload-arch=gfx950 -O3 -std=c++17 -fPIC -ffp-contract=off -fno-fast-math -Wno-unused-function -Wno-unused-variable -Wno-unused-but-set-variable".split()
objs = [os.path.join(C, f) for f in sorted(os.listdir(C)) if f.endswith(".o") and f != "imgpool.o"]
import sys
for name in (sys.argv[1:] or ["nostore", "nostage3", "loadsonly", "nostore_nostage3"]):
    lab = os.path.join(C, "_imgpool_%s.hip" % name)
    open(lab, "w").write(head + variant(name) + tail)
    try:
        subprocess.check_call(["/opt/rocm/bin/hipcc"] + flags + ["-c", lab, "-o", os.path.join(out, "imgpool_%s.o" % name)])
    finally:
        os.remove(lab)
    subprocess.check_call(["/opt/rocm/bin/hipcc", "--offload-arch=gfx950", "-shared", "-fPIC", "-o", os.path.join(out, "lib_%s.so" % name),
                           os.path.join(out, "imgpool_%s.o" % name)] + objs)
    print("built", name)
```

Measured before the change: 19020 scenes/s.

## Pad image key-projection width to 32 and slim the chained GEMM kernel

The per-head width of the fused key projection (KT1s) is padded to a multiple of 32, so the chained second GEMM covers full 32-column tiles and rows of the we buffer stay aligned. The prep kernel zero-fills the padding columns. The chained GEMM variant now uses a single LDS buffer instead of double buffering, drops the residual, activation and row-scale epilogue paths, and sets a minimum-occupancy launch bound so more blocks can stay resident. The trade is lost load/compute overlap from the removed double buffer, plus a little extra padded work and memory.

After: 18300 scenes/s. -3.8%, worse.

```diff
diff --git a/proxytransformation_amd/csrc/api.hip b/proxytransformation_amd/csrc/api.hip
--- a/proxytransformation_amd/csrc/api.hip
+++ b/proxytransformation_amd/csrc/api.hip
@@ -119,12 +119,14 @@
     auto take = [&](size_t n) { size_t r = o; o += align_up(n, 64); return r; };
     P.hd = s.C / s.heads;
     P.KT1 = s.in_dim + s.hw + 1;
-    P.KT2p = (int)align_up((size_t)s.in_dim + s.hw + 1, 4);
+    P.EW = (int)align_up((size_t)s.hw + 1, 32);
+    P.KT1s = s.in_dim + P.EW;
+    P.KT2p = s.in_dim + P.EW;
     P.off_ab = take(2 * kSlotHidden); P.enc_ab = take(2 * (size_t)s.C);
     P.ttn_ab = take(6); P.itn_ab = take(18);
     P.posb_t = take((size_t)s.Mk * s.C); P.posb_i = take((size_t)s.Mk * s.C);
     P.w3 = take((size_t)3 * s.C * s.in_dim); P.b3 = take((size_t)3 * s.C);
-    P.t1 = take((size_t)s.heads * P.KT1 * P.hd);
+    P.t1 = take((size_t)s.heads * P.KT1s * P.hd);
     P.t2 = take((size_t)s.heads * P.hd * P.KT2p);
     P.ppg_w = take((size_t)s.C * s.C); P.ppg_c = take(s.C);
     for (int i = 0; i < 2; ++i) {
@@ -197,9 +199,9 @@
     L.pp_all = take(em * B * Mt * C * 4); L.order_e = take(em * B * Mt * 4);
     for (int i = 0; i < 2; ++i) { L.xln_all[i] = take(em * B * Mt * C * 4); L.g_all[i] = take(em * B * Mt * 3 * C * 4); }
     L.fm = take(nimg * s.in_dim * 4); L.qkv0 = take(nimg * 3 * C * 4);
-    L.we = take(nimg * s.heads * (size_t)P.KT1 * 4);
+    L.we = take(nimg * s.heads * (size_t)P.KT1s * 4);
     {
-        const size_t pool_b = img_pool_bytes((int)nimg, s.in_dim, P.KT2p - s.in_dim), gbuf_b = nimg * s.heads * (size_t)P.KT2p * 4;
+        const size_t pool_b = img_pool_bytes((int)nimg, s.in_dim, P.EW), gbuf_b = nimg * s.heads * (size_t)P.KT2p * 4;
         L.pool = L.gbuf = take(pool_b > gbuf_b ? pool_b : gbuf_b);
     }
     L.obuf = take(nimg * C * 4); L.cbuf = take(nimg * C * 4); L.img_proxy = take(nimg * C * 4);
@@ -407,13 +409,13 @@
     const WsLayout L = ws_layout(s);
     const int C = s.C, hd = P.hd, nall = s.B * s.V, nimg = ni < 0 ? nall : ni;
     float *fm = at<float>(ws, L.fm) + (size_t)i0 * s.in_dim, *qkv0 = at<float>(ws, L.qkv0) + (size_t)i0 * 3 * C;
-    float *we = at<float>(ws, L.we) + (size_t)i0 * s.heads * P.KT1, *gbuf = at<float>(ws, L.gbuf) + (size_t)i0 * s.heads * P.KT2p;
+    float *we = at<float>(ws, L.we) + (size_t)i0 * s.heads * P.KT1s, *gbuf = at<float>(ws, L.gbuf) + (size_t)i0 * s.heads * P.KT2p;
     float *obuf = at<float>(ws, L.obuf) + (size_t)i0 * C, *cbuf = at<float>(ws, L.cbuf) + (size_t)i0 * C;
     if (img_proxy) img_proxy += (size_t)i0 * C;
     const int dt = s.img_dtype;
     img = static_cast<const char *>(img) + (size_t)i0 * s.in_dim * s.hw * (dt == 0 ? 4 : 2);
     float *Gs = nullptr, *E = nullptr, *ML = nullptr;
-    const int EW = P.KT2p - s.in_dim;
+    const int EW = P.EW;
     const bool pooled32 = img_pool32_supported(dt, s.in_dim, s.hw, s.heads);
     const bool pooled = pooled32 || img_pool_supported(dt, s.in_dim, s.hw, s.heads);
     if (pooled) {
@@ -428,8 +430,8 @@
         g.p[0] = GemmProb{fm, prep + P.w3, qkv0, prep + P.b3, nullptr, nullptr, nullptr,
                           nimg, 3 * C, s.in_dim, s.in_dim, s.in_dim, 3 * C, 0, 0, 0, EPI_NONE};
         if (chained) {
-            g.p[0].w2 = prep + P.t1; g.p[0].c2 = we; g.p[0].n2 = P.KT1; g.p[0].ldc2 = s.heads * P.KT1;
-            g.p[0].chain_tiles = s.heads; g.p[0].w2_stride = (long)P.KT1 * hd; g.p[0].c2_stride = P.KT1;
+            g.p[0].w2 = prep + P.t1; g.p[0].c2 = we; g.p[0].n2 = P.KT1s; g.p[0].ldc2 = s.heads * P.KT1s;
+            g.p[0].chain_tiles = s.heads; g.p[0].w2_stride = (long)P.KT1s * hd; g.p[0].c2_stride = P.KT1s;
         }
         PTX_TIMED(KID_IMG_QKV0, st, launch_gemm(g, st));
     }
@@ -437,20 +439,20 @@
         for (int h0 = 0; h0 < s.heads; h0 += kMaxGroups) {
             GemmBatch g{}; g.n = std::min(kMaxGroups, s.heads - h0);
             for (int h = h0; h < h0 + g.n; ++h)
-                g.p[h - h0] = GemmProb{qkv0 + h * hd, prep + P.t1 + (size_t)h * P.KT1 * hd, we + (size_t)h * P.KT1,
-                                       nullptr, nullptr, nullptr, nullptr, nimg, P.KT1, hd, 3 * C, hd,
-                                       s.heads * P.KT1, 0, 0, 0, EPI_NONE};
+                g.p[h - h0] = GemmProb{qkv0 + h * hd, prep + P.t1 + (size_t)h * P.KT1s * hd, we + (size_t)h * P.KT1s,
+                                       nullptr, nullptr, nullptr, nullptr, nimg, P.KT1s, hd, 3 * C, hd,
+                                       s.heads * P.KT1s, 0, 0, 0, EPI_NONE};
             PTX_TIMED(KID_IMG_WE, st, launch_gemm(g, st));
         }
     }
     if (pooled32) {
-        PTX_TIMED_EXT(KID_IMG_SCORES, st, launch_img_pool32(static_cast<const float *>(img), we, qkv0, nimg, s.in_dim, s.hw, C, P.KT1, EW,
+        PTX_TIMED_EXT(KID_IMG_SCORES, st, launch_img_pool32(static_cast<const float *>(img), we, qkv0, nimg, s.in_dim, s.hw, C, P.KT1s, EW,
                                                         attn_scale(hd), Gs, E, ML, st));
     } else if (pooled) {
-        PTX_TIMED_EXT(KID_IMG_SCORES, st, launch_img_pool(img, dt, we, qkv0, nimg, s.in_dim, s.hw, C, P.KT1,
+        PTX_TIMED_EXT(KID_IMG_SCORES, st, launch_img_pool(img, dt, we, qkv0, nimg, s.in_dim, s.hw, C, P.KT1s,
                                                       EW, attn_scale(hd), Gs, E, ML, st));
     } else {
-        PTX_TIMED(KID_IMG_SCORES, st, launch_img_scores(img, dt, we, qkv0, nimg, s.in_dim, s.hw, s.heads, C, P.KT1,
+        PTX_TIMED(KID_IMG_SCORES, st, launch_img_scores(img, dt, we, qkv0, nimg, s.in_dim, s.hw, s.heads, C, P.KT1s,
                                                         P.KT2p, attn_scale(hd), gbuf, st));
         PTX_TIMED(KID_IMG_GATHER, st, launch_img_gather(img, dt, nimg, s.in_dim, s.hw, s.heads, P.KT2p, gbuf, st));
     }
diff --git a/proxytransformation_amd/csrc/common.h b/proxytransformation_amd/csrc/common.h
--- a/proxytransformation_amd/csrc/common.h
+++ b/proxytransformation_amd/csrc/common.h
@@ -198,7 +198,7 @@
     size_t mlp_w1p[2], mlp_w2p[2];
     size_t qkvb[2];
     size_t total;
-    int KT1, KT2p, hd;
+    int KT1, KT1s, EW, KT2p, hd;
 };
 PrepLayout prep_layout(const PtxShape &s);
 
@@ -345,17 +345,17 @@
 int launch_img_mean(const void *img, int dt, int nimg, int in_dim, int hw, float *fm, hipStream_t st,
                     uint32_t *gate = nullptr, uint32_t gate_seq = 0);
 int launch_img_scores(const void *img, int dt, const float *we, const float *qkv0, int nimg, int in_dim,
-                      int hw, int heads, int C, int KT1, int KT2p, float scale, float *gbuf, hipStream_t st);
+                      int hw, int heads, int C, int KT1s, int KT2p, float scale, float *gbuf, hipStream_t st);
 int launch_img_gather(const void *img, int dt, int nimg, int in_dim, int hw, int heads, int KT2p, float *gbuf,
                       hipStream_t st);
 bool img_pool_supported(int dt, int in_dim, int hw, int heads);
 size_t img_pool_bytes(int nimg, int in_dim, int EW);
 void img_pool_layout(float *scratch, int nimg, int in_dim, int EW, float **Gs, float **E, float **ML);
 int launch_img_pool(const void *img, int dt, const float *we, const float *qkv0, int nimg, int in_dim, int hw, int C,
-                    int KT1, int EW, float scale, float *Gs, float *E, float *ML, hipStream_t st);
+                    int KT1s, int EW, float scale, float *Gs, float *E, float *ML, hipStream_t st);
 
 bool img_pool32_supported(int dt, int in_dim, int hw, int heads);
-int launch_img_pool32(const float *img, const float *we, const float *qkv0, int nimg, int in_dim, int hw, int C, int KT1, int EW,
+int launch_img_pool32(const float *img, const float *we, const float *qkv0, int nimg, int in_dim, int hw, int C, int KT1s, int EW,
                       float scale, float *Gs, float *E, float *ML, hipStream_t st);
 
 int run_prepare(const PtxShape &s, const PtxWeights &w, float *prep, hipStream_t st);
diff --git a/proxytransformation_amd/csrc/gemm.hip b/proxytransformation_amd/csrc/gemm.hip
--- a/proxytransformation_amd/csrc/gemm.hip
+++ b/proxytransformation_amd/csrc/gemm.hip
@@ -475,15 +475,18 @@
 #undef PTX_Y_COMPUTE
 
 template <int SK, int AMODE, bool CHAIN = false, bool LN = false>
-__global__ __launch_bounds__(SK * 64) void k_gemm32(GemmBatch gb)
-{
+__global__ __launch_bounds__(SK * 64, CHAIN ? 3 : 1) void k_gemm32(GemmBatch gb)
+{
+    constexpr bool ONE = CHAIN;
+    static_assert(!ONE || (AMODE == 0 && !LN), "the one-buffer form exists for the chained launch only");
+    constexpr int WSZ = (ONE ? 2 : 4) * 32 * LDT;
     const GemmProb pr = gb.p[blockIdx.z];
     const int row0 = blockIdx.x * 32, col0 = blockIdx.y * 32;
     if (row0 >= pr.R || col0 >= pr.N) return;
     extern __shared__ __attribute__((aligned(16))) float lds[];
     const int lane = threadIdx.x & 63;
     const int wv = __builtin_amdgcn_readfirstlane(threadIdx.x >> 6);
-    float *base = lds + (size_t)wv * (4 * 32 * LDT);
+    float *base = lds + (size_t)wv * WSZ;
     const int li = lane & 31, hh = lane >> 5;
     const int nk = (pr.K + BK - 1) / BK, per = (nk + SK - 1) / SK;
     const int it0 = wv * per, it1 = min(nk, it0 + per);
@@ -499,7 +502,7 @@
     (void)kA; (void)kB;
     size_t g0 = 0, g1 = 0, g2 = 0, g3 = 0, e0 = 0, e1 = 0, e2 = 0, e3 = 0;
     float fc0[4] = {0.f, 0.f, 0.f, 0.f}, fc1[4] = {0.f, 0.f, 0.f, 0.f}, fct[4] = {0.f, 0.f, 0.f, 0.f};
-    float *cts = lds + (size_t)SK * (4 * 32 * LDT);
+    float *cts = lds + (size_t)SK * WSZ;
     float *lnst = cts + 32 + wv * 64;
     const bool ln = LN && pr.lnp_in != nullptr;
     float mu4[4] = {0.0f, 0.0f, 0.0f, 0.0f};
@@ -568,7 +571,7 @@
     } while (0)
 #define PTX_STASH(S, buf_)                                                                \
     do {                                                                                  \
-        float *A_s = base + (buf_) * (2 * 32 * LDT) + r0 * LDT + kq, *W_s = A_s + 32 * LDT; \
+        float *A_s = base + (ONE ? 0 : (buf_)) * (2 * 32 * LDT) + r0 * LDT + kq, *W_s = A_s + 32 * LDT; \
         if (AMODE == 1) { PTX_MERGE(S, 0); PTX_MERGE(S, 1); PTX_MERGE(S, 2); PTX_MERGE(S, 3); } \
         if (LN) { sub4(a##S##0, mu4[0]); sub4(a##S##1, mu4[1]); sub4(a##S##2, mu4[2]); sub4(a##S##3, mu4[3]); } \
         *reinterpret_cast<float4 *>(A_s) = a##S##0;                                       \
@@ -582,7 +585,7 @@
     } while (0)
 #define PTX_COMPUTE(buf_)                                                                 \
     do {                                                                                  \
-        const float *A_ = base + (buf_) * (2 * 32 * LDT) + li * LDT + hh * 4, *W_ = A_ + 32 * LDT; \
+        const float *A_ = base + (ONE ? 0 : (buf_)) * (2 * 32 * LDT) + li * LDT + hh * 4, *W_ = A_ + 32 * LDT; \
         _Pragma("unroll") for (int kk = 0; kk < BK / 8; ++kk) {                           \
             const float4 a4 = *reinterpret_cast<const float4 *>(A_ + kk * 8);             \
             const float4 b4 = *reinterpret_cast<const float4 *>(W_ + kk * 8);             \
@@ -602,7 +605,7 @@
         if (pr.bias) bias = pr.bias[nc];
         if (ln) lnc = pr.ln_c[nc];
 #pragma unroll
-        for (int r = 0; r < 16; ++r) {
+        for (int r = 0; r < (ONE ? 0 : 16); ++r) {
             const int row = min(row0 + (r & 3) + 8 * (r >> 2) + 4 * hh, pr.R - 1);
             if (pr.res) resv[r] = pr.res[(size_t)row * pr.ldres + nc];
             if (has_ad) adv[r] = pr.ad[(size_t)row * pr.ldad + nc];
@@ -652,7 +655,7 @@
         if (wv == 0) {
 #pragma unroll
             for (int w = 1; w < SK; ++w) {
-                const float *o = lds + (size_t)w * (4 * 32 * LDT);
+                const float *o = lds + (size_t)w * WSZ;
 #pragma unroll
                 for (int r = 0; r < 16; ++r) acc[r] += o[r * 64 + lane];
             }
@@ -666,12 +669,12 @@
             const int rl = (r & 3) + 8 * (r >> 2) + 4 * hh, row = row0 + rl;
             float v = acc[r] + bias;
             if (ln) v = fmaf(lnst[2 * rl + 1], acc[r], lnc);
-            if (pr.epi == EPI_GELU) v = gelu_erf(v);
+            if (!ONE && pr.epi == EPI_GELU) v = gelu_erf(v);
             const bool ok = ncol && row < pr.R;
             if (ok) {
                 if (AMODE == 1) v = fmaf(cts[rl], adv[r], v);
-                else if (pr.rs) v = fmaf(rsv[r], adv[r], v);
-                if (pr.res) v += resv[r];
+                else if (!ONE && pr.rs) v = fmaf(rsv[r], adv[r], v);
+                if (!ONE && pr.res) v += resv[r];
                 pr.C[(size_t)row * pr.ldc + n] = v;
             }
             fin[r] = ok ? v : 0.0f;
@@ -729,7 +732,7 @@
 template <int SK, int AMODE, bool CHAIN = false, bool LN = false>
 static int launch_gemm32(const GemmBatch &gb, int rmax, int nmax, hipStream_t st)
 {
-    const size_t lds = sizeof(float) * (SK * 4 * 32 * LDT + 32 + 64 * SK);
+    const size_t lds = sizeof(float) * (SK * (CHAIN ? 2 : 4) * 32 * LDT + 32 + 64 * SK);
     if (lds > 64 * 1024)
         PTX_HIP(hipFuncSetAttribute(reinterpret_cast<const void *>(&k_gemm32<SK, AMODE, CHAIN, LN>),
                                     hipFuncAttributeMaxDynamicSharedMemorySize, (int)lds));
@@ -779,6 +782,8 @@
         PTX_REQUIRE(gb.n == 1 && gb.p[0].pg == nullptr && gb.p[0].c2 && gb.p[0].n2 >= 1 && gb.p[0].chain_tiles >= 1 &&
                     gb.p[0].chain_tiles * 32 <= gb.p[0].N && gb.p[0].K >= 4 * BK && gb.p[0].lnp_out == nullptr && !any_ln,
                     "gemm: bad chained-product description");
+        PTX_REQUIRE(!gb.p[0].res && !gb.p[0].rs && !gb.p[0].ad && gb.p[0].epi == EPI_NONE,
+                    "gemm: the chained product takes no residual, row-scaled addend or activation");
         PTX_TRY((launch_gemm32<4, 0, true>(gb, rmax, nmax, st)));
         PTX_LAUNCHED("k_gemm");
         return PTX_OK;
diff --git a/proxytransformation_amd/csrc/imgpool.hip b/proxytransformation_amd/csrc/imgpool.hip
--- a/proxytransformation_amd/csrc/imgpool.hip
+++ b/proxytransformation_amd/csrc/imgpool.hip
@@ -69,7 +69,7 @@
 
 struct PoolArgs {
     const unsigned short *img; const float *we, *qkv0;
-    int nimg, in_dim, hw, C, KT1, EW; float scale;
+    int nimg, in_dim, hw, C, KT1s, EW; float scale;
     float *Gs;
     float *E;
     float *ML;
@@ -92,14 +92,14 @@
     const int tid = threadIdx.x, lane = lane_id();
     const int wid = __builtin_amdgcn_readfirstlane(tid >> 6);
     const int n = lane & 15, kq = lane >> 4;
-    const float *wim = a.we + (size_t)im * heads * a.KT1;
+    const float *wim = a.we + (size_t)im * heads * a.KT1s;
     const unsigned short *f = a.img + (size_t)im * in_dim * hw;
     const int px = 128 * T + 8 * n;
     const bool full = px + 8 <= hw;
     const int cw = 64 * wid;
     float wv[heads];
 #pragma unroll
-    for (int h = 0; h < heads; ++h) wv[h] = wim[(size_t)h * a.KT1 + tid];
+    for (int h = 0; h < heads; ++h) wv[h] = wim[(size_t)h * a.KT1s + tid];
     u32x4 L[2][8];
     const bool tensor_end = im == a.nimg - 1 && cw + 64 == in_dim;
 #pragma unroll
@@ -122,7 +122,7 @@
 #pragma unroll
     for (int u = 0; u < 2; ++u) {
         const int p = 128 * T + lane + 64 * u;
-        ev[u] = p < hw ? wim[(size_t)wid * a.KT1 + in_dim + 1 + p] : 0.0f;
+        ev[u] = p < hw ? wim[(size_t)wid * a.KT1s + in_dim + 1 + p] : 0.0f;
     }
     float sq = 0.0f, sk = 0.0f;
     if (T == 0) {
@@ -307,10 +307,10 @@
 }
 
 int launch_img_pool(const void *img, int dt, const float *we, const float *qkv0, int nimg, int in_dim, int hw, int C,
-                    int KT1, int EW, float scale, float *Gs, float *E, float *ML, hipStream_t st)
+                    int KT1s, int EW, float scale, float *Gs, float *E, float *ML, hipStream_t st)
 {
     PTX_REQUIRE(EW % 4 == 0 && EW >= hw + 1 && hw > 128 && hw <= 255, "img pool: hw=%d EW=%d", hw, EW);
-    PoolArgs pa{static_cast<const unsigned short *>(img), we, qkv0, nimg, in_dim, hw, C, KT1, EW, scale, Gs, E, ML};
+    PoolArgs pa{static_cast<const unsigned short *>(img), we, qkv0, nimg, in_dim, hw, C, KT1s, EW, scale, Gs, E, ML};
     const size_t lds = sizeof(float) * 8 * kPoolHeads * 128 + sizeof(unsigned short) * 24 * (kPoolWPad + kPoolPPad);
     PTX_REQUIRE(lds <= 64 * 1024, "img pool: %zu B of LDS", lds);
     static const int nt_env = getenv("PTX_POOL_NT") ? atoi(getenv("PTX_POOL_NT")) : -1;
diff --git a/proxytransformation_amd/csrc/imgpool32.hip b/proxytransformation_amd/csrc/imgpool32.hip
--- a/proxytransformation_amd/csrc/imgpool32.hip
+++ b/proxytransformation_amd/csrc/imgpool32.hip
@@ -14,7 +14,7 @@
 
 struct Pool32Args {
     const float *img; const float *we, *qkv0;
-    int nimg, in_dim, hw, C, KT1, EW; float scale;
+    int nimg, in_dim, hw, C, KT1s, EW; float scale;
     float *Gs, *E, *ML;
 };
 
@@ -36,17 +36,17 @@
     const int wid = __builtin_amdgcn_readfirstlane(tid >> 6);
     const int n = lane & 7, kq = lane >> 3;
     const int mr = lane & 15, mk = lane >> 4;
-    const float *wim = a.we + (size_t)im * heads * a.KT1;
+    const float *wim = a.we + (size_t)im * heads * a.KT1s;
     const float *f = a.img + (size_t)im * in_dim * hw;
     float *T_w = T_s + (size_t)wid * (16 * kP32TRow);
     float wv[heads];
 #pragma unroll
-    for (int h = 0; h < heads; ++h) wv[h] = wim[(size_t)h * a.KT1 + tid];
+    for (int h = 0; h < heads; ++h) wv[h] = wim[(size_t)h * a.KT1s + tid];
     float ev[kP32Tiles];
 #pragma unroll
     for (int t = 0; t < kP32Tiles; ++t) {
         const int p = 128 * H + TP * t + (lane & (TP - 1));
-        ev[t] = p < hw ? wim[(size_t)wid * a.KT1 + in_dim + 1 + p] : 0.0f;
+        ev[t] = p < hw ? wim[(size_t)wid * a.KT1s + in_dim + 1 + p] : 0.0f;
     }
     float sq = 0.0f, sk = 0.0f;
     if (H == 0) {
@@ -201,12 +201,12 @@
     return dt == 0 && heads == kP32Heads && in_dim == 512 && hw > 128 && hw <= 255;
 }
 
-int launch_img_pool32(const float *img, const float *we, const float *qkv0, int nimg, int in_dim, int hw, int C, int KT1, int EW,
+int launch_img_pool32(const float *img, const float *we, const float *qkv0, int nimg, int in_dim, int hw, int C, int KT1s, int EW,
                       float scale, float *Gs, float *E, float *ML, hipStream_t st)
 {
     PTX_REQUIRE(EW % 4 == 0 && EW >= hw + 1 && hw > 128 && hw <= 255 && in_dim == 512, "img pool (fp32): hw=%d EW=%d in_dim=%d", hw, EW, in_dim);
     PTX_REQUIRE((reinterpret_cast<uintptr_t>(img) & 15) == 0, "img_feat must be 16-byte aligned");
-    Pool32Args pa{img, we, qkv0, nimg, in_dim, hw, C, KT1, EW, scale, Gs, E, ML};
+    Pool32Args pa{img, we, qkv0, nimg, in_dim, hw, C, KT1s, EW, scale, Gs, E, ML};
     const size_t lds = sizeof(float) * (512 * kP32Heads + 8 * kP32Heads * kP32Tile + kP32Heads * kP32Tile + 16 + 8 * 16 * kP32TRow);
     const dim3 grid(cdiv(nimg, 8) * 16);
     hipEvent_t ta = nullptr, tb = nullptr;
diff --git a/proxytransformation_amd/csrc/imgproxy.hip b/proxytransformation_amd/csrc/imgproxy.hip
--- a/proxytransformation_amd/csrc/imgproxy.hip
+++ b/proxytransformation_amd/csrc/imgproxy.hip
@@ -112,7 +112,7 @@
 template <int HEADS, int DT>
 __global__ __launch_bounds__(kScoreWaves * 64) void k_img_scores(
     const typename ImgStore<DT>::elem *__restrict__ img, const float *__restrict__ we, const float *__restrict__ qkv0,
-    int in_dim, int hw, int C, int KT1, int KT2p, float scale, float *__restrict__ gbuf)
+    int in_dim, int hw, int C, int KT1s, int KT2p, float scale, float *__restrict__ gbuf)
 {
     using St = ImgStore<DT>;
     constexpr int heads = HEADS, NW = kScoreWaves;
@@ -121,7 +121,7 @@
     float *S = sm + (NW / 2) * heads * 256;
     const int im = gridDim.x - 1 - blockIdx.x, tid = threadIdx.x, lane = lane_id();
     const int wid = __builtin_amdgcn_readfirstlane(tid >> 6);
-    const float *wim = we + (size_t)im * heads * KT1;
+    const float *wim = we + (size_t)im * heads * KT1s;
     const typename St::elem *f = img + (size_t)im * in_dim * hw;
     const int nv4 = hw >> 2, tail = hw & 3;
     const bool edge = tail != 0 && lane == nv4;
@@ -145,7 +145,7 @@
     for (int c0 = 0; c0 < cper; c0 += 64) {
     const int cn = min(64, cper - c0);
 #pragma unroll
-    for (int h = 0; h < HEADS; ++h) wreg[h] = lane < cn ? wim[(size_t)h * KT1 + cbeg + c0 + lane] : 0.0f;
+    for (int h = 0; h < HEADS; ++h) wreg[h] = lane < cn ? wim[(size_t)h * KT1s + cbeg + c0 + lane] : 0.0f;
     for (int cc = 0; cc < cn; cc += UNR) {
         typename St::px4 t[UNR];
 #pragma unroll
@@ -169,7 +169,7 @@
     for (int h = 0; h < HEADS; ++h)
 #pragma unroll
         for (int c = 0; c < 4; ++c)
-            ev[h][c] = (wid == 0 && vec && c >= cfirst) ? wim[(size_t)h * KT1 + in_dim + 1 + poff + c] : 0.0f;
+            ev[h][c] = (wid == 0 && vec && c >= cfirst) ? wim[(size_t)h * KT1s + in_dim + 1 + poff + c] : 0.0f;
 #pragma unroll
     for (int half = NW / 2; half >= 1; half >>= 1) {
         if (wid >= half && wid < 2 * half) {
@@ -213,7 +213,7 @@
 }
 
 int launch_img_scores(const void *img, int dt, const float *we, const float *qkv0, int nimg, int in_dim,
-                      int hw, int heads, int C, int KT1, int KT2p, float scale, float *gbuf,
+                      int hw, int heads, int C, int KT1s, int KT2p, float scale, float *gbuf,
                       hipStream_t st)
 {
     PTX_REQUIRE((heads == 4 || heads == 8 || heads == 16) && in_dim % (8 * kScoreWaves) == 0 && in_dim / kScoreWaves <= 256,
@@ -226,7 +226,7 @@
         if (lds > 64 * 1024)                                                                                                      \
             PTX_HIP(hipFuncSetAttribute(reinterpret_cast<const void *>(&k_img_scores<H_, DT_>), hipFuncAttributeMaxDynamicSharedMemorySize, (int)lds)); \
         hipLaunchKernelGGL((k_img_scores<H_, DT_>), dim3(nimg), dim3(kScoreWaves * 64), lds, st,                                    \
-                           static_cast<const ImgStore<DT_>::elem *>(img), we, qkv0, in_dim, hw, C, KT1, KT2p, scale, gbuf);         \
+                           static_cast<const ImgStore<DT_>::elem *>(img), we, qkv0, in_dim, hw, C, KT1s, KT2p, scale, gbuf);         \
     } while (0)
 #define PTX_SCORES_DT(DT_)                                                                                                          \
     do { if (heads == 4) PTX_SCORES(4, DT_); else if (heads == 8) PTX_SCORES(8, DT_); else PTX_SCORES(16, DT_); } while (0)
diff --git a/proxytransformation_amd/csrc/prep.hip b/proxytransformation_amd/csrc/prep.hip
--- a/proxytransformation_amd/csrc/prep.hip
+++ b/proxytransformation_amd/csrc/prep.hip
@@ -50,17 +50,17 @@
 }
 
 __global__ void k_prep_t1(const float *kw, const float *cw, const float *cb, const float *pos, int C,
-                          int in_dim, int hw, int heads, float scale, float *t1)
+                          int in_dim, int hw, int heads, int KT1s, float scale, float *t1)
 {
-    const int hd = C / heads, KT1 = in_dim + hw + 1;
+    const int hd = C / heads;
     const int i = blockIdx.x * blockDim.x + threadIdx.x;
-    if (i >= heads * KT1 * hd) return;
-    const int h = i / (KT1 * hd), rem = i - h * KT1 * hd, t = rem / hd, d = rem - t * hd;
+    if (i >= heads * KT1s * hd) return;
+    const int h = i / (KT1s * hd), rem = i - h * KT1s * hd, t = rem / hd, d = rem - t * hd;
     const float *wk = kw + (size_t)(h * hd + d) * C;
     float s = 0.0f;
     if (t < in_dim) {
         for (int j = 0; j < C; ++j) s = fmaf(wk[j], cw[(size_t)j * in_dim + t], s);
-    } else if (t > in_dim) {
+    } else if (t > in_dim && t <= in_dim + hw) {
         const float *pi = pos + (size_t)(t - in_dim) * C;
         for (int j = 0; j < C; ++j) s = fmaf(wk[j], cb[j] + pi[j], s);
     }
@@ -134,8 +134,8 @@
                        w.q_b, w.cm_w, w.cm_b, w.pos, C, s.in_dim, prep + P.w3, prep + P.b3);
     PTX_LAUNCHED("k_prep_w3");
     const float scale = (float)(1.0 / sqrt((double)P.hd));
-    hipLaunchKernelGGL(k_prep_t1, dim3(cdiv(s.heads * P.KT1 * P.hd, T)), dim3(T), 0, st, w.k_w, w.cm_w,
-                       w.cm_b, w.pos, C, s.in_dim, s.hw, s.heads, scale, prep + P.t1);
+    hipLaunchKernelGGL(k_prep_t1, dim3(cdiv(s.heads * P.KT1s * P.hd, T)), dim3(T), 0, st, w.k_w, w.cm_w,
+                       w.cm_b, w.pos, C, s.in_dim, s.hw, s.heads, P.KT1s, scale, prep + P.t1);
     PTX_LAUNCHED("k_prep_t1");
     hipLaunchKernelGGL(k_prep_t2, dim3(cdiv(s.heads * P.hd * P.KT2p, T)), dim3(T), 0, st, w.v_w, w.cm_w,
                        w.cm_b, w.pos, C, s.in_dim, s.hw, s.heads, P.KT2p, prep + P.t2);
diff --git a/scratch/pool_variants.py b/scratch/pool_variants.py
--- a/scratch/pool_variants.py
+++ b/scratch/pool_variants.py
@@ -23,7 +23,7 @@
         t = t[:a] + keep + t[b:]
     if name == "s12_notrail":
         t = variant("nostore_nostage3")
-        t = t.replace("ev[u] = p < hw ? wim[(size_t)wid * a.KT1 + in_dim + 1 + p] : 0.0f;", "ev[u] = p < hw ? 0.25f * (float)p : 0.0f;")
+        t = t.replace("ev[u] = p < hw ? wim[(size_t)wid * a.KT1s + in_dim + 1 + p] : 0.0f;", "ev[u] = p < hw ? 0.25f * (float)p : 0.0f;")
         t = t.replace("if (lane < hd) { sq = qv[lane]; sk = qv[a.C + lane]; }", "if (lane < hd) { sq = (float)lane; sk = 0.5f; (void)qv; }")
         return t
     if name == "s1only":
```
